# MILVLG/mmnas

Measured on AMD Instinct MI355X. Metric: supernet fwd+bwd steps/sec (VQA arch, bs=64), higher is better.
Workload: dtype f32 (bf16x6 split-operand MFMA, fp32 accumulate); 1 GPU; Net_Search supernet WEIGHT step: sample + fwd + BCE(sum) + bwd (+ gradient all-reduce), HSIZE 256, B=64/GPU, 100x2048 regions + 14 tokens, dropout 0.1 (search_vqa.py:279-292; BASELINE configs[2]); global_batch=64, parallelism=dp1, grad_allreduce=none, rccl_ranks=1, rank_id_sum_ok=True, lstm_fallback=False, dp_rows=1, dp_buckets=3, optimizer_in_step=False, gemm_split=6, hip_force_dev_kernarg=1

## Files before the change

include/mmnas_hip.h:

```cpp
#ifndef MMNAS_HIP_H
#define MMNAS_HIP_H

#include <stddef.h>
#include <stdint.h>

#ifdef __cplusplus
extern "C" {
#endif

#define MMNAS_ABI_VERSION 1

enum {
  MMNAS_OK = 0,
  MMNAS_E_SHAPE = -1,
  MMNAS_E_ARG = -2,
  MMNAS_E_LAUNCH = -3
};

enum {
  MMNAS_F_NORM = 1,
  MMNAS_F_RESIDUAL = 2,
  MMNAS_F_MASK = 4,
  MMNAS_F_REL = 8,
  MMNAS_F_SELF = 16,
  MMNAS_F_TRAIN = 32,
  MMNAS_F_RELRAW = 64
};

int mmnas_abi_version(void);
const char* mmnas_last_error(void);

enum {
  MMNAS_SWITCH_DEFAULT = 0,
  MMNAS_SWITCH_ENV = 1,
  MMNAS_SWITCH_SET = 2,
  MMNAS_SWITCH_UNREAD = 4
};
int mmnas_switch_count(void);
int mmnas_switch_info(int i, const char** name, const char** help, int* dflt, int* value, int* source);

int mmnas_dropout_mask(float* out, size_t n, float p, uint64_t seed, uint32_t site, void* stream);

enum { MMNAS_GEMM_NT = 0, MMNAS_GEMM_NN = 1, MMNAS_GEMM_TN = 2 };

typedef struct mmnas_gemm_group {
  int M;
  const float* A[3];
  const float* B[3];
  float* C;
  const float* bias;
  const float* residual;
  const float* gate;
  float* colsum;
  uint64_t drop_seed;
} mmnas_gemm_group;

#define MMNAS_GEMM_MAX_GROUPS 9

typedef struct mmnas_gemm_desc {
  int layout, ngroups, nseg;
  int N, K;
  int lda, ldb, ldc, ldres, ldgate;
  int relu, split_k;
  int accumulate;
  int b_planes;
  float alpha, gate_scale;
  float drop_p;
  uint32_t drop_site;
  uint64_t drop_seed;
  mmnas_gemm_group g[MMNAS_GEMM_MAX_GROUPS];
} mmnas_gemm_desc;

int mmnas_gemm(const mmnas_gemm_desc* d, void* stream);

int mmnas_gemm_ln(const mmnas_gemm_desc* d, const float* ln_a, const float* ln_b, float* y, float eps, void* stream);
int mmnas_set_gemm_ln(int on);

int mmnas_split_planes(const float* w, void* planes, size_t n, void* stream);

int mmnas_gemm_pair(const mmnas_gemm_desc* dgrad, const mmnas_gemm_desc* wgrad, void* stream);

int mmnas_lstm_supported(int E, int H);
int mmnas_lstm_fwd(const float* x_tm, const float* Wih, const float* Whh, const float* bias, float* xp, float* Hall,
                   float* Call, float* Gall, float* out, int T, int B, int E, int H, void* stream);
int mmnas_lstm_bwd(const float* dout, const float* Whh, const float* Call, const float* Gall, float* DG, float* dc,
                   float* scratch, int T, int B, int H, void* stream);

int mmnas_lstm_seq_supported(int H, int B);
int mmnas_lstm_seq_fwd(const float* xp, const float* bhh, const float* Whh, float* Hprev, float* Cs, float* Gall,
                       float* out, int T, int B, int H, void* stream);
int mmnas_lstm_seq_bwd(const float* dout, const float* Whh, const float* Cs, const float* Gall, float* DG, int T,
                       int B, int H, void* stream);
int mmnas_lstm_seq_timed_out(void* stream);

int mmnas_gemm_reload_tuning(void);

int mmnas_layernorm_fwd(const float* x, const float* a, const float* b, float* y,
                        int M, int d, float eps, void* stream);
int mmnas_layernorm_bwd(const float* x, const float* a, const float* dy, float* dx,
                        float* da, float* db, float* ddrop, float* dcol, float* ws,
                        float drop_p, uint64_t seed, uint32_t site,
                        int M, int d, float eps, void* stream);

size_t mmnas_layernorm_bwd_ws_floats(int M, int d);

int mmnas_colsum(const float* x, float* out, int M, int N, int ldx, void* stream);

int mmnas_eltwise_fwd(int kind, const float* x, float* y, size_t n, void* stream);
int mmnas_eltwise_bwd(int kind, const float* x, const float* dy, float* dx, size_t n, void* stream);
int mmnas_drop_add(const float* x, const float* res, float* y, size_t n, float drop_p, uint64_t seed,
                   uint32_t site, void* stream);
int mmnas_glu_fwd(const float* h, float* y, int M, int C, int relu, float drop_p, uint64_t seed,
                  uint32_t site, void* stream);
int mmnas_glu_bwd(const float* h, const float* dy, float* dh, int M, int C, int relu, float drop_p,
                  uint64_t seed, uint32_t site, void* stream);

int mmnas_row_is_zero(const float* f, uint8_t* mask, long rows, int d, void* stream);
int mmnas_glimpse1_supported(int K);
size_t mmnas_glimpse1_bwd_ws_floats(long rows, int K);
int mmnas_glimpse1_fwd(const float* x, const float* w, const float* b, float* y, long rows, int K, void* stream);
int mmnas_glimpse1_bwd(const float* dy, const float* x, const float* w, float* dx, float* dw, float* db, float* ws, long rows, int K,
                       void* stream);
int mmnas_attflat_pool_fwd(const float* logits, const float* x, const uint8_t* mask, float* probs, float* pooled,
                           int B, int S, int d, int G, void* stream);
int mmnas_attflat_pool_bwd(const float* probs, const float* x, const uint8_t* mask, const float* dpooled,
                           float* dlogits, float* dx, int B, int S, int d, int G, void* stream);

int mmnas_relation_embedding(const float* bbox, const int* nobj, float* out, int B, int S, void* stream);

int mmnas_semantic_embedding(const long* ques_ix, const int* nwords, const float* emb, float* out, int B, int S,
                             int E, long V, void* stream);

int mmnas_onehot_rows(float* out, int rows, int width, const int* idx_host, void* stream);

#define MMNAS_MIXED_MAX 8
size_t mmnas_mixed_sum_ws_floats(void);
int mmnas_node_mix_fwd(const float* const* z, const float* const* ln_a, const float* const* ln_b, int n, const float* gate,
                       float* out, int M, int d, float eps, void* stream);
int mmnas_node_mix_bwd(const float* const* z, const float* const* ln_a, const float* const* ln_b, int n, const float* gate,
                       const float* dout, float* d_active, int active, float* dgate, float* ws, int M, int d, float eps,
                       void* stream);
int mmnas_mixed_sum_fwd(const float* const* outs_host, int n, const float* gate, float* out, size_t count,
                        void* stream);
int mmnas_mixed_sum_bwd(const float* const* outs_host, int n, const float* gate, const float* dout,
                        float* d_active, int active, float* dgate, float* ws, size_t count, void* stream);
int mmnas_alpha_full_step(float* prob, const float* gate_grad, float* m, float* v, float* prob_grad, int rows,
                          int width, float lr, float beta1, float beta2, float eps, int step, void* stream);
int mmnas_alpha_full_step_wd(float* prob, const float* gate_grad, float* m, float* v, float* prob_grad, int rows,
                             int width, float lr, float beta1, float beta2, float eps, float weight_decay, int step,
                             void* stream);
int mmnas_alpha_two_step(float* prob, const float* gate_grad, float* m, float* v, float* prob_grad, int rows, int width,
                         const int* pair_host, float lr, float beta1, float beta2, float eps, float weight_decay, int step,
                         void* stream);

int mmnas_embedding_bwd(const long* idx, const float* dy, float* dW, long n_tok, int E, long V, void* stream);
size_t mmnas_embedding_bwd_det_ws_floats(long n_tok, int E);
int mmnas_embedding_bwd_det(const long* idx, const float* dy, float* dW, float* ws, long n_tok, int E, long V, float scale,
                            void* stream);

int mmnas_rel_bias_fwd(const float* rel, const float* Wr, const float* br, float* biasT,
                       int B, int Sq, int Sk, int R, int H, void* stream);
int mmnas_rel_bias_bwd(const float* rel, const float* Wr, const float* br, const float* dbiasT,
                       float* drel, float* dWr, float* dbr, int accumulate_drel,
                       int B, int Sq, int Sk, int R, int H, void* stream);

int mmnas_rel_fused_supported(int C, int R, int H);
int mmnas_rel_fused_fwd(const float* raw, const float* Wy, const float* by, const float* Wr,
                        const float* br, float* biasT, int B, int Sq, int Sk, int C, int R, int H,
                        void* stream);
size_t mmnas_rel_fused_bwd_ws_floats(int B, int Sq, int Sk);
int mmnas_rel_fused_bwd(const float* raw, const float* Wy, const float* by, const float* Wr,
                        const float* br, const float* dbiasT, float* dWy, float* dby, float* dWr,
                        float* dbr, float* ws, int B, int Sq, int Sk, int C, int R, int H,
                        void* stream);
int mmnas_rel_fused_fwd_ragged(const float* raw, const float* Wy, const float* by, const float* Wr, const float* br,
                               float* biasT, int B, int S, int C, int R, int H, const int* off, void* stream);
int mmnas_rel_fused_bwd_ragged(const float* raw, const float* Wy, const float* by, const float* Wr, const float* br,
                               const float* dbiasT, float* dWy, float* dby, float* dWr, float* dbr, float* ws,
                               int B, int S, int C, int R, int H, const int* off, const int* tile_off, int ntiles, void* stream);

#define MMNAS_REL_MULTI_MAX 32
typedef struct mmnas_rel_multi {
  int B, S, C, R, H, n_ops;
  const float* raw;
  const float* Wy; const float* by;
  float* dWy; float* dby;
  const float* Wr[MMNAS_REL_MULTI_MAX];
  const float* br[MMNAS_REL_MULTI_MAX];
  float* biasT[MMNAS_REL_MULTI_MAX];
  const float* dbiasT[MMNAS_REL_MULTI_MAX];
  float* dWr[MMNAS_REL_MULTI_MAX]; float* dbr[MMNAS_REL_MULTI_MAX];
  const int* off; const int* tile_off; int ntiles, reserved;
  float* ws;
  const unsigned char* key_mask;
} mmnas_rel_multi;
int mmnas_rel_multi_supported(int C, int R, int H);
size_t mmnas_rel_multi_bwd_ws_floats(int B, int S);
int mmnas_rel_multi_fwd(const mmnas_rel_multi* m, void* stream);
int mmnas_rel_multi_bwd(const mmnas_rel_multi* m, void* stream);
int mmnas_set_rel_hoist(int on);
int mmnas_set_rel_keylimit(int on);
int mmnas_set_guided_hoist(int on);
int mmnas_set_rel_overlap(int on);

typedef struct mmnas_mha_desc {
  int B, H, Sq, Sk, dh;
  int ldq, ldk, ldv, ldo;
  const float* Q; const float* K; const float* V;
  const uint8_t* mask;
  const float* biasT;
  float* O;
  float* lse;
  float drop_p; uint32_t drop_site; uint64_t drop_seed;
  const float* dO;
  float* dQ; float* dK; float* dV;
  float* dbiasT;
  float* delta;
  const int* q_off; const int* k_off;
} mmnas_mha_desc;

int mmnas_mha_core_fwd(const mmnas_mha_desc* d, void* stream);
int mmnas_mha_core_bwd(const mmnas_mha_desc* d, void* stream);
int mmnas_mha_core_fwd_indexed(const mmnas_mha_desc* d, const int* kv_idx, void* stream);

typedef struct mmnas_att_op {
  int B, Sq, Sk, d, di, H, dh, R;
  int flags;
  float drop_p, eps;
  uint64_t seed;
  const float* xq;
  const float* xkv;
  const uint8_t* mask;
  const float* rel;
  const float* Wq; const float* Wk; const float* Wv;
  const float* Wm;
  const float* Wr; const float* br;
  const float* ln_a; const float* ln_b;
  float* y;
  void* save;
  void* ws;
  const float* dy;
  float* dxq;
  float* dxkv;
  float* drel;
  float* dWq; float* dWk; float* dWv; float* dWm;
  float* dWr; float* dbr; float* dln_a; float* dln_b;
  int C;
  const float* Wy; const float* by;
  float* dWy; float* dby;
  const int* q_off; const int* k_off;
  int Mq, Mk;
  const int* rel_tile_off;
  int rel_ntiles, reserved2;
} mmnas_att_op;

typedef struct mmnas_plan {
  size_t save_bytes, ws_fwd_bytes, ws_bwd_bytes;
} mmnas_plan;

int mmnas_set_small_ops(int on);
int mmnas_set_small_bwd(int on);
int mmnas_set_small_ffn(int on);
int mmnas_att_op_plan(const mmnas_att_op* op, mmnas_plan* plan);
int mmnas_att_op_fwd(const mmnas_att_op* op, void* stream);
int mmnas_att_op_bwd(const mmnas_att_op* op, void* stream);

typedef struct mmnas_mlp_op {
  int M, nl;
  int dims[4];
  int flags;
  float drop_p, eps;
  uint64_t seed;
  const float* x;
  const float* W[3];
  const float* b[3];
  const float* ln_a; const float* ln_b;
  float* y;
  void* save; void* ws;
  const float* dy;
  float* dx;
  float* dW[3]; float* db[3];
  float* dln_a; float* dln_b;
} mmnas_mlp_op;

int mmnas_mlp_op_plan(const mmnas_mlp_op* op, mmnas_plan* plan);
int mmnas_mlp_op_fwd(const mmnas_mlp_op* op, void* stream);
int mmnas_mlp_op_bwd(const mmnas_mlp_op* op, void* stream);

#define MMNAS_CHAIN_MAX_OPS 128
enum { MMNAS_CHAIN_ATT = 0, MMNAS_CHAIN_MLP = 1 };
typedef struct mmnas_chain_op {
  int kind, on_y;
  mmnas_att_op att;
  mmnas_mlp_op mlp;
  int node, cand, detached, reserved;
} mmnas_chain_op;
typedef struct mmnas_chain {
  int n_ops;
  const mmnas_chain_op* ops;
  int B, Sx, Sy, d;
  const float* x_in; const float* y_in;
  const uint8_t* x_mask; const uint8_t* y_mask;
  const float* x_rel; const float* y_rel;
  void* arena;
  float* x_out; float* y_out;
  const float* dx_out; const float* dy_out;
  float* dx_in; float* dy_in;
  int use_side_stream, reserved;
  void* const* marks;
  int mixed, gate_width;
  const float* gate;
  float* dgate;
  const int* y_off;
  const int* y_tile_off;
  int Ny, y_ntiles;
} mmnas_chain;
int mmnas_chain_plan(const mmnas_chain* c, size_t* arena_bytes);
int mmnas_chain_fwd(const mmnas_chain* c, void* stream);
int mmnas_chain_bwd(const mmnas_chain* c, void* stream);
int mmnas_chain_join(void* main_stream, void* waiting_stream);
int mmnas_set_chain_overlap(int on);

typedef struct mmnas_attflat_side {
  int S, reserved;
  const float* x; const uint8_t* mask;
  const float* W1; const float* b1; const float* W2; const float* b2; const float* Wm; const float* bm;
  float* dW1; float* db1; float* dW2; float* db2; float* dWm; float* dbm;
  uint64_t seed;
  float* dx;
  const int* off;
  int M, reserved2;
} mmnas_attflat_side;
typedef struct mmnas_head {
  int B, d, MID, G, OUT, ANS, flags, reserved;
  float drop_p, eps;
  mmnas_attflat_side sx, sy;
  const float* ln_a; const float* ln_b; float* dln_a; float* dln_b;
  const float* Wp; const float* bp; float* dWp; float* dbp;
  float* logits;
  const float* dlogits;
  void* arena;
} mmnas_head;
int mmnas_head_plan(const mmnas_head* hd, size_t* arena_bytes);
int mmnas_head_fwd(const mmnas_head* hd, void* stream);
int mmnas_head_bwd(const mmnas_head* hd, void* stream);
int mmnas_bce_logits_sum_fwd(const float* logits, const float* target, float* loss, size_t n, void* stream);
int mmnas_bce_logits_bwd(const float* logits, const float* target, const float* go, float* dlogits, size_t n, void* stream);

int mmnas_im2col_seq(const float* x, float* col, int B, int S, int d, int k, void* stream);
int mmnas_pad_seq(const float* x, float* xp, int B, int S, int d, int front, int Sp, long rows_total, void* stream);
int mmnas_col2im_seq(const float* dcol, float* dx, int B, int S, int d, int k, void* stream);
int mmnas_dwconv_seq_fwd(const float* x, const float* w, const float* bias, float* y,
                         int B, int S, int d, int k, void* stream);
int mmnas_dwconv_seq_bwd(const float* x, const float* w, const float* dy, float* dx, float* dw,
                         float* db, int B, int S, int d, int k, void* stream);

typedef struct mmnas_segment { float* ptr; uint64_t offset; uint64_t n; } mmnas_segment;
int mmnas_pack_segments(const mmnas_segment* segs, int nseg, float* staging, float scale,
                        int direction, void* stream);
int mmnas_pack_rows(const float* x, const int* off, float* packed, int B, int S, int d, void* stream);
int mmnas_unpack_rows(const float* packed, const int* off, float* x, int B, int S, int d, void* stream);
int mmnas_pack_segments_host(const mmnas_segment* segs_host, int nseg, float* staging, float scale,
                             int direction, void* stream);

int mmnas_adam_step(float* p, const float* g, float* m, float* v, size_t n, float lr, float beta1,
                    float beta2, float eps, float weight_decay, const float* sumsq, float max_norm,
                    int step, void* stream);
int mmnas_sgd_step(float* p, const float* g, float* buf, size_t n, float lr, float momentum, float dampening,
                   float weight_decay, int nesterov, int first, const float* sumsq, float max_norm, void* stream);
int mmnas_sumsq(const float* g, size_t n, float* out, void* stream);

int mmnas_itm_pair_head(const float* xflat, const int* cap_idx, const float* yflat, const float* ln_a, const float* ln_b,
                        const float* Wp, const float* bp, float* logits, float* scores, const int* img_row, const int* cap_col,
                        long ld, int P, int D, float eps, void* stream);
int mmnas_rank_matrix(const float* S, int Ni, int Nc, long ld, int* i2t_rank, int* i2t_tie, int* t2i_rank, int* t2i_tie,
                      int* nan_flag, void* stream);
int mmnas_row_topk(const float* S, int N, int C, long ld, int k, int* out, int* nan_flag, void* stream);

int mmnas_vgd_targets(const float* bbox, const int* nobj, const double* gt, int B, int S, double thr, int mode, const double* norm,
                      float* scores, float* scores_mask, float* transformed, float* bbox_mask, int* err_flag, void* stream);
int mmnas_vgd_ground(const float* pred_scores, const float* pred_reg, const float* bbox, const float* img_shape, const float* gt,
                     int B, int S, double thr, long long* idx, float* box, double* iou, unsigned char* hit, long long* counts,
                     int* err_flag, void* stream);

int mmnas_vqa_answer(const float* logits, int B, int A, long ld, const int* slot_idx, long slot_base, int slot_step, int nslots,
                     const int* qmap, const int* row_ptr, const int* col, const int* k, int nq, long long* pred, int* credit,
                     int* count, int* err_flag, void* stream);
int mmnas_vqa_accuracy(const int* credit, const int* qmap, const int* ans_type, const int* ques_type, int N, int nq, int n_at,
                       int n_qt, long long* totals, int* err_flag, void* stream);
int mmnas_vqa_answer_targets(const int* ans_ix, int B, int n, int A, float* out, int* err_flag, void* stream);

int mmnas_vgd_loss_fwd(const float* pred_scores, const float* pred_reg, const float* scores, const float* bbox,
                       const float* scores_mask, const float* bbox_mask, int B, int S, int smask_full, int bmask_full, int mode,
                       int loss_avg, double batch_size, double lam, float* loss, float* parts, float* dpred_scores,
                       float* dpred_reg, void* stream);
int mmnas_itm_triplet_loss_fwd(const float* scores_pos, const float* scores_negc, const float* scores_negi, long n, int mode,
                               float margin, int mean, float* loss, float* grads, void* stream);
int mmnas_loss_grad_scale(const float* saved, const float* go, float* out, size_t n, void* stream);

int mmnas_vgd_head_supported(int S, int F);
size_t mmnas_vgd_head_bwd_ws_floats(int B, int S, int F);
int mmnas_vgd_head_fwd(const float* yf, const float* xp, const float* ln_a, const float* ln_b, const float* Ws, const float* bs,
                       const float* Wr, const float* br, float* scores, float* reg, float* mean, float* rstd, int B, int S, int F,
                       float eps, int log_softmax, void* stream);
int mmnas_vgd_head_bwd(const float* dscores, const float* dreg, const float* yf, const float* xp, const float* ln_a,
                       const float* ln_b, const float* Ws, const float* Wr, const float* scores, const float* mean,
                       const float* rstd, float* dyf, float* dxp, float* dln_a, float* dln_b, float* dWs, float* dbs, float* dWr,
                       float* dbr, float* ws, int B, int S, int F, float eps, int log_softmax, void* stream);

enum { MMNAS_K_GEMM = 0, MMNAS_K_MHA_FWD = 1, MMNAS_K_MHA_BWD = 2, MMNAS_K_REL_FWD = 3, MMNAS_K_REL_BWD = 4,
       MMNAS_K_ROWOPS = 5, MMNAS_K_LSTM = 6, MMNAS_K_SMALL = 7 , MMNAS_K_COUNT = 8 };
typedef struct mmnas_prof_stat { double ms, flops, bytes; long launches; } mmnas_prof_stat;
int mmnas_prof_enable(int on);
int mmnas_prof_collect(mmnas_prof_stat* stats );

#ifdef __cplusplus
}
#endif
#endif
```

mmnas_amd/_lib.py:

```python
import ctypes as C
import logging
import os

import torch

from . import switches

_HERE = os.path.dirname(os.path.abspath(__file__))
LIB_PATH = os.environ.get(switches.LIB_PATH.name) or os.path.join(_HERE, 'lib', 'libmmnas_hip.so')

log = logging.getLogger('mmnas_amd')


def _launch_configuration():
    name = 'HIP_FORCE_DEV_KERNARG'
    if name in os.environ:
        return os.environ[name], 'inherited'
    if torch.cuda.is_initialized():
        log.warning('mmnas_amd was imported after HIP had initialised and %s is not set: kernel arguments go through host-visible '
                    'memory, the ~300 short launches of a step run 20-40 %% slower.  Export %s=1 or import mmnas / mmnas_amd '
                    'before the first CUDA call.', name, name)
        return None, 'unset_after_hip_init'
    os.environ[name] = '1'
    return '1', 'set_by_library'


KERNARG_VALUE, KERNARG_SOURCE = _launch_configuration()

F_NORM, F_RESIDUAL, F_MASK, F_REL, F_SELF, F_TRAIN, F_RELRAW = 1, 2, 4, 8, 16, 32, 64
GEMM_NT, GEMM_NN, GEMM_TN = 0, 1, 2

_fp = C.c_void_p


class GemmGroup(C.Structure):
    _fields_ = [('M', C.c_int), ('A', _fp * 3), ('B', _fp * 3), ('C', _fp), ('bias', _fp),
                ('residual', _fp), ('gate', _fp), ('colsum', _fp), ('drop_seed', C.c_uint64)]


GEMM_MAX_GROUPS = 9


class GemmDesc(C.Structure):
    _fields_ = [('layout', C.c_int), ('ngroups', C.c_int), ('nseg', C.c_int), ('N', C.c_int), ('K', C.c_int),
                ('lda', C.c_int), ('ldb', C.c_int), ('ldc', C.c_int), ('ldres', C.c_int), ('ldgate', C.c_int),
                ('relu', C.c_int), ('split_k', C.c_int), ('accumulate', C.c_int), ('b_planes', C.c_int), ('alpha', C.c_float), ('gate_scale', C.c_float),
                ('drop_p', C.c_float), ('drop_site', C.c_uint32), ('drop_seed', C.c_uint64),
                ('g', GemmGroup * GEMM_MAX_GROUPS)]


class MhaDesc(C.Structure):
    _fields_ = [('B', C.c_int), ('H', C.c_int), ('Sq', C.c_int), ('Sk', C.c_int), ('dh', C.c_int),
                ('ldq', C.c_int), ('ldk', C.c_int), ('ldv', C.c_int), ('ldo', C.c_int),
                ('Q', _fp), ('K', _fp), ('V', _fp), ('mask', _fp), ('biasT', _fp), ('O', _fp), ('lse', _fp),
                ('drop_p', C.c_float), ('drop_site', C.c_uint32), ('drop_seed', C.c_uint64),
                ('dO', _fp), ('dQ', _fp), ('dK', _fp), ('dV', _fp), ('dbiasT', _fp), ('delta', _fp), ('q_off', _fp), ('k_off', _fp)]


class AttOp(C.Structure):
    _fields_ = [('B', C.c_int), ('Sq', C.c_int), ('Sk', C.c_int), ('d', C.c_int), ('di', C.c_int),
                ('H', C.c_int), ('dh', C.c_int), ('R', C.c_int), ('flags', C.c_int),
                ('drop_p', C.c_float), ('eps', C.c_float), ('seed', C.c_uint64),
                ('xq', _fp), ('xkv', _fp), ('mask', _fp), ('rel', _fp),
                ('Wq', _fp), ('Wk', _fp), ('Wv', _fp), ('Wm', _fp), ('Wr', _fp), ('br', _fp),
                ('ln_a', _fp), ('ln_b', _fp), ('y', _fp), ('save', _fp), ('ws', _fp),
                ('dy', _fp), ('dxq', _fp), ('dxkv', _fp), ('drel', _fp),
                ('dWq', _fp), ('dWk', _fp), ('dWv', _fp), ('dWm', _fp), ('dWr', _fp), ('dbr', _fp),
                ('dln_a', _fp), ('dln_b', _fp),
                ('C', C.c_int), ('Wy', _fp), ('by', _fp), ('dWy', _fp), ('dby', _fp),
                ('q_off', _fp), ('k_off', _fp), ('Mq', C.c_int), ('Mk', C.c_int), ('rel_tile_off', _fp), ('rel_ntiles', C.c_int), ('reserved2', C.c_int)]


class Plan(C.Structure):
    _fields_ = [('save_bytes', C.c_size_t), ('ws_fwd_bytes', C.c_size_t), ('ws_bwd_bytes', C.c_size_t)]


class MlpOp(C.Structure):
    _fields_ = [('M', C.c_int), ('nl', C.c_int), ('dims', C.c_int * 4), ('flags', C.c_int),
                ('drop_p', C.c_float), ('eps', C.c_float), ('seed', C.c_uint64),
                ('x', _fp), ('W', _fp * 3), ('b', _fp * 3), ('ln_a', _fp), ('ln_b', _fp), ('y', _fp),
                ('save', _fp), ('ws', _fp), ('dy', _fp), ('dx', _fp), ('dW', _fp * 3), ('db', _fp * 3),
                ('dln_a', _fp), ('dln_b', _fp)]


class ChainOp(C.Structure):
    _fields_ = [('kind', C.c_int), ('on_y', C.c_int), ('att', AttOp), ('mlp', MlpOp),
                ('node', C.c_int), ('cand', C.c_int), ('detached', C.c_int), ('reserved', C.c_int)]


class Chain(C.Structure):
    _fields_ = [('n_ops', C.c_int), ('ops', C.POINTER(ChainOp)), ('B', C.c_int), ('Sx', C.c_int), ('Sy', C.c_int),
                ('d', C.c_int), ('x_in', _fp), ('y_in', _fp), ('x_mask', _fp), ('y_mask', _fp), ('x_rel', _fp),
                ('y_rel', _fp), ('arena', _fp), ('x_out', _fp), ('y_out', _fp), ('dx_out', _fp), ('dy_out', _fp),
                ('dx_in', _fp), ('dy_in', _fp), ('use_side_stream', C.c_int), ('reserved', C.c_int),
                ('marks', C.c_void_p), ('mixed', C.c_int), ('gate_width', C.c_int), ('gate', _fp), ('dgate', _fp),
                ('y_off', _fp), ('y_tile_off', _fp), ('Ny', C.c_int), ('y_ntiles', C.c_int)]


CHAIN_MAX_OPS = 128


class AttFlatSide(C.Structure):
    _fields_ = [('S', C.c_int), ('reserved', C.c_int), ('x', _fp), ('mask', _fp), ('W1', _fp), ('b1', _fp), ('W2', _fp),
                ('b2', _fp), ('Wm', _fp), ('bm', _fp), ('dW1', _fp), ('db1', _fp), ('dW2', _fp), ('db2', _fp), ('dWm', _fp),
                ('dbm', _fp), ('seed', C.c_uint64), ('dx', _fp), ('off', _fp), ('M', C.c_int), ('reserved2', C.c_int)]


class Head(C.Structure):
    _fields_ = [('B', C.c_int), ('d', C.c_int), ('MID', C.c_int), ('G', C.c_int), ('OUT', C.c_int), ('ANS', C.c_int),
                ('flags', C.c_int), ('reserved', C.c_int), ('drop_p', C.c_float), ('eps', C.c_float),
                ('sx', AttFlatSide), ('sy', AttFlatSide), ('ln_a', _fp), ('ln_b', _fp), ('dln_a', _fp), ('dln_b', _fp),
                ('Wp', _fp), ('bp', _fp), ('dWp', _fp), ('dbp', _fp), ('logits', _fp), ('dlogits', _fp), ('arena', _fp)]


REL_MULTI_MAX = 32


class RelMulti(C.Structure):
    _fields_ = [('B', C.c_int), ('S', C.c_int), ('C', C.c_int), ('R', C.c_int), ('H', C.c_int), ('n_ops', C.c_int),
                ('raw', _fp), ('Wy', _fp), ('by', _fp), ('dWy', _fp), ('dby', _fp),
                ('Wr', _fp * REL_MULTI_MAX), ('br', _fp * REL_MULTI_MAX), ('biasT', _fp * REL_MULTI_MAX),
                ('dbiasT', _fp * REL_MULTI_MAX), ('dWr', _fp * REL_MULTI_MAX), ('dbr', _fp * REL_MULTI_MAX),
                ('off', _fp), ('tile_off', _fp), ('ntiles', C.c_int), ('reserved', C.c_int), ('ws', _fp), ('key_mask', _fp)]


class ProfStat(C.Structure):
    _fields_ = [('ms', C.c_double), ('flops', C.c_double), ('bytes', C.c_double), ('launches', C.c_long)]


K_NAMES = ['gemm', 'mha_fwd', 'mha_bwd', 'rel_fwd', 'rel_bwd', 'rowops', 'lstm', 'small_ops']


class Segment(C.Structure):
    _fields_ = [('ptr', _fp), ('offset', C.c_uint64), ('n', C.c_uint64)]


_i, _f, _u32, _u64, _sz = C.c_int, C.c_float, C.c_uint32, C.c_uint64, C.c_size_t
SYMBOLS = {
    'mmnas_abi_version': (_i, []),
    'mmnas_last_error': (C.c_char_p, []),
    'mmnas_switch_count': (_i, []),
    'mmnas_switch_info': (_i, [_i, C.POINTER(C.c_char_p), C.POINTER(C.c_char_p)] + [C.POINTER(_i)] * 3),
    'mmnas_dropout_mask': (_i, [_fp, _sz, _f, _u64, _u32, _fp]),
    'mmnas_gemm': (_i, [C.POINTER(GemmDesc), _fp]),
    'mmnas_split_planes': (_i, [_fp, _fp, _sz, _fp]),
    'mmnas_gemm_ln': (_i, [C.POINTER(GemmDesc), _fp, _fp, _fp, _f, _fp]),
    'mmnas_set_gemm_ln': (_i, [_i]),
    'mmnas_gemm_pair': (_i, [C.POINTER(GemmDesc), C.POINTER(GemmDesc), _fp]),
    'mmnas_gemm_reload_tuning': (_i, []),
    'mmnas_lstm_supported': (_i, [_i, _i]),
    'mmnas_lstm_fwd': (_i, [_fp] * 9 + [_i, _i, _i, _i, _fp]),
    'mmnas_lstm_bwd': (_i, [_fp] * 7 + [_i, _i, _i, _fp]),
    'mmnas_lstm_seq_supported': (_i, [_i, _i]),
    'mmnas_set_small_ops': (_i, [_i]),
    'mmnas_set_small_bwd': (_i, [_i]),
    'mmnas_set_small_ffn': (_i, [_i]),
    'mmnas_set_chain_overlap': (_i, [_i]),
    'mmnas_lstm_seq_fwd': (_i, [_fp] * 7 + [_i, _i, _i, _fp]),
    'mmnas_lstm_seq_bwd': (_i, [_fp] * 5 + [_i, _i, _i, _fp]),
    'mmnas_lstm_seq_timed_out': (_i, [_fp]),
    'mmnas_layernorm_fwd': (_i, [_fp, _fp, _fp, _fp, _i, _i, _f, _fp]),
    'mmnas_layernorm_bwd': (_i, [_fp, _fp, _fp, _fp, _fp, _fp, _fp, _fp, _fp, _f, _u64, _u32, _i, _i, _f, _fp]),
    'mmnas_layernorm_bwd_ws_floats': (_sz, [_i, _i]),
    'mmnas_colsum': (_i, [_fp, _fp, _i, _i, _i, _fp]),
    'mmnas_eltwise_fwd': (_i, [_i, _fp, _fp, _sz, _fp]),
    'mmnas_eltwise_bwd': (_i, [_i, _fp, _fp, _fp, _sz, _fp]),
    'mmnas_drop_add': (_i, [_fp, _fp, _fp, _sz, _f, _u64, _u32, _fp]),
    'mmnas_glu_fwd': (_i, [_fp, _fp, _i, _i, _i, _f, _u64, _u32, _fp]),
    'mmnas_glu_bwd': (_i, [_fp, _fp, _fp, _i, _i, _i, _f, _u64, _u32, _fp]),
    'mmnas_rel_bias_fwd': (_i, [_fp, _fp, _fp, _fp, _i, _i, _i, _i, _i, _fp]),
    'mmnas_rel_bias_bwd': (_i, [_fp, _fp, _fp, _fp, _fp, _fp, _fp, _i, _i, _i, _i, _i, _i, _fp]),
    'mmnas_row_is_zero': (_i, [_fp, _fp, C.c_long, _i, _fp]),
    'mmnas_glimpse1_supported': (_i, [_i]),
    'mmnas_glimpse1_bwd_ws_floats': (_sz, [C.c_long, _i]),
    'mmnas_glimpse1_fwd': (_i, [_fp, _fp, _fp, _fp, C.c_long, _i, _fp]),
    'mmnas_glimpse1_bwd': (_i, [_fp, _fp, _fp, _fp, _fp, _fp, _fp, C.c_long, _i, _fp]),
    'mmnas_attflat_pool_fwd': (_i, [_fp, _fp, _fp, _fp, _fp, _i, _i, _i, _i, _fp]),
    'mmnas_attflat_pool_bwd': (_i, [_fp, _fp, _fp, _fp, _fp, _fp, _i, _i, _i, _i, _fp]),
    'mmnas_relation_embedding': (_i, [_fp, _fp, _fp, _i, _i, _fp]),
    'mmnas_semantic_embedding': (_i, [_fp, _fp, _fp, _fp, _i, _i, _i, C.c_long, _fp]),
    'mmnas_onehot_rows': (_i, [_fp, _i, _i, C.POINTER(C.c_int), _fp]),
    'mmnas_mixed_sum_ws_floats': (_sz, []),
    'mmnas_mixed_sum_fwd': (_i, [C.POINTER(_fp), _i, _fp, _fp, _sz, _fp]),
    'mmnas_mixed_sum_bwd': (_i, [C.POINTER(_fp), _i, _fp, _fp, _fp, _i, _fp, _fp, _sz, _fp]),
    'mmnas_alpha_full_step': (_i, [_fp, _fp, _fp, _fp, _fp, _i, _i, _f, _f, _f, _f, _i, _fp]),
    'mmnas_alpha_full_step_wd': (_i, [_fp, _fp, _fp, _fp, _fp, _i, _i, _f, _f, _f, _f, _f, _i, _fp]),
    'mmnas_alpha_two_step': (_i, [_fp, _fp, _fp, _fp, _fp, _i, _i, C.POINTER(C.c_int), _f, _f, _f, _f, _f, _i, _fp]),
    'mmnas_embedding_bwd': (_i, [_fp, _fp, _fp, C.c_long, _i, C.c_long, _fp]),
    'mmnas_node_mix_fwd': (_i, [_fp, _fp, _fp, _i, _fp, _fp, _i, _i, _f, _fp]),
    'mmnas_node_mix_bwd': (_i, [_fp, _fp, _fp, _i, _fp, _fp, _fp, _i, _fp, _fp, _i, _i, _f, _fp]),
    'mmnas_embedding_bwd_det': (_i, [_fp, _fp, _fp, _fp, C.c_long, _i, C.c_long, _f, _fp]),
    'mmnas_embedding_bwd_det_ws_floats': (_sz, [C.c_long, _i]),
    'mmnas_rel_fused_supported': (_i, [_i, _i, _i]),
    'mmnas_rel_fused_fwd': (_i, [_fp, _fp, _fp, _fp, _fp, _fp, _i, _i, _i, _i, _i, _i, _fp]),
    'mmnas_rel_fused_bwd_ws_floats': (_sz, [_i, _i, _i]),
    'mmnas_rel_fused_bwd': (_i, [_fp, _fp, _fp, _fp, _fp, _fp, _fp, _fp, _fp, _fp, _fp, _i, _i, _i, _i, _i, _i, _fp]),
    'mmnas_rel_fused_fwd_ragged': (_i, [_fp, _fp, _fp, _fp, _fp, _fp, _i, _i, _i, _i, _i, _fp, _fp]),
    'mmnas_rel_fused_bwd_ragged': (_i, [_fp] * 11 + [_i, _i, _i, _i, _i, _fp, _fp, _i, _fp]),
    'mmnas_rel_multi_supported': (_i, [_i, _i, _i]),
    'mmnas_rel_multi_bwd_ws_floats': (_sz, [_i, _i]),
    'mmnas_rel_multi_fwd': (_i, [C.POINTER(RelMulti), _fp]),
    'mmnas_rel_multi_bwd': (_i, [C.POINTER(RelMulti), _fp]),
    'mmnas_set_rel_hoist': (_i, [_i]),
    'mmnas_set_rel_keylimit': (_i, [_i]),
    'mmnas_set_guided_hoist': (_i, [_i]),
    'mmnas_set_rel_overlap': (_i, [_i]),
    'mmnas_mha_core_fwd': (_i, [C.POINTER(MhaDesc), _fp]),
    'mmnas_mha_core_bwd': (_i, [C.POINTER(MhaDesc), _fp]),
    'mmnas_mha_core_fwd_indexed': (_i, [C.POINTER(MhaDesc), _fp, _fp]),
    'mmnas_itm_pair_head': (_i, [_fp] * 11 + [C.c_long, _i, _i, _f, _fp]),
    'mmnas_rank_matrix': (_i, [_fp, _i, _i, C.c_long, _fp, _fp, _fp, _fp, _fp, _fp]),
    'mmnas_row_topk': (_i, [_fp, _i, _i, C.c_long, _i, _fp, _fp, _fp]),
    'mmnas_vgd_targets': (_i, [_fp, _fp, _fp, _i, _i, C.c_double, _i, _fp, _fp, _fp, _fp, _fp, _fp, _fp]),
    'mmnas_vgd_ground': (_i, [_fp] * 5 + [_i, _i, C.c_double] + [_fp] * 7),
    'mmnas_vqa_answer': (_i, [_fp, _i, _i, C.c_long, _fp, C.c_long, _i, _i] + [_fp] * 4 + [_i] + [_fp] * 5),
    'mmnas_vqa_accuracy': (_i, [_fp] * 4 + [_i] * 4 + [_fp, _fp, _fp]),
    'mmnas_vqa_answer_targets': (_i, [_fp, _i, _i, _i, _fp, _fp, _fp]),
    'mmnas_vgd_loss_fwd': (_i, [_fp] * 6 + [_i] * 6 + [C.c_double, C.c_double] + [_fp] * 5),
    'mmnas_itm_triplet_loss_fwd': (_i, [_fp, _fp, _fp, C.c_long, _i, _f, _i, _fp, _fp, _fp]),
    'mmnas_loss_grad_scale': (_i, [_fp, _fp, _fp, _sz, _fp]),
    'mmnas_vgd_head_supported': (_i, [_i, _i]),
    'mmnas_vgd_head_bwd_ws_floats': (_sz, [_i, _i, _i]),
    'mmnas_vgd_head_fwd': (_i, [_fp] * 12 + [_i, _i, _i, _f, _i, _fp]),
    'mmnas_vgd_head_bwd': (_i, [_fp] * 20 + [_i, _i, _i, _f, _i, _fp]),
    'mmnas_att_op_plan': (_i, [C.POINTER(AttOp), C.POINTER(Plan)]),
    'mmnas_att_op_fwd': (_i, [C.POINTER(AttOp), _fp]),
    'mmnas_att_op_bwd': (_i, [C.POINTER(AttOp), _fp]),
    'mmnas_mlp_op_plan': (_i, [C.POINTER(MlpOp), C.POINTER(Plan)]),
    'mmnas_mlp_op_fwd': (_i, [C.POINTER(MlpOp), _fp]),
    'mmnas_mlp_op_bwd': (_i, [C.POINTER(MlpOp), _fp]),
    'mmnas_chain_plan': (_i, [C.POINTER(Chain), C.POINTER(C.c_size_t)]),
    'mmnas_chain_fwd': (_i, [C.POINTER(Chain), _fp]),
    'mmnas_chain_bwd': (_i, [C.POINTER(Chain), _fp]),
    'mmnas_chain_join': (_i, [_fp, _fp]),
    'mmnas_head_plan': (_i, [C.POINTER(Head), C.POINTER(C.c_size_t)]),
    'mmnas_head_fwd': (_i, [C.POINTER(Head), _fp]),
    'mmnas_head_bwd': (_i, [C.POINTER(Head), _fp]),
    'mmnas_bce_logits_sum_fwd': (_i, [_fp, _fp, _fp, _sz, _fp]),
    'mmnas_bce_logits_bwd': (_i, [_fp, _fp, _fp, _fp, _sz, _fp]),
    'mmnas_im2col_seq': (_i, [_fp, _fp, _i, _i, _i, _i, _fp]),
    'mmnas_pack_rows': (_i, [_fp, _fp, _fp, _i, _i, _i, _fp]),
    'mmnas_unpack_rows': (_i, [_fp, _fp, _fp, _i, _i, _i, _fp]),
    'mmnas_pad_seq': (_i, [_fp, _fp, _i, _i, _i, _i, _i, C.c_long, _fp]),
    'mmnas_col2im_seq': (_i, [_fp, _fp, _i, _i, _i, _i, _fp]),
    'mmnas_dwconv_seq_fwd': (_i, [_fp, _fp, _fp, _fp, _i, _i, _i, _i, _fp]),
    'mmnas_dwconv_seq_bwd': (_i, [_fp, _fp, _fp, _fp, _fp, _fp, _i, _i, _i, _i, _fp]),
    'mmnas_pack_segments': (_i, [_fp, _i, _fp, _f, _i, _fp]),
    'mmnas_pack_segments_host': (_i, [C.POINTER(Segment), _i, _fp, _f, _i, _fp]),
    'mmnas_adam_step': (_i, [_fp, _fp, _fp, _fp, _sz, _f, _f, _f, _f, _f, _fp, _f, _i, _fp]),
    'mmnas_sgd_step': (_i, [_fp, _fp, _fp, _sz, _f, _f, _f, _f, _i, _i, _fp, _f, _fp]),
    'mmnas_sumsq': (_i, [_fp, _sz, _fp, _fp]),
    'mmnas_prof_enable': (_i, [_i]),
    'mmnas_prof_collect': (_i, [C.POINTER(ProfStat)]),
}

_lib = None


class MMNasHipError(RuntimeError):
    pass


def lib():
    global _lib
    if _lib is None:
        if not os.path.exists(LIB_PATH):
            raise MMNasHipError(
                'libmmnas_hip.so not found at %s -- build it with `python -c "import __graft_entry__ as g; '
                'g.build()"` or `make -C mmnas_amd/csrc`.  There is no CPU fallback.' % LIB_PATH)
        l = C.CDLL(LIB_PATH)
        for name, (res, args) in SYMBOLS.items():
            fn = getattr(l, name)
            fn.restype = res
            fn.argtypes = args
        if l.mmnas_abi_version() != 1:
            raise MMNasHipError('libmmnas_hip.so ABI version %d != 1' % l.mmnas_abi_version())
        _lib = l
    return _lib


def check(rc):
    if rc != 0:
        raise MMNasHipError('libmmnas_hip: %s (code %d)' % (lib().mmnas_last_error().decode(), rc))


def ptr(t):
    if t is None:
        return None
    if not t.is_cuda:
        raise MMNasHipError('mmnas_amd operators run on the MI355X only: got a %s tensor (no CPU fallback)'
                            % t.device)
    if not t.is_contiguous():
        raise MMNasHipError('non-contiguous tensor passed to the HIP boundary')
    return t.data_ptr()


def fptr(t):
    if t is not None and t.dtype != torch.float32:
        raise MMNasHipError('expected float32, got %s' % t.dtype)
    return ptr(t)


def stream():
    return torch._C._cuda_getCurrentRawStream(torch._C._cuda_getDevice())
```

mmnas_amd/csrc/gemm.hip:

```cpp
#include <stddef.h>
#include <string.h>
#include <map>
#include <mutex>
#include <utility>
#include <algorithm>
#include <climits>
#include "common.h"
#include "gemm_split.h"

namespace mmnas {

struct GemmGroupK {
  int M;
  int tile0;
  const float* A[3];
  const float* B[3];
  float* C;
  const float* bias;
  const float* residual;
  const float* gate;
  float* colsum;
  uint32_t seed_lo, site_key;
};

constexpr int MAXG = MMNAS_GEMM_MAX_GROUPS;

struct GemmK {
  int ngroups, nseg, N, K;
  int lda, ldb, ldc, ldres, ldgate;
  int relu, accumulate;
  int tiles_n, ntiles;
  int xcd_remap;
  int gm;
  int ntk, T;
  int mode;
  int n_full, full_per, sk_per;
  int P;
  int U;
  int gtile0[MAXG];
  int tn_shift;
  unsigned nt_magic;
  float* ws;
  int* cnt;
  int avec, bvec;
  float alpha, gate_scale;
  DropCfg drop;
  const float* lg_cprev;
  const float* lg_c;
  float* lg_cout;
  float* lg_gates;
  float* lg_h2;
  float* lg_dc;
  const float* lg_act;
  int lg_ldh2, lg_pad;
  GemmGroupK g[MAXG];
};

enum { MODE_TILE = 0, MODE_SPLIT = 1, MODE_STREAM = 2 };

__device__ __forceinline__ int cdiv_dev(int a, int b) { return (a + b - 1) / b; }

#ifndef MMNAS_OCC64
#define MMNAS_OCC64 4
#endif
#ifndef MMNAS_OCC_NS
#define MMNAS_OCC_NS 3
#endif
#ifndef MMNAS_OCC128
#define MMNAS_OCC128 2
#endif
#ifndef MMNAS_BK
#define MMNAS_BK 32
#endif
constexpr int BK = MMNAS_BK;
constexpr int LDK = BK + 4;
constexpr int KQ = BK / 4;

typedef unsigned long long u64;
__device__ __forceinline__ void st_agent(u64* ptr, float a, float b) {
  __hip_atomic_store(ptr, ((u64)__float_as_uint(b) << 32) | __float_as_uint(a), __ATOMIC_RELAXED, __HIP_MEMORY_SCOPE_AGENT);
}
__device__ __forceinline__ u64 ld_agent(const u64* ptr) {
  return __hip_atomic_load(ptr, __ATOMIC_RELAXED, __HIP_MEMORY_SCOPE_AGENT);
}

#ifndef MMNAS_TMAP
#define MMNAS_TMAP 2
#endif
template <int BR>
__device__ __forceinline__ void t_map(int tid, int j, int& kp, int& rq) {
#if MMNAS_TMAP == 2
  const int hi = tid >> 5;
  constexpr int RB = BR / 32;
  rq = (tid & 7) | ((hi % RB) << 3);
  kp = ((tid >> 3) & 3) + 4 * (hi / RB) + (1024 / BR) * j;
#elif MMNAS_TMAP == 1
  rq = (tid >> 3) % (BR / 4);
  kp = (tid & 7) + 8 * ((tid >> 3) / (BR / 4)) + (1024 / BR) * j;
#else
  kp = tid / (BR / 4) + (1024 / BR) * j;
  rq = tid % (BR / 4);
#endif
}
__device__ __forceinline__ int t_flip(int rq) { return MMNAS_TMAP == 2 ? (rq >> 2) & 1 : 0; }

template <int NS>
__device__ __forceinline__ void split_put(unsigned* dst, float x0, float x1, int row, int kp) {
  constexpr int RSW = NS * 16 + 4;
  unsigned a0, a1 = 0, a2 = 0;
  split_pair<NS>(x0, x1, a0, a1, a2);
  unsigned* d = dst + row * RSW + swz(kp, row);
  d[0] = a0;
  if (NS > 1) d[16] = a1;
  if (NS > 2) d[32] = a2;
}
template <int BR, int NS>
__device__ __forceinline__ void split_store_t(unsigned* dst, const float4 e, const float4 o, int tid, int j) {
  int kp, rq;
  t_map<BR>(tid, j, kp, rq);
  const int row = 4 * rq, fl = t_flip(rq);
  split_put<NS>(dst, fl ? e.y : e.x, fl ? o.y : o.x, row + fl, kp);
  split_put<NS>(dst, fl ? e.x : e.y, fl ? o.x : o.y, row + 1 - fl, kp);
  split_put<NS>(dst, fl ? e.w : e.z, fl ? o.w : o.z, row + 2 + fl, kp);
  split_put<NS>(dst, fl ? e.z : e.w, fl ? o.z : o.w, row + 3 - fl, kp);
}

#ifdef MMNAS_DBG_STAMP
__device__ unsigned long long g_stamp_acc[8];
__device__ unsigned long long g_life_acc[8];
#endif

template <int BM, int BN, int NS>
struct GemmShape {
  static constexpr int RSW = NS ? NS * 16 + 4 : LDK;
  static constexpr int A_SZ = BM * RSW, B_SZ = BN * RSW;
};

template <int BM, int BN, bool AKC, bool BKC, bool FAST, int NS, int EPI = 0, int PF = 1, bool BDMA = false, int LEAN = 0>
__device__ __forceinline__ void gemm_body(const GemmK& p, const int bid, const int nwg, const int koff,
                                          float* __restrict__ As, float* __restrict__ Bs, float* __restrict__ As1,
                                          float* __restrict__ Bs1, int& s_old) {
  static_assert(PF == 1 || (PF == 2 && FAST && (NS == 0 || NS == 1 || NS == 3)), "the two-stage prefetch exists for the buffer-load path (fp32, bf16x1 and bf16x6)");
  static_assert(NS == 0 || (FAST && BK == 32), "the bf16-split path exists for the buffer-load path only");
  static_assert(!BDMA || (NS == 3 && AKC && BKC && FAST && PF == 1 && BM == 64 && BN == 64 && EPI == 0), "LDS-DMA weight planes: NT 64^2 bf16x6 only");
  static_assert(!LEAN || (NS > 0 && (AKC || !BKC) && FAST && PF == 2 && BM == 64 && BN == 64 && EPI == 0 && !BDMA), "lean form: 64^2 split-operand kernels");
  constexpr bool LEAN_TN = LEAN && !AKC;
  constexpr bool LEAN_EL = LEAN == 3;
  constexpr bool LEAN_SW = LEAN && AKC && !LEAN_EL;
  constexpr bool LEAN_WT = (LEAN_SW && LEAN == 1) || LEAN_EL;
  constexpr int RSWB = 48;
  constexpr int WM = BM / 2, WN = BN / 2, TM = WM / 32, TN = WN / 32;
  constexpr int RSW = GemmShape<BM, BN, NS>::RSW;
  constexpr int NA = BM * BK / 1024, NB = BN * BK / 1024;

#ifdef MMNAS_DBG_STAMP
  unsigned long long life_prev = __builtin_readcyclecounter();
#define MMNAS_LIFE(i) do { const unsigned long long c_ = __builtin_readcyclecounter(); if (threadIdx.x == 0 && bid == MMNAS_DBG_STAMP) g_life_acc[i] += c_ - life_prev; life_prev = c_; } while (0)
#else
#define MMNAS_LIFE(i) do { } while (0)
#endif
  {
    const char* ka = (const char*)__builtin_amdgcn_kernarg_segment_ptr() + koff;
    unsigned t0, t1, t2, t3, t4, t5, t6, t7, t8, t9;
    asm volatile(
        "s_load_dword %0, %10, 0x0\n\ts_load_dword %1, %10, 0x40\n\ts_load_dword %2, %10, 0x80\n\t"
        "s_load_dword %3, %10, 0xc0\n\ts_load_dword %4, %10, 0x100\n\ts_load_dword %5, %10, 0x140\n\t"
        "s_load_dword %6, %10, 0x180\n\ts_load_dword %7, %10, 0x1c0\n\ts_load_dword %8, %10, 0x200\n\t"
        "s_load_dword %9, %10, 0x240\n\ts_waitcnt lgkmcnt(0)"
        : "=&s"(t0), "=&s"(t1), "=&s"(t2), "=&s"(t3), "=&s"(t4), "=&s"(t5), "=&s"(t6), "=&s"(t7), "=&s"(t8), "=&s"(t9)
        : "s"(ka)
        : "memory");
  }
  static_assert(offsetof(GemmK, g) + 3 * sizeof(GemmGroupK) > 0x200 && offsetof(GemmK, g) + 3 * sizeof(GemmGroupK) <= 0x280,
                "update the kernel-argument warm-up loads (header + the first three groups; further groups -- the architecture "
                "step's node-wide launches -- take their first-touch miss)");

  MMNAS_LIFE(0);
  const int tid = threadIdx.x;
  const int lane = tid & 63, wave = tid >> 6;
  const int l31 = lane & 31, hh = lane >> 5;
  const int wm = wave >> 1, wn = wave & 1;

  struct Hdr { int N, K, lda, ldb, tiles_n, ntiles, xcd_remap, gm, ntk, T, mode, n_full, full_per, sk_per, P, U, gt[MAXG]; };
  Hdr h;
  h.N = p.N; h.K = p.K; h.lda = p.lda; h.ldb = p.ldb; h.tiles_n = p.tiles_n; h.ntiles = p.ntiles; h.xcd_remap = p.xcd_remap;
  h.gm = p.gm; h.ntk = p.ntk; h.T = p.T; h.mode = p.mode; h.n_full = p.n_full; h.full_per = p.full_per; h.sk_per = p.sk_per;
  h.P = p.P; h.U = p.U;
#pragma unroll
  for (int g = 0; g < MAXG; ++g) h.gt[g] = p.gtile0[g];
  asm volatile("" : "+s"(h.N), "+s"(h.K), "+s"(h.lda), "+s"(h.ldb), "+s"(h.tiles_n), "+s"(h.ntiles), "+s"(h.xcd_remap), "+s"(h.gm),
               "+s"(h.ntk), "+s"(h.T), "+s"(h.mode), "+s"(h.n_full), "+s"(h.full_per), "+s"(h.sk_per), "+s"(h.P));
  static_assert(MAXG == 9, "the list of group boundaries below names nine groups");
  asm volatile("" : "+s"(h.U), "+s"(h.gt[1]), "+s"(h.gt[2]), "+s"(h.gt[3]), "+s"(h.gt[4]), "+s"(h.gt[5]), "+s"(h.gt[6]), "+s"(h.gt[7]),
               "+s"(h.gt[8]));
  int v;
  {
    const int q = nwg >> 3, r = nwg & 7, xcd = bid & 7, in = bid >> 3;
    v = (xcd < r ? xcd * (q + 1) : r * (q + 1) + (xcd - r) * q) + in;
    if (!h.xcd_remap) v = bid;
  }
  const int mode = LEAN_TN ? (int)MODE_SPLIT : (LEAN_WT ? (int)MODE_TILE : h.mode);
  int u = 0, uend = 1;
  int vs = v;
  int whole = -1;
  if (mode == MODE_STREAM) {
    if (h.n_full > 0) {
      const int xcd = bid & 7, li = bid >> 3;
      if (li < h.sk_per) vs = xcd * h.sk_per + li;
      else whole = xcd * h.full_per + (li - h.sk_per);
    }
    if (whole < 0) { u = vs * h.P; uend = min(h.U, u + h.P); }
  }

  while (u < uend) {
    int tile, q0, nq;
    if (mode == MODE_TILE || whole >= 0) {
      tile = whole >= 0 ? whole : v; q0 = 0; nq = h.T;
      u = uend;
    } else if (!LEAN_SW && !LEAN_EL && mode == MODE_SPLIT) {
      const int sl = LEAN_TN ? (int)__umulhi((unsigned)v, p.nt_magic) : v / h.ntiles;
      tile = v - sl * h.ntiles;
      q0 = sl * h.P;
      nq = min(h.P, h.T - q0);
      u = uend;
      if (nq <= 0) break;
    } else {
      const int tt = u / h.T;
      tile = h.n_full + tt;
      q0 = u - tt * h.T;
      nq = min(h.T - q0, uend - u);
      u += nq;
    }
    int grp = 0;
#pragma unroll
    for (int g = 1; g < MAXG; ++g) grp += tile >= h.gt[g] ? 1 : 0;
    const GemmGroupK& G = p.g[grp];
    const int Mg = G.M;
    const int tl = tile - G.tile0;
    float* __restrict__ const Cp = G.C;
    const float* __restrict__ const biasp = G.bias;
    const float* __restrict__ const resp = G.residual;
    const float* __restrict__ const gatep = G.gate;
    float* __restrict__ const csp = G.colsum;
    const uint32_t gseed_lo = G.seed_lo, gsite_key = G.site_key;
    const float* const Aseg[3] = {G.A[0], G.A[1], G.A[2]};
    const float* const Bseg[3] = {G.B[0], G.B[1], G.B[2]};
    int tile_m, tile_n;
    if (LEAN) {
      tile_m = tl >> p.tn_shift;
      tile_n = tl - (tile_m << p.tn_shift);
    } else {
      const int tiles_m = cdiv_dev(Mg, BM);
      const int per_block = h.gm * h.tiles_n;
      const int blk = tl / per_block, in = tl - blk * per_block;
      const int rows = min(h.gm, tiles_m - blk * h.gm);
      tile_n = in / rows;
      tile_m = blk * h.gm + (in - tile_n * rows);
    }
    const int m0 = tile_m * BM, n0 = tile_n * BN;

    f32x16 acc[TM][TN];
#pragma unroll
    for (int i = 0; i < TM; ++i)
#pragma unroll
      for (int j = 0; j < TN; ++j)
#pragma unroll
        for (int r = 0; r < 16; ++r) acc[i][j][r] = 0.f;

    float4 rA[2][NA], rB[2][NB];

    unsigned offa[NA], offb[NB];
    size_t bdma_off[3] = {0, 0, 0};
    unsigned stepa = 0, stepb = 0;
    unsigned bytesa = 0, bytesb = 0;
    if (FAST) {
#pragma unroll
      for (int i = 0; i < NA; ++i) {
        const int f = tid + 256 * i;
        if (AKC) {
          const int row = NS ? kc_row(f) : f / KQ, kq = f % KQ, gr = m0 + row;
          offa[i] = gr < Mg ? (unsigned)(gr * h.lda + 4 * kq) * 4u : ~0u;
        } else if (NS) {
          int kp, rq;
          t_map<BM>(tid, i >> 1, kp, rq);
          const int gr = m0 + 4 * rq;
          offa[i] = gr < Mg ? (unsigned)((2 * kp + (i & 1)) * h.lda + gr) * 4u : ~0u;
        } else {
          const int k = f / (BM / 4), rq = f - k * (BM / 4), gr = m0 + 4 * rq;
          offa[i] = gr < Mg ? (unsigned)(k * h.lda + gr) * 4u : ~0u;
        }
      }
#pragma unroll
      for (int i = 0; i < NB; ++i) {
        const int f = tid + 256 * i;
        if (BDMA) {
          offb[i] = 0;
        } else if (BKC) {
          const int row = NS ? kc_row(f) : f / KQ, kq = f % KQ, gr = n0 + row;
          offb[i] = gr < h.N ? (unsigned)(gr * h.ldb + 4 * kq) * 4u : ~0u;
        } else if (NS) {
          int kp, rq;
          t_map<BN>(tid, i >> 1, kp, rq);
          const int gr = n0 + 4 * rq;
          offb[i] = gr < h.N ? (unsigned)((2 * kp + (i & 1)) * h.ldb + gr) * 4u : ~0u;
        } else {
          const int k = f / (BN / 4), rq = f - k * (BN / 4), gr = n0 + 4 * rq;
          offb[i] = gr < h.N ? (unsigned)(k * h.ldb + gr) * 4u : ~0u;
        }
      }
      if (BDMA) {
#pragma unroll
        for (int i = 0; i < 3; ++i) {
          const int o = (wave * 3 + i) * 1024 + lane * 16;
          const int r = o / 192, w = o - r * 192, c = w >> 6, j = ((w & 63) >> 4) ^ ((r >> 2) & 3);
          bdma_off[i] = ((size_t)c * (size_t)h.N * (size_t)h.ldb + (size_t)(n0 + r) * (size_t)h.ldb + 8 * j) * 2u;
        }
      }
      stepa = AKC ? BK * 4u : (unsigned)h.lda * BK * 4u;
      stepb = BKC ? BK * 4u : (unsigned)h.ldb * BK * 4u;
      bytesa = (unsigned)(AKC ? Mg : h.K) * (unsigned)h.lda * 4u;
      bytesb = (unsigned)(BKC ? h.N : h.K) * (unsigned)h.ldb * 4u;
    }

    int seg_c = 0, kt_c = 0;
    if (LEAN_TN) kt_c = q0;
    else if (q0 != 0) { seg_c = q0 / h.ntk; kt_c = q0 - seg_c * h.ntk; }
    auto gload_to = [&](int q, bool live, const int st, const int dbuf = 0) __attribute__((always_inline)) {
      float4* const ra = rA[st];
      float4* const rb = rB[st];
      const int seg = seg_c, kt = kt_c;
      if (++kt_c == h.ntk) { kt_c = 0; ++seg_c; }
      const float* __restrict__ Ap = seg == 0 ? Aseg[0] : (seg == 1 ? Aseg[1] : Aseg[2]);
      const float* __restrict__ Bp = seg == 0 ? Bseg[0] : (seg == 1 ? Bseg[1] : Bseg[2]);
      if (FAST) {
        const __amdgpu_buffer_rsrc_t ra_src = __builtin_amdgcn_make_buffer_rsrc((void*)Ap, 0, bytesa, 0x00020000);
        const __amdgpu_buffer_rsrc_t rb_src = __builtin_amdgcn_make_buffer_rsrc((void*)Bp, 0, bytesb, 0x00020000);
        const unsigned ka = (unsigned)kt * stepa, kb = (unsigned)kt * stepb;
        if (LEAN_SW || LEAN_EL) {
          const __amdgpu_buffer_rsrc_t la_src = __builtin_amdgcn_make_buffer_rsrc((void*)Ap, 0, live ? bytesa : 0u, 0x00020000);
          const __amdgpu_buffer_rsrc_t lb_src = __builtin_amdgcn_make_buffer_rsrc((void*)Bp, 0, live ? bytesb : 0u, 0x00020000);
#pragma unroll
          for (int i = 0; i < NA; ++i) ra[i] = buf_load4(la_src, offa[i], ka);
#pragma unroll
          for (int i = 0; i < NB; ++i) rb[i] = buf_load4(lb_src, offb[i], kb);
          return;
        }
#pragma unroll
        for (int i = 0; i < NA; ++i) ra[i] = buf_load4(ra_src, (offa[i] == ~0u || !live) ? ~0u : offa[i] + ka);
        if (BDMA) {
          const char* bsrc = reinterpret_cast<const char*>(Bp) + (size_t)kt * 64u;
          float* const bd = dbuf ? Bs1 : Bs;
          const int wv = __builtin_amdgcn_readfirstlane(wave);
#pragma unroll
          for (int i = 0; i < 3; ++i)
            __builtin_amdgcn_global_load_lds((const __attribute__((address_space(1))) void*)(bsrc + bdma_off[i]),
                                             (__attribute__((address_space(3))) void*)(bd + (wv * 3 + i) * 256), 16, 0, 0);
          return;
        }
#pragma unroll
        for (int i = 0; i < NB; ++i) rb[i] = buf_load4(rb_src, (offb[i] == ~0u || !live) ? ~0u : offb[i] + kb);
        return;
      }
      const int k0 = kt * BK, kend = h.K;
#pragma unroll
      for (int i = 0; i < NA; ++i) {
        const int f = tid + 256 * i;
        float4 v4 = make_float4(0.f, 0.f, 0.f, 0.f);
        if (AKC) {
          const int row = f / KQ, kq = f % KQ;
          const int gr = m0 + row, gk = k0 + 4 * kq;
          if (gr < Mg && gk < kend) {
            const float* src = Ap + (size_t)gr * h.lda + gk;
            if (p.avec) v4 = *reinterpret_cast<const float4*>(src);
            else {
              v4.x = src[0];
              if (gk + 1 < kend) v4.y = src[1];
              if (gk + 2 < kend) v4.z = src[2];
              if (gk + 3 < kend) v4.w = src[3];
            }
          }
        } else {
          const int k = f / (BM / 4), rq = f - k * (BM / 4);
          const int gk = k0 + k, gr = m0 + 4 * rq;
          if (gk < kend && gr < Mg) {
            const float* src = Ap + (size_t)gk * h.lda + gr;
            if (p.avec) v4 = *reinterpret_cast<const float4*>(src);
            else {
              v4.x = src[0];
              if (gr + 1 < Mg) v4.y = src[1];
              if (gr + 2 < Mg) v4.z = src[2];
              if (gr + 3 < Mg) v4.w = src[3];
            }
          }
        }
        ra[i] = v4;
      }
#pragma unroll
      for (int i = 0; i < NB; ++i) {
        const int f = tid + 256 * i;
        float4 v4 = make_float4(0.f, 0.f, 0.f, 0.f);
        if (BKC) {
          const int row = f / KQ, kq = f % KQ;
          const int gr = n0 + row, gk = k0 + 4 * kq;
          if (gr < h.N && gk < kend) {
            const float* src = Bp + (size_t)gr * h.ldb + gk;
            if (p.bvec) v4 = *reinterpret_cast<const float4*>(src);
            else {
              v4.x = src[0];
              if (gk + 1 < kend) v4.y = src[1];
              if (gk + 2 < kend) v4.z = src[2];
              if (gk + 3 < kend) v4.w = src[3];
            }
          }
        } else {
          const int k = f / (BN / 4), rq = f - k * (BN / 4);
          const int gk = k0 + k, gr = n0 + 4 * rq;
          if (gk < kend && gr < h.N) {
            const float* src = Bp + (size_t)gk * h.ldb + gr;
            if (p.bvec) v4 = *reinterpret_cast<const float4*>(src);
            else {
              v4.x = src[0];
              if (gr + 1 < h.N) v4.y = src[1];
              if (gr + 2 < h.N) v4.z = src[2];
              if (gr + 3 < h.N) v4.w = src[3];
            }
          }
        }
        rb[i] = v4;
      }
    };
    auto gload = [&](int q, int dbuf = 0) __attribute__((always_inline)) { gload_to(q, true, 0, dbuf); };

    auto lstore_from = [&](int buf, const int st) __attribute__((always_inline)) {
      const float4* const ra = rA[st];
      const float4* const rb = rB[st];
      float* a = buf ? As1 : As;
      float* b = buf ? Bs1 : Bs;
      if (NS) {
        unsigned* ua = reinterpret_cast<unsigned*>(a);
        unsigned* ub = reinterpret_cast<unsigned*>(b);
        if (AKC) {
#pragma unroll
          for (int i = 0; i < NA; ++i) split_store_kc<BM, true, NS ? NS : 2>(ua, ra[i], tid + 256 * i);
        } else {
#pragma unroll
          for (int j = 0; j < NA / 2; ++j) split_store_t<BM, NS ? NS : 2>(ua, ra[2 * j], ra[2 * j + 1], tid, j);
        }
        if (BDMA) {
        } else if (BKC) {
#pragma unroll
          for (int i = 0; i < NB; ++i) split_store_kc<BN, true, NS ? NS : 2>(ub, rb[i], tid + 256 * i);
        } else {
#pragma unroll
          for (int j = 0; j < NB / 2; ++j) split_store_t<BN, NS ? NS : 2>(ub, rb[2 * j], rb[2 * j + 1], tid, j);
        }
        return;
      }
#pragma unroll
      for (int i = 0; i < NA; ++i) {
        const int f = tid + 256 * i;
        if (AKC) {
          const int row = f / KQ, kq = f % KQ;
          *reinterpret_cast<float4*>(a + row * LDK + 4 * kq) = ra[i];
        } else {
          const int k = f / (BM / 4), rq = f - k * (BM / 4);
          *reinterpret_cast<float4*>(a + k * BM + 4 * rq) = ra[i];
        }
      }
#pragma unroll
      for (int i = 0; i < NB; ++i) {
        const int f = tid + 256 * i;
        if (BKC) {
          const int row = f / KQ, kq = f % KQ;
          *reinterpret_cast<float4*>(b + row * LDK + 4 * kq) = rb[i];
        } else {
          const int k = f / (BN / 4), rq = f - k * (BN / 4);
          *reinterpret_cast<float4*>(b + k * BN + 4 * rq) = rb[i];
        }
      }
    };
    auto lstore = [&](int buf) __attribute__((always_inline)) { lstore_from(buf, 0); };

    auto mfma_block = [&](int buf) __attribute__((always_inline)) {
#ifdef MMNAS_DBG_NOMFMA
      return;
#endif
      const float* a = buf ? As1 : As;
      const float* b = buf ? Bs1 : Bs;
      if (NS) {
#pragma unroll
// ... 587 lines not shown
    const mmnas_gemm_group& s = d->g[g];
    if (!akc && s.M % 4 != 0) avec = 0;
    MMNAS_REQUIRE(s.M > 0 && s.C, MMNAS_E_ARG, "mmnas_gemm: group %d M=%d C=%p", g, s.M, (void*)s.C);
    k.g[g].M = s.M; k.g[g].C = s.C; k.g[g].bias = s.bias; k.g[g].residual = s.residual; k.g[g].gate = s.gate;
    k.g[g].colsum = s.colsum;
    {
      const DropCfg gd = s.drop_seed ? make_drop(d->drop_p, s.drop_seed, d->drop_site) : k.drop;
      k.g[g].seed_lo = gd.seed_lo; k.g[g].site_key = gd.site_key;
    }
    MMNAS_REQUIRE(!(s.colsum && accumulate), MMNAS_E_ARG, "mmnas_gemm: no column sums when accumulating onto C");
    for (int i = 0; i < 3; ++i) {
      k.g[g].A[i] = s.A[i]; k.g[g].B[i] = s.B[i];
      if (i < d->nseg) {
        MMNAS_REQUIRE(s.A[i] && s.B[i], MMNAS_E_ARG, "mmnas_gemm: group %d segment %d null operand", g, i);
        if (((uintptr_t)s.A[i] & 15) != 0) avec = 0;
        if (((uintptr_t)s.B[i] & 15) != 0) bvec = 0;
      }
    }
    sumM += s.M;
    const double ab = 4.0 * (akc ? (double)(s.M + 128) : (double)d->K) * d->lda;
    if (ab > maxbytes) maxbytes = ab;
  }
  const double bb = 4.0 * (bkc ? (double)(d->N + 128) : (double)d->K) * d->ldb;
  if (bb > maxbytes) maxbytes = bb;
  k.avec = avec; k.bvec = bvec;
  bool fast = avec && bvec && (d->K % BK == 0 || tn) && maxbytes < 4.0e9;
  if (g_tune.generic) fast = false;
  k.ntk = cdiv(d->K, BK);
  k.T = k.ntk * d->nseg;

  auto ntiles_for = [&](int bt) {
    long n = 0;
    for (int g = 0; g < d->ngroups; ++g) n += (long)cdiv(d->g[g].M, bt) * cdiv(d->N, bt);
    return n;
  };
  const int min_units = g_tune.min_units;
  bool big = ntiles_for(128) >= 2048;
  if (g_tune.tile == 128) big = true;
  if (g_tune.tile == 64 || g_tune.tile == 12864) big = false;
  bool wide = !big && g_tune.tile == 12864 && !accumulate && fast && g_tune.split != 2 && g_tune.split != 1;
  if (wide) {
    long n = 0;
    for (int g = 0; g < d->ngroups; ++g) n += (long)cdiv(d->g[g].M, 128) * cdiv(d->N, 64);
    if (n < g_tune.wide_min) wide = false;
  }
  const int bt = big ? 128 : 64;
  const int btm = wide ? 128 : bt, btn = bt;
  k.tiles_n = cdiv(d->N, btn);
  long t0 = 0;
  for (int g = 0; g < MAXG; ++g) k.gtile0[g] = INT_MAX;
  for (int g = 0; g < d->ngroups; ++g) { k.g[g].tile0 = k.gtile0[g] = (int)t0; t0 += (long)cdiv(d->g[g].M, btm) * k.tiles_n; }
  MMNAS_REQUIRE(t0 < (1l << 30), MMNAS_E_SHAPE, "mmnas_gemm: too many output tiles");
  k.ntiles = (int)t0;
  k.gm = g_tune.gm > 0 ? g_tune.gm : 8;
  k.xcd_remap = g_tune.xcd;
  const int slots = g_tune.wgs > 0 ? (g_tune.wgs < MAX_WGS ? g_tune.wgs : MAX_WGS) : ((big || wide) ? 512 : 1024);
  const double per_cu = (double)k.ntiles / 256.0;
  const double dp_eff = per_cu / (double)(long)(per_cu + 0.999999);
  const long long U = (long long)k.ntiles * k.T;
  int sk = g_tune.sk;
  k.mode = MODE_TILE;
  k.P = k.T;
  int nwg = k.ntiles;
  if (accumulate && sk != 0) {
    int want;
    if (g_tune.split_slots > 0) want = g_tune.split_slots / k.ntiles;
    else {
      want = (k.T + g_tune.split_p / 2) / g_tune.split_p;
      if ((long)want * k.ntiles < g_tune.split_minwg) want = (g_tune.split_minwg + k.ntiles - 1) / k.ntiles;
    }
    if (want < 1) want = 1;
    if (want > k.T / min_units) want = k.T / min_units;
    if (want > 1) {
      k.P = (k.T + want - 1) / want;
      const int S = (k.T + k.P - 1) / k.P;
      MMNAS_REQUIRE((long long)S * k.ntiles < (1ll << 30), MMNAS_E_SHAPE, "mmnas_gemm: too many split-K pieces");
      k.mode = MODE_SPLIT;
      nwg = S * k.ntiles;
    }
  } else if (!accumulate && sk != 0 && !big && !wide && U < (1ll << 30) && k.ntiles <= MAX_CNT_TILES && g_tune.wgs == 0 &&
             sk == 1 && k.ntiles > 256 && k.ntiles < 8192 && k.ntiles % 256 != 0 && k.T >= g_tune.hyb_t) {
    const int n_full = (k.ntiles / 256) * 256, R = k.ntiles - n_full;
    const long long Ut = (long long)R * k.T;
    long long P = (Ut + 255) / 256;
    if (P < 2) P = 2;
    int n_sk = (int)((Ut + P - 1) / P);
    n_sk = (n_sk + 7) / 8 * 8;
    k.mode = MODE_STREAM;
    k.n_full = n_full; k.full_per = n_full / 8; k.sk_per = n_sk / 8;
    k.P = (int)P;
    k.U = (int)Ut;
    nwg = n_full + n_sk;
  } else if (!accumulate && sk != 0 && U < (1ll << 30) && k.ntiles <= MAX_CNT_TILES && k.T >= 2 * min_units &&
             (sk == 2 || (!big && !wide && ((dp_eff < 0.6 && k.T >= 16) || (dp_eff < 0.9 && k.T >= 48))))) {
    const int smu = sk == 2 ? min_units : 2 * min_units;
    long long G = U / smu;
    if (G > slots) G = slots;
    if (G < 1) G = 1;
    const long long P = (U + G - 1) / G;
    if (P < k.T) {
      k.mode = MODE_STREAM;
      k.P = (int)P;
      k.U = (int)U;
      nwg = (int)((U + P - 1) / P);
    }
  }
  if (k.mode == MODE_STREAM) {
    SkWorkspace w;
    const int rc = get_workspace(st, &w);
    if (rc) return rc;
    k.ws = w.ws; k.cnt = w.cnt;
  }
  out.tag[0] = 0;
  if (prof_enabled())
    snprintf(out.tag, sizeof(out.tag), "%s M=%d/%d/%d N=%d K=%d seg=%d t%d wg=%d P=%d/%d %s%s", tn ? "TN" : (bkc ? "NT" : "NN"),
             d->g[0].M, d->ngroups > 1 ? d->g[1].M : 0, d->ngroups > 2 ? d->g[2].M : 0, d->N, d->K, d->nseg, wide ? 12864 : bt, nwg, k.P, k.T,
             k.mode == MODE_TILE ? "tile" : (k.mode == MODE_SPLIT ? "split" : (k.n_full ? "hybrid" : "stream")),
             fast ? (g_tune.split == 2 ? " bf16x3" : (g_tune.split == 3 ? " bf16x6" : (g_tune.split == 1 ? " bf16x1" : ""))) : " generic");
  out.flops = 2.0 * sumM * d->N * d->K * d->nseg;
  out.bytes = 4.0 * (sumM * d->K * d->nseg + (double)d->N * d->K * d->nseg * d->ngroups + sumM * d->N);
  out.nwg = nwg; out.layout = d->layout; out.big = big; out.fast = fast; out.wide = wide;
  out.bdma = d->b_planes != 0;
  if (out.bdma) {
    MMNAS_REQUIRE(d->layout == MMNAS_GEMM_NT && fast && !big && !wide && !accumulate && g_tune.split == 3 && d->N % 64 == 0 &&
                  (d->ldb % 8) == 0, MMNAS_E_ARG,
                  "mmnas_gemm: b_planes needs layout NT, 64^2 tiles on the buffer-load path, N %% 64 == 0, ldb %% 8 == 0, MMNAS_GEMM_SPLIT=6 "
                  "(N=%d K=%d ldb=%d)", d->N, d->K, d->ldb);
    if (out.tag[0]) strncat(out.tag, " Bdma", sizeof(out.tag) - strlen(out.tag) - 1);
  }
  out.lean = 0;
  const bool lean_base = fast && !big && !wide && !out.bdma && g_tune.split == 3 && g_tune.pf == 2 &&
                         (k.tiles_n & (k.tiles_n - 1)) == 0 && d->ldc % 4 == 0;
  if (lean_base && (g_tune.lean & 1) && !tn && k.mode != MODE_SPLIT && d->N % 4 == 0 && 4.0 * d->N * d->K * d->nseg <= (double)g_tune.lean_maxb) {
    bool ok = true, any_colsum = false;
    for (int g = 0; g < d->ngroups && ok; ++g) {
      const mmnas_gemm_group& s = d->g[g];
      const double rows = (double)s.M + 1.0;
      if (s.colsum) any_colsum = true;
      ok = ((uintptr_t)s.C & 15) == 0 && rows * d->ldc * 4.0 < 4.0e9 &&
           (!s.bias || ((uintptr_t)s.bias & 15) == 0) &&
           (!s.residual || (((uintptr_t)s.residual & 15) == 0 && d->ldres % 4 == 0 && rows * d->ldres * 4.0 < 4.0e9)) &&
           (!s.gate || (((uintptr_t)s.gate & 15) == 0 && d->ldgate % 4 == 0 && rows * d->ldgate * 4.0 < 4.0e9));
    }
    out.lean = ok ? (k.mode == MODE_TILE ? 1 : 2) : 0;
    if (any_colsum) out.lean = (ok && k.mode == MODE_TILE && d->layout == MMNAS_GEMM_NN) ? 3 : 0;
  } else if (lean_base && tn && k.mode == MODE_SPLIT && d->nseg == 1 && (g_tune.lean & 2) && k.ntiles >= 2 && k.ntiles < 65536 && nwg < 65536) {
    bool ok = true;
    for (int g = 0; g < d->ngroups && ok; ++g) {
      const mmnas_gemm_group& s = d->g[g];
      ok = !s.bias && !s.residual && !s.gate && !s.colsum && ((double)s.M + 1.0) * d->ldc * 4.0 < 4.0e9;
    }
    out.lean = ok ? 1 : 0;
    if (ok) k.nt_magic = (unsigned)(((1ull << 32) + (unsigned)k.ntiles - 1) / (unsigned)k.ntiles);
  }
  if (out.lean) {
    int sh = 0;
    while ((1 << sh) < k.tiles_n) ++sh;
    k.tn_shift = sh;
    if (out.tag[0]) strncat(out.tag, " lean", sizeof(out.tag) - strlen(out.tag) - 1);
  }
  return MMNAS_OK;
}

static int launch_plan(GemmPlan& pl, hipStream_t st) {
  GemmK& k = pl.k;
  ProfScope ps(MMNAS_K_GEMM, pl.flops, pl.bytes, st, pl.tag);
  const int ns = pl.fast ? g_tune.split : 0;
  if (pl.bdma) {
    MMNAS_LAUNCH((gemm_kernel<64, 64, true, true, true, 3, 0, 1, true>), dim3(pl.nwg), dim3(256), 0, st, k);
    return check_launch("gemm");
  }
  if (pl.lean) {
    const dim3 grid(pl.nwg), block(256);
    if (pl.layout == MMNAS_GEMM_NT) {
      if (pl.lean == 1) MMNAS_LAUNCH((gemm_kernel<64, 64, true, true, true, 3, 0, 2, false, 1>), grid, block, 0, st, k);
      else MMNAS_LAUNCH((gemm_kernel<64, 64, true, true, true, 3, 0, 2, false, 2>), grid, block, 0, st, k);
    } else if (pl.layout == MMNAS_GEMM_NN) {
      if (pl.lean == 3) MMNAS_LAUNCH((gemm_kernel<64, 64, true, false, true, 3, 0, 2, false, 3>), grid, block, 0, st, k);
      else if (pl.lean == 1) MMNAS_LAUNCH((gemm_kernel<64, 64, true, false, true, 3, 0, 2, false, 1>), grid, block, 0, st, k);
      else MMNAS_LAUNCH((gemm_kernel<64, 64, true, false, true, 3, 0, 2, false, 2>), grid, block, 0, st, k);
    } else MMNAS_LAUNCH((gemm_kernel<64, 64, false, false, true, 3, 0, 2, false, 1>), grid, block, 0, st, k);
    return check_launch("gemm");
  }
  if (pl.big) {
    if (ns == 1) return launch<128, 128, true, 1>(k, pl.layout, pl.nwg, st);
    if (ns == 2) return launch<128, 128, true, 2>(k, pl.layout, pl.nwg, st);
    if (ns == 3) return launch<128, 128, true, 3>(k, pl.layout, pl.nwg, st);
    return pl.fast ? launch<128, 128, true, 0>(k, pl.layout, pl.nwg, st) : launch<128, 128, false, 0>(k, pl.layout, pl.nwg, st);
  }
  if (pl.wide) return ns == 3 ? launch<128, 64, true, 3>(k, pl.layout, pl.nwg, st) : launch<128, 64, true, 0, 2>(k, pl.layout, pl.nwg, st);
  if (ns == 1) return launch<64, 64, true, 1, 2>(k, pl.layout, pl.nwg, st);
  if (ns == 2) return launch<64, 64, true, 2>(k, pl.layout, pl.nwg, st);
  if (ns == 3) return g_tune.pf == 2 ? launch<64, 64, true, 3, 2>(k, pl.layout, pl.nwg, st) : launch<64, 64, true, 3>(k, pl.layout, pl.nwg, st);
  if (pl.fast && g_tune.pf == 2) return launch<64, 64, true, 0, 2>(k, pl.layout, pl.nwg, st);
  return pl.fast ? launch<64, 64, true, 0>(k, pl.layout, pl.nwg, st) : launch<64, 64, false, 0>(k, pl.layout, pl.nwg, st);
}

}

extern "C" int mmnas_gemm(const mmnas_gemm_desc* d, void* stream) {
  GemmPlan pl;
  const int rc = plan_gemm(d, (hipStream_t)stream, pl);
  if (rc) return rc;
  return launch_plan(pl, (hipStream_t)stream);
}

namespace mmnas {
int gemm_pair_aux(const mmnas_gemm_desc* dgrad, const mmnas_gemm_desc* wgrad, const AuxReduce* aux, hipStream_t st) {
  GemmPlan p0, p1;
  int rc;
  if ((rc = plan_gemm(dgrad, st, p0))) return rc;
  if ((rc = plan_gemm(wgrad, st, p1))) return rc;
  const bool pair = g_tune.pair && p0.fast && p1.fast && !p0.big && !p1.big && !p0.wide && !p1.wide && p0.layout == MMNAS_GEMM_NN &&
                    p1.layout == MMNAS_GEMM_TN && p1.k.mode != MODE_STREAM;
  if (!pair) {
    if (aux && (rc = launch_aux_reduce(*aux, st))) return rc;
    if ((rc = launch_plan(p0, st))) return rc;
    return launch_plan(p1, st);
  }
  AuxReduceK ak;
  memset(&ak, 0, sizeof(ak));
  if (aux && aux->part && g_tune.pair != 3) {
    ak.part = aux->part; ak.nrows = aux->nrows; ak.d = aux->d;
    for (int i = 0; i < 3; ++i) ak.out[i] = aux->out[i];
    ak.ncb = cdiv(aux->d, 16);
    ak.njobs = 3 * ak.ncb;
  } else if (aux && (rc = launch_aux_reduce(*aux, st))) return rc;
  const int naux8 = (ak.njobs + 7) / 8 * 8;
  char tag[96] = "";
  if (prof_enabled()) snprintf(tag, sizeof(tag), "PAIR %.44s | %.40s", p0.tag, p1.tag);
  ProfScope ps(MMNAS_K_GEMM, p0.flops + p1.flops, p0.bytes + p1.bytes, st, tag);
  const int nwg0p = (p0.nwg + 7) / 8 * 8;
  dim3 grid(naux8 + nwg0p + p1.nwg), block(256);
  switch (g_tune.split) {
    case 1: MMNAS_LAUNCH((gemm_pair_kernel<64, 64, 1, 2>), grid, block, 0, st, p0.k, p1.k, p0.nwg, nwg0p, ak, naux8); break;
    case 2: MMNAS_LAUNCH((gemm_pair_kernel<64, 64, 2>), grid, block, 0, st, p0.k, p1.k, p0.nwg, nwg0p, ak, naux8); break;
    case 3:
      if (p0.lean == 3 && p1.lean) MMNAS_LAUNCH((gemm_pair_kernel<64, 64, 3, 2, 3, 1>), grid, block, 0, st, p0.k, p1.k, p0.nwg, nwg0p, ak, naux8);
      else if (p0.lean == 3) MMNAS_LAUNCH((gemm_pair_kernel<64, 64, 3, 2, 3, 0>), grid, block, 0, st, p0.k, p1.k, p0.nwg, nwg0p, ak, naux8);
      else if (p0.lean == 1 && p1.lean) MMNAS_LAUNCH((gemm_pair_kernel<64, 64, 3, 2, 1, 1>), grid, block, 0, st, p0.k, p1.k, p0.nwg, nwg0p, ak, naux8);
      else if (p0.lean == 2 && p1.lean) MMNAS_LAUNCH((gemm_pair_kernel<64, 64, 3, 2, 2, 1>), grid, block, 0, st, p0.k, p1.k, p0.nwg, nwg0p, ak, naux8);
      else if (p0.lean) MMNAS_LAUNCH((gemm_pair_kernel<64, 64, 3, 2, 2, 0>), grid, block, 0, st, p0.k, p1.k, p0.nwg, nwg0p, ak, naux8);
      else if (p1.lean) MMNAS_LAUNCH((gemm_pair_kernel<64, 64, 3, 2, 0, 1>), grid, block, 0, st, p0.k, p1.k, p0.nwg, nwg0p, ak, naux8);
      else if (g_tune.pf == 2) MMNAS_LAUNCH((gemm_pair_kernel<64, 64, 3, 2>), grid, block, 0, st, p0.k, p1.k, p0.nwg, nwg0p, ak, naux8);
      else MMNAS_LAUNCH((gemm_pair_kernel<64, 64, 3>), grid, block, 0, st, p0.k, p1.k, p0.nwg, nwg0p, ak, naux8);
      break;
    default:
      if (g_tune.pf == 2) MMNAS_LAUNCH((gemm_pair_kernel<64, 64, 0, 2>), grid, block, 0, st, p0.k, p1.k, p0.nwg, nwg0p, ak, naux8);
      else MMNAS_LAUNCH((gemm_pair_kernel<64, 64, 0>), grid, block, 0, st, p0.k, p1.k, p0.nwg, nwg0p, ak, naux8);
      break;
  }
  return check_launch("gemm_pair");
}
}

namespace mmnas {
int gemm_wgrad_aux(const mmnas_gemm_desc* wgrad, const AuxReduce* aux, hipStream_t st) {
  GemmPlan p1;
  int rc;
  if ((rc = plan_gemm(wgrad, st, p1))) return rc;
  const bool ride = aux && aux->part && g_tune.pair && g_tune.pair != 3 && g_tune.split == 3 && g_tune.pf == 2 && p1.fast && !p1.big && !p1.wide &&
                    p1.layout == MMNAS_GEMM_TN && p1.k.mode != MODE_STREAM;
  if (!ride) {
    if (aux && (rc = launch_aux_reduce(*aux, st))) return rc;
    return launch_plan(p1, st);
  }
  AuxReduceK ak;
  memset(&ak, 0, sizeof(ak));
  ak.part = aux->part; ak.nrows = aux->nrows; ak.d = aux->d;
  for (int i = 0; i < 3; ++i) ak.out[i] = aux->out[i];
  ak.ncb = cdiv(aux->d, 16);
  ak.njobs = 3 * ak.ncb;
  const int naux8 = (ak.njobs + 7) / 8 * 8;
  char tag[96] = "";
  if (prof_enabled()) snprintf(tag, sizeof(tag), "WGRAD+AUX %.60s", p1.tag);
  ProfScope ps(MMNAS_K_GEMM, p1.flops, p1.bytes, st, tag);
  dim3 grid(naux8 + p1.nwg), block(256);
  if (p1.lean) MMNAS_LAUNCH((gemm_pair_kernel<64, 64, 3, 2, 0, 1>), grid, block, 0, st, p1.k, p1.k, 0, 0, ak, naux8);
  else MMNAS_LAUNCH((gemm_pair_kernel<64, 64, 3, 2>), grid, block, 0, st, p1.k, p1.k, 0, 0, ak, naux8);
  return check_launch("gemm_wgrad_aux");
}
}

extern "C" int mmnas_gemm_pair(const mmnas_gemm_desc* dgrad, const mmnas_gemm_desc* wgrad, void* stream) {
  return gemm_pair_aux(dgrad, wgrad, nullptr, (hipStream_t)stream);
}

namespace mmnas {
__global__ void __launch_bounds__(256) split_planes_kernel(const float4* __restrict__ w, uint2* __restrict__ p0, uint2* __restrict__ p1,
                                                           uint2* __restrict__ p2, size_t n4) {
  for (size_t i = (size_t)blockIdx.x * 256 + threadIdx.x; i < n4; i += (size_t)gridDim.x * 256) {
    const float4 v = w[i];
    unsigned a0, a1, a2, b0, b1, b2;
    split_pair<3>(v.x, v.y, a0, a1, a2);
    split_pair<3>(v.z, v.w, b0, b1, b2);
    p0[i] = make_uint2(a0, b0);
    p1[i] = make_uint2(a1, b1);
    p2[i] = make_uint2(a2, b2);
  }
}
}

extern "C" int mmnas_split_planes(const float* w, void* planes, size_t n, void* stream) {
  MMNAS_REQUIRE(w && planes, MMNAS_E_ARG, "split_planes: null pointer");
  MMNAS_REQUIRE(n > 0 && n % 8 == 0 && ((uintptr_t)w & 15) == 0 && ((uintptr_t)planes & 15) == 0, MMNAS_E_SHAPE,
                "split_planes: n = %zu must be a multiple of 8 and both buffers 16-byte aligned", n);
  const size_t n4 = n / 4;
  unsigned short* pl = (unsigned short*)planes;
  const int blocks = (int)std::min<size_t>((n4 + 255) / 256, 2048);
  MMNAS_LAUNCH(split_planes_kernel, dim3(blocks), dim3(256), 0, (hipStream_t)stream, (const float4*)w, (uint2*)pl, (uint2*)(pl + n),
               (uint2*)(pl + 2 * n), n4);
  return check_launch("split_planes");
}

namespace mmnas {
static int lstm_step_plan(GemmPlan& pl, const mmnas_gemm_desc& d, hipStream_t st, const char* who, int units_per_wg) {
  int rc = plan_gemm(&d, st, pl);
  if (rc) return rc;
  MMNAS_REQUIRE(pl.fast && !pl.big && !pl.wide, MMNAS_E_SHAPE, "%s: shape outside the step kernel's range (hidden size %% 32 == 0, aligned buffers)", who);
  GemmK& k = pl.k;
  k.n_full = k.full_per = k.sk_per = 0;
  if (units_per_wg <= 0 || units_per_wg >= k.T) {
    k.mode = MODE_TILE; k.P = k.T; pl.nwg = k.ntiles;
  } else {
    SkWorkspace w;
    if ((rc = get_workspace(st, &w))) return rc;
    k.ws = w.ws; k.cnt = w.cnt;
    k.mode = MODE_STREAM; k.P = units_per_wg; k.U = k.ntiles * k.T;
    pl.nwg = (k.U + k.P - 1) / k.P;
  }
  return MMNAS_OK;
}
}

extern "C" int mmnas_lstm_supported(int E, int H) { return E > 0 && H >= 32 && H % 32 == 0 && H <= 4096; }

extern "C" int mmnas_lstm_fwd(const float* x_tm, const float* Wih, const float* Whh, const float* bias, float* xp, float* Hall,
                              float* Call, float* Gall, float* out, int T, int B, int E, int H, void* stream) {
  MMNAS_REQUIRE(x_tm && Wih && Whh && bias && xp && Hall && Call && Gall && out, MMNAS_E_ARG, "lstm_fwd: null pointer");
  MMNAS_REQUIRE(T > 0 && B > 0 && mmnas_lstm_supported(E, H), MMNAS_E_SHAPE, "lstm_fwd: T=%d B=%d E=%d H=%d", T, B, E, H);
  hipStream_t st = (hipStream_t)stream;
  mmnas_gemm_desc d;
  memset(&d, 0, sizeof(d));
  d.layout = MMNAS_GEMM_NT; d.ngroups = 1; d.nseg = 1; d.N = 4 * H; d.K = E; d.lda = E; d.ldb = E; d.ldc = 4 * H;
  d.alpha = 1.f; d.gate_scale = 1.f; d.split_k = 1;
  d.g[0].M = T * B; d.g[0].A[0] = x_tm; d.g[0].B[0] = Wih; d.g[0].C = xp; d.g[0].bias = bias;
  int rc = mmnas_gemm(&d, stream);
  if (rc) return rc;
  const size_t bh = (size_t)B * H, bg = (size_t)B * 4 * H;
  for (int t = 0; t < T; ++t) {
    memset(&d, 0, sizeof(d));
    d.layout = MMNAS_GEMM_NT; d.ngroups = 1; d.nseg = 1; d.N = 4 * H; d.K = H; d.lda = H; d.ldb = H; d.ldc = H;
    d.ldres = 4 * H; d.alpha = 1.f; d.gate_scale = 1.f; d.split_k = 1;
    d.g[0].M = B; d.g[0].A[0] = Hall + t * bh; d.g[0].B[0] = Whh; d.g[0].C = Hall + (t + 1) * bh; d.g[0].residual = xp + t * bg;
    GemmPlan pl;
    if ((rc = lstm_step_plan(pl, d, st, "lstm_fwd", sw::lstm_fwd_p.get()))) return rc;
    pl.k.lg_cprev = Call + t * bh; pl.k.lg_cout = Call + (t + 1) * bh; pl.k.lg_gates = Gall + t * bg;
    pl.k.lg_h2 = out + (size_t)t * H; pl.k.lg_ldh2 = T * H;
    ProfScope ps(MMNAS_K_GEMM, pl.flops, pl.bytes, st, pl.tag);
    MMNAS_LAUNCH((gemm_kernel<64, 64, true, true, true, 0, 1>), dim3(pl.nwg), dim3(256), 0, st, pl.k);
  }
  return check_launch("lstm_fwd");
}

extern "C" int mmnas_lstm_bwd(const float* dout, const float* Whh, const float* Call, const float* Gall, float* DG, float* dc,
                              float* scratch, int T, int B, int H, void* stream) {
  MMNAS_REQUIRE(dout && Whh && Call && Gall && DG && dc && scratch, MMNAS_E_ARG, "lstm_bwd: null pointer");
  MMNAS_REQUIRE(T > 0 && B > 0 && mmnas_lstm_supported(1, H), MMNAS_E_SHAPE, "lstm_bwd: T=%d B=%d H=%d", T, B, H);
  hipStream_t st = (hipStream_t)stream;
  const size_t bh = (size_t)B * H, bg = (size_t)B * 4 * H;
  for (int t = T - 1; t >= 0; --t) {
    mmnas_gemm_desc d;
    memset(&d, 0, sizeof(d));
    d.layout = MMNAS_GEMM_NN; d.ngroups = 1; d.nseg = 1; d.N = H; d.K = 4 * H; d.lda = 4 * H; d.ldb = H; d.ldc = H;
    d.ldres = T * H; d.alpha = 1.f; d.gate_scale = 1.f; d.split_k = 1;
    d.g[0].M = B; d.g[0].A[0] = DG + (t + 1) * bg; d.g[0].B[0] = Whh; d.g[0].C = scratch; d.g[0].residual = dout + (size_t)t * H;
    GemmPlan pl;
    int rc;
    if ((rc = lstm_step_plan(pl, d, st, "lstm_bwd", sw::lstm_bwd_p.get()))) return rc;
    pl.k.lg_act = Gall + t * bg; pl.k.lg_c = Call + (t + 1) * bh; pl.k.lg_cprev = Call + t * bh;
    pl.k.lg_dc = dc; pl.k.lg_gates = DG + t * bg;
    ProfScope ps(MMNAS_K_GEMM, pl.flops, pl.bytes, st, pl.tag);
    MMNAS_LAUNCH((gemm_kernel<64, 64, true, false, true, 0, 2>), dim3(pl.nwg), dim3(256), 0, st, pl.k);
  }
  return check_launch("lstm_bwd");
}

#ifdef MMNAS_DBG_STAMP
extern "C" int mmnas_dbg_stamps(unsigned long long* out8, int reset) {
  if (hipMemcpyFromSymbol(out8, reset & 2 ? HIP_SYMBOL(mmnas::g_life_acc) : HIP_SYMBOL(mmnas::g_stamp_acc), 8 * sizeof(unsigned long long)) != hipSuccess) return 1;
  if (reset & 1) {
    unsigned long long z[8] = {0, 0, 0, 0, 0, 0, 0, 0};
    if (hipMemcpyToSymbol(reset & 2 ? HIP_SYMBOL(mmnas::g_life_acc) : HIP_SYMBOL(mmnas::g_stamp_acc), z, sizeof(z)) != hipSuccess) return 1;
  }
  return 0;
}
#endif
```

mmnas_amd/csrc/ops.hip:

```cpp
#include <string.h>
#include <functional>
#include <vector>
#include "common.h"

namespace mmnas {

static inline size_t al(size_t n) { return (n + 255) & ~(size_t)255; }
template <class Op> static inline bool drops(const Op* op) { return (op->flags & MMNAS_F_TRAIN) && op->drop_p > 0.f; }

struct Carver {
  char* base; size_t off;
  explicit Carver(void* p) : base((char*)p), off(0) {}
  float* take(size_t nfloats) { float* r = (float*)(base + off); off += al(nfloats * sizeof(float)); return r; }
};

static void gemm_init(mmnas_gemm_desc& g, int layout, int N, int K, int lda, int ldb, int ldc) {
  memset(&g, 0, sizeof(g));
  g.layout = layout; g.ngroups = 1; g.nseg = 1; g.N = N; g.K = K; g.lda = lda; g.ldb = ldb; g.ldc = ldc;
  g.alpha = 1.f; g.gate_scale = 1.f; g.split_k = 1;
}

struct AttLayout {
  size_t Mq, Mk;
  float *Q, *K, *V, *att, *stats, *z, *biasT;
// ... 64 lines not shown
                    "%s: a relation bias on packed rows needs the lazy handle (RELRAW), SELF and the relation tile offsets", who);
  }
  return MMNAS_OK;
}

}

using namespace mmnas;

extern "C" int mmnas_att_op_plan(const mmnas_att_op* op, mmnas_plan* plan) {
  int rc = att_check(op, "att_op_plan");
  if (rc) return rc;
  MMNAS_REQUIRE(plan, MMNAS_E_ARG, "att_op_plan: null plan");
  mmnas_att_op tmp = *op;
  tmp.save = nullptr; tmp.ws = nullptr;
  AttLayout L = att_layout(&tmp);
  plan->save_bytes = L.save_bytes;
  plan->ws_fwd_bytes = 256;
  plan->ws_bwd_bytes = L.ws_bwd_bytes;
  return MMNAS_OK;
}

namespace mmnas {
static int att_fwd_impl(const mmnas_att_op* op, void* stream, bool defer_ln, bool* ln_done, bool rel_ready = false, bool kv_ready = false);
}
extern "C" int mmnas_att_op_fwd(const mmnas_att_op* op, void* stream) {
  bool done;
  return mmnas::att_fwd_impl(op, stream, false, &done);
}
namespace mmnas {
static void att_qkv_groups(const mmnas_att_op* op, const AttLayout& L, mmnas_gemm_group* g) {
  memset(g, 0, 3 * sizeof(*g));
  g[0].M = (int)L.Mq; g[0].A[0] = op->xq;  g[0].B[0] = op->Wq; g[0].C = L.Q;
  g[1].M = (int)L.Mk; g[1].A[0] = op->xkv; g[1].B[0] = op->Wk; g[1].C = L.K;
  g[2].M = (int)L.Mk; g[2].A[0] = op->xkv; g[2].B[0] = op->Wv; g[2].C = L.V;
}

static void att_core_desc(const mmnas_att_op* op, const AttLayout& L, mmnas_mha_desc* m) {
  const int fl = op->flags, di = op->di;
  const bool drop = drops(op);
  memset(m, 0, sizeof(*m));
  m->B = op->B; m->H = op->H; m->Sq = op->Sq; m->Sk = op->Sk; m->dh = op->dh;
  m->ldq = m->ldk = m->ldv = m->ldo = di;
  m->Q = L.Q; m->K = L.K; m->V = L.V; m->mask = (fl & MMNAS_F_MASK) ? op->mask : nullptr; m->biasT = L.biasT;
  m->O = L.att; m->lse = L.stats;
  m->q_off = op->q_off; m->k_off = op->k_off;
  m->drop_p = drop ? op->drop_p : 0.f; m->drop_site = 0; m->drop_seed = op->seed;
}

static int att_core_fwd(const mmnas_att_op* op, const AttLayout& L, void* stream, mmnas_mha_desc* desc_only = nullptr, bool rel_ready = false) {
  const int fl = op->flags;
  const bool rel = (fl & MMNAS_F_REL) && !rel_ready;
  int rc;
  if (rel) {
    if (fl & MMNAS_F_RELRAW) {
      MMNAS_REQUIRE(op->Wy && op->by, MMNAS_E_ARG, "att_op_fwd: RELRAW without Wy/by");
      if (op->Sq == op->Sk && mmnas_rel_multi_supported(op->C, op->R, op->H) && (long)op->B * op->H * op->Sq * op->Sq < (1l << 31) &&
          !sw::rel_fwd_valu.get()) {
        mmnas_rel_multi q;
        memset(&q, 0, sizeof(q));
        q.B = op->B; q.S = op->Sq; q.C = op->C; q.R = op->R; q.H = op->H; q.n_ops = 1;
        q.raw = op->rel; q.Wy = op->Wy; q.by = op->by;
        q.Wr[0] = op->Wr; q.br[0] = op->br; q.biasT[0] = L.biasT;
        if (op->q_off) {
          MMNAS_REQUIRE(op->rel_tile_off, MMNAS_E_ARG, "att_op_fwd: packed rows without the relation tile offsets");
          q.off = op->q_off; q.tile_off = op->rel_tile_off; q.ntiles = op->rel_ntiles;
        }
        rc = mmnas_rel_multi_fwd(&q, stream);
      } else
      rc = op->q_off ? mmnas_rel_fused_fwd_ragged(op->rel, op->Wy, op->by, op->Wr, op->br, L.biasT, op->B, op->Sq, op->C, op->R,
                                                  op->H, op->q_off, stream)
                     : mmnas_rel_fused_fwd(op->rel, op->Wy, op->by, op->Wr, op->br, L.biasT, op->B, op->Sq, op->Sk, op->C, op->R,
                                           op->H, stream);
    } else {
      rc = mmnas_rel_bias_fwd(op->rel, op->Wr, op->br, L.biasT, op->B, op->Sq, op->Sk, op->R, op->H, stream);
    }
    if (rc) return rc;
  }
  if (desc_only) { att_core_desc(op, L, desc_only); return MMNAS_OK; }
  mmnas_mha_desc m;
  att_core_desc(op, L, &m);
  return mmnas_mha_core_fwd(&m, stream);
}

static void att_merge_group(const mmnas_att_op* op, const AttLayout& L, mmnas_gemm_group* g) {
  const bool norm = op->flags & MMNAS_F_NORM;
  memset(g, 0, sizeof(*g));
  g->M = (int)L.Mq; g->A[0] = L.att; g->B[0] = op->Wm; g->C = norm ? L.z : op->y;
  if (op->flags & MMNAS_F_RESIDUAL) g->residual = op->xq;
  g->drop_seed = op->seed;
}

static int att_fwd_args(const mmnas_att_op* op) {
  int rc = att_check(op, "att_op_fwd");
  if (rc) return rc;
  MMNAS_REQUIRE(op->xq && op->xkv && op->Wq && op->Wk && op->Wv && op->Wm && op->y && op->save, MMNAS_E_ARG,
                "att_op_fwd: null pointer");
  const int fl = op->flags;
  if (fl & MMNAS_F_NORM) MMNAS_REQUIRE(op->ln_a && op->ln_b, MMNAS_E_ARG, "att_op_fwd: NORM without ln parameters");
  if (fl & MMNAS_F_REL) MMNAS_REQUIRE(op->rel && op->Wr && op->br, MMNAS_E_ARG, "att_op_fwd: REL without rel/Wr/br");
  if (fl & MMNAS_F_MASK) MMNAS_REQUIRE(op->mask, MMNAS_E_ARG, "att_op_fwd: MASK without mask");
  return MMNAS_OK;
}
}

static int mmnas::att_fwd_impl(const mmnas_att_op* op, void* stream, bool defer_ln, bool* ln_done, bool rel_ready, bool kv_ready) {
  *ln_done = true;
  int rc = att_fwd_args(op);
  if (rc) return rc;
  const int fl = op->flags;
  const bool norm = fl & MMNAS_F_NORM;
  const bool drop = drops(op);
  AttLayout L = att_layout(op);
  const int d = op->d, di = op->di;
  if (op->xq == op->xkv && att_ln_place(op).fwd) return sa_small_fwd(op, L.Q, L.K, L.V, L.att, L.stats, L.z, (hipStream_t)stream);

  mmnas_gemm_desc g;
  gemm_init(g, MMNAS_GEMM_NT, di, d, d, d, di);
  g.ngroups = kv_ready ? 1 : 3;
  att_qkv_groups(op, L, g.g);
  if ((rc = mmnas_gemm(&g, stream))) return rc;
  if ((rc = att_core_fwd(op, L, stream, nullptr, rel_ready))) return rc;
  gemm_init(g, MMNAS_GEMM_NT, d, di, di, di, d);
  att_merge_group(op, L, &g.g[0]);
  if (fl & MMNAS_F_RESIDUAL) g.ldres = d;
  if (drop) { g.drop_p = op->drop_p; g.drop_site = 1; g.drop_seed = op->seed; }
  if (norm && !defer_ln && gemm_ln_applies(&g)) return gemm_ln(&g, op->ln_a, op->ln_b, op->y, d, op->eps, (hipStream_t)stream);
  if ((rc = mmnas_gemm(&g, stream))) return rc;

  if (norm && defer_ln) { *ln_done = false; return MMNAS_OK; }
  if (norm) return mmnas_layernorm_fwd(L.z, op->ln_a, op->ln_b, op->y, (int)L.Mq, d, op->eps, stream);
  return MMNAS_OK;
}

namespace mmnas {
struct SideQueue {
  std::vector<std::function<int(hipStream_t)>> work;
  bool rel_only = false;
  int flush(hipStream_t main, hipStream_t side, hipEvent_t ev) {
    if (work.empty()) return MMNAS_OK;
    hipStream_t s = side;
    if (hipEventRecord(ev, main) != hipSuccess || hipStreamWaitEvent(side, ev, 0) != hipSuccess)
      s = main;
    for (auto& f : work) {
      const int rc = f(s);
      if (rc) return rc;
    }
    work.clear();
    return MMNAS_OK;
  }
};

static int att_bwd_impl(const mmnas_att_op* op, hipStream_t stream, SideQueue* sq, bool acc_kv = false, bool rel_defer = false, bool kv_defer = false,
                        const AuxReduce* ln_pre = nullptr) {
  const bool side = sq != nullptr && !sq->rel_only;
  const bool side_rel = sq != nullptr;
  int rc = att_check(op, "att_op_bwd");
  if (rc) return rc;
  MMNAS_REQUIRE(op->xq && op->xkv && op->Wq && op->Wk && op->Wv && op->Wm && op->save && op->ws && op->dy &&
                    op->dxq && op->dWq && op->dWk && op->dWv && op->dWm,
                MMNAS_E_ARG, "att_op_bwd: null pointer");
  const int fl = op->flags;
  const bool norm = fl & MMNAS_F_NORM, rel = fl & MMNAS_F_REL, self = fl & MMNAS_F_SELF;
  const bool drop = drops(op);
  if (!self) MMNAS_REQUIRE(op->dxkv, MMNAS_E_ARG, "att_op_bwd: dxkv required unless SELF");
  if (norm) MMNAS_REQUIRE(op->ln_a && op->dln_a && op->dln_b, MMNAS_E_ARG, "att_op_bwd: NORM gradients missing");
  if (rel) MMNAS_REQUIRE(op->rel && op->Wr && op->br && op->dWr && op->dbr, MMNAS_E_ARG, "att_op_bwd: REL gradients missing");
  AttLayout L = att_layout(op);
  const int d = op->d, di = op->di, Mq = (int)L.Mq, Mk = (int)L.Mk;

  if (!ln_pre && !sq && op->xq == op->xkv && att_ln_place(op).bwd) {
    float* const dt_out = drop ? L.dt : (norm ? L.dz : nullptr);
    if ((rc = sa_small_bwd(op, L.Q, L.K, L.V, L.stats, L.z, dt_out, L.dQ, L.dK, L.dV, norm ? L.lnws : nullptr, stream))) return rc;
    mmnas_gemm_desc w4;
    gemm_init(w4, MMNAS_GEMM_TN, d, Mq, d, d, d);
    w4.ngroups = 4;
    w4.g[0].M = d; w4.g[0].A[0] = dt_out ? dt_out : op->dy; w4.g[0].B[0] = L.att; w4.g[0].C = op->dWm;
    w4.g[1].M = d; w4.g[1].A[0] = L.dQ; w4.g[1].B[0] = op->xq; w4.g[1].C = op->dWq;
    w4.g[2].M = d; w4.g[2].A[0] = L.dK; w4.g[2].B[0] = op->xq; w4.g[2].C = op->dWk;
    w4.g[3].M = d; w4.g[3].A[0] = L.dV; w4.g[3].B[0] = op->xq; w4.g[3].C = op->dWv;
    w4.accumulate = 1;
    AuxReduce red;
    red.part = norm ? L.lnws : nullptr; red.nrows = op->B; red.d = d;
    red.out[0] = op->dln_a; red.out[1] = op->dln_b; red.out[2] = nullptr;
    return gemm_wgrad_aux(&w4, &red, stream);
  }

  const float* dz = op->dy;
  const float* dt = op->dy;
  AuxReduce lnred;
  lnred.part = nullptr;
  if (norm && ln_pre) {
    lnred = *ln_pre;
    dz = L.dz; dt = drop ? L.dt : L.dz;
  } else if (norm) {
    if ((rc = layernorm_bwd_deferred(L.z, op->ln_a, op->dy, L.dz, op->dln_a, op->dln_b, drop ? L.dt : nullptr, nullptr,
                                     L.lnws, drop ? op->drop_p : 0.f, op->seed, 1, Mq, d, op->eps, (hipStream_t)stream, &lnred)))
      return rc;
    dz = L.dz; dt = drop ? L.dt : L.dz;
  } else if (drop) {
    if ((rc = mmnas_drop_add(op->dy, nullptr, L.dt, (size_t)Mq * d, op->drop_p, op->seed, 1, stream))) return rc;
    dt = L.dt;
  }

  mmnas_gemm_desc g, w, wm, w2;
  gemm_init(g, MMNAS_GEMM_NN, di, d, d, di, di);
  g.g[0].M = Mq; g.g[0].A[0] = dt; g.g[0].B[0] = op->Wm; g.g[0].C = L.datt;
  gemm_init(wm, MMNAS_GEMM_TN, di, Mq, d, di, di);
  wm.g[0].M = d; wm.g[0].A[0] = dt; wm.g[0].B[0] = L.att; wm.g[0].C = op->dWm;
  wm.accumulate = 1;
  if (side) { if ((rc = mmnas_gemm(&g, stream))) return rc; }
  else if ((rc = gemm_pair_aux(&g, &wm, &lnred, (hipStream_t)stream))) return rc;

  mmnas_mha_desc m;
  att_core_desc(op, L, &m);
  m.dO = L.datt; m.dQ = L.dQ; m.dK = L.dK; m.dV = L.dV; m.dbiasT = L.dbiasT; m.delta = L.delta;
  if ((rc = mmnas_mha_core_bwd(&m, stream))) return rc;

  if (self) {
    gemm_init(w, MMNAS_GEMM_TN, d, Mq, di, d, d);
    w.ngroups = 3;
    w.g[0].M = di; w.g[0].A[0] = L.dQ; w.g[0].B[0] = op->xq;  w.g[0].C = op->dWq;
    w.g[1].M = di; w.g[1].A[0] = L.dK; w.g[1].B[0] = op->xkv; w.g[1].C = op->dWk;
    w.g[2].M = di; w.g[2].A[0] = L.dV; w.g[2].B[0] = op->xkv; w.g[2].C = op->dWv;
    w.accumulate = 1;
    gemm_init(g, MMNAS_GEMM_NN, d, di, di, d, d);
    g.nseg = 3;
    g.g[0].M = Mq; g.g[0].C = op->dxq;
    g.g[0].A[0] = L.dQ; g.g[0].B[0] = op->Wq;
    g.g[0].A[1] = L.dK; g.g[0].B[1] = op->Wk;
    g.g[0].A[2] = L.dV; g.g[0].B[2] = op->Wv;
    if (fl & MMNAS_F_RESIDUAL) { g.g[0].residual = dz; g.ldres = d; }
    if (side) {
      if ((rc = mmnas_gemm(&g, stream))) return rc;
    } else if ((rc = mmnas_gemm_pair(&g, &w, stream))) return rc;
  } else {
    gemm_init(w, MMNAS_GEMM_TN, d, Mq, di, d, d);
    w.g[0].M = di; w.g[0].A[0] = L.dQ; w.g[0].B[0] = op->xq; w.g[0].C = op->dWq;
    w.accumulate = 1;
    gemm_init(g, MMNAS_GEMM_NN, d, di, di, d, d);
    g.g[0].M = Mq; g.g[0].C = op->dxq; g.g[0].A[0] = L.dQ; g.g[0].B[0] = op->Wq;
    if (fl & MMNAS_F_RESIDUAL) { g.g[0].residual = dz; g.ldres = d; }
    if (side) {
      if ((rc = mmnas_gemm(&g, stream))) return rc;
    } else if ((rc = mmnas_gemm_pair(&g, &w, stream))) return rc;
    if (kv_defer) goto params;
    gemm_init(w2, MMNAS_GEMM_TN, d, Mk, di, d, d);
    w2.ngroups = 2;
    w2.g[0].M = di; w2.g[0].A[0] = L.dK; w2.g[0].B[0] = op->xkv; w2.g[0].C = op->dWk;
    w2.g[1].M = di; w2.g[1].A[0] = L.dV; w2.g[1].B[0] = op->xkv; w2.g[1].C = op->dWv;
    w2.accumulate = 1;
    gemm_init(g, MMNAS_GEMM_NN, d, di, di, d, d);
    g.nseg = 2;
    g.g[0].M = Mk; g.g[0].C = op->dxkv;
    g.g[0].A[0] = L.dK; g.g[0].B[0] = op->Wk;
    g.g[0].A[1] = L.dV; g.g[0].B[1] = op->Wv;
    if (acc_kv) g.accumulate = 1;
    if (side) {
      if ((rc = mmnas_gemm(&g, stream))) return rc;
    } else if ((rc = mmnas_gemm_pair(&g, &w2, stream))) return rc;
  }

params:
  if (side) {
    sq->work.push_back([lnred](hipStream_t s) { return launch_aux_reduce(lnred, s); });
    sq->work.push_back([wm](hipStream_t s) { return mmnas_gemm(&wm, s); });
    sq->work.push_back([w](hipStream_t s) { return mmnas_gemm(&w, s); });
    if (!self) sq->work.push_back([w2](hipStream_t s) { return mmnas_gemm(&w2, s); });
  }
  if (rel && rel_defer) return MMNAS_OK;
  if (rel && (fl & MMNAS_F_RELRAW)) {
    MMNAS_REQUIRE(op->Wy && op->by && op->dWy && op->dby, MMNAS_E_ARG, "att_op_bwd: RELRAW gradients missing");
    const mmnas_att_op o = *op;
    float* const dbiasT = L.dbiasT;
    float* const relws = L.relws;
    auto relb = [o, dbiasT, relws](hipStream_t s) {
      if (o.q_off)
        return mmnas_rel_fused_bwd_ragged(o.rel, o.Wy, o.by, o.Wr, o.br, dbiasT, o.dWy, o.dby, o.dWr, o.dbr, relws, o.B, o.Sq,
                                          o.C, o.R, o.H, o.q_off, o.rel_tile_off, o.rel_ntiles, s);
      return mmnas_rel_fused_bwd(o.rel, o.Wy, o.by, o.Wr, o.br, dbiasT, o.dWy, o.dby, o.dWr, o.dbr, relws, o.B, o.Sq, o.Sk,
                                 o.C, o.R, o.H, s);
    };
    if (side_rel) { sq->work.push_back(relb); return MMNAS_OK; }
    return relb(stream);
  }
  if (rel)
    return mmnas_rel_bias_bwd(op->rel, op->Wr, op->br, L.dbiasT, op->drel, op->dWr, op->dbr, 0, op->B, op->Sq,
                              op->Sk, op->R, op->H, stream);
  return MMNAS_OK;
}
}

extern "C" int mmnas_att_op_bwd(const mmnas_att_op* op, void* stream) {
  return att_bwd_impl(op, (hipStream_t)stream, nullptr);
}

namespace mmnas {

struct MlpLayout {
  float* h[3];
  float* z;
  float *dz, *dt, *dp[3], *lnws;
  size_t save_bytes, ws_bwd_bytes;
};

static MlpLayout mlp_layout(const mmnas_mlp_op* op) {
  MlpLayout L;
  const bool norm = op->flags & MMNAS_F_NORM;
  const bool drop = drops(op);
  const size_t M = (size_t)op->M;
  Carver s(op->save);
  L.h[0] = nullptr;
  for (int i = 1; i < 3; ++i) L.h[i] = (i < op->nl) ? s.take(M * op->dims[i]) : nullptr;
  L.z = norm ? s.take(M * op->dims[0]) : nullptr;
  L.save_bytes = s.off;
  size_t maxh = 4;
  for (int i = 1; i < op->nl; ++i) if ((size_t)op->dims[i] > maxh) maxh = op->dims[i];
  Carver w(op->ws);
  L.dz = norm ? w.take(M * op->dims[0]) : nullptr;
  L.dt = drop ? w.take(M * op->dims[0]) : nullptr;
  L.dp[0] = w.take(M * maxh);
  L.dp[1] = op->nl > 2 ? w.take(M * maxh) : nullptr;
  L.dp[2] = nullptr;
  L.lnws = norm ? w.take(mmnas_layernorm_bwd_ws_floats(op->M, op->dims[0])) : nullptr;
  L.ws_bwd_bytes = w.off;
  return L;
}

static int mlp_check(const mmnas_mlp_op* op, const char* who) {
  MMNAS_REQUIRE(op, MMNAS_E_ARG, "%s: null descriptor", who);
  MMNAS_REQUIRE(op->nl >= 1 && op->nl <= 3 && op->M > 0, MMNAS_E_SHAPE, "%s: nl=%d M=%d", who, op->nl, op->M);
  MMNAS_REQUIRE(op->dims[0] == op->dims[op->nl], MMNAS_E_SHAPE, "%s: in/out width differ (%d vs %d)", who,
                op->dims[0], op->dims[op->nl]);
  for (int i = 0; i <= op->nl; ++i)
    MMNAS_REQUIRE(op->dims[i] > 0 && op->dims[i] % 4 == 0, MMNAS_E_SHAPE, "%s: dims[%d]=%d", who, i, op->dims[i]);
  return MMNAS_OK;
}

}

extern "C" int mmnas_mlp_op_plan(const mmnas_mlp_op* op, mmnas_plan* plan) {
  int rc = mlp_check(op, "mlp_op_plan");
  if (rc) return rc;
  MMNAS_REQUIRE(plan, MMNAS_E_ARG, "mlp_op_plan: null plan");
  mmnas_mlp_op tmp = *op;
  tmp.save = nullptr; tmp.ws = nullptr;
  MlpLayout L = mlp_layout(&tmp);
  plan->save_bytes = L.save_bytes ? L.save_bytes : 256;
  plan->ws_fwd_bytes = 256;
  plan->ws_bwd_bytes = L.ws_bwd_bytes;
  return MMNAS_OK;
}

namespace mmnas {
static int mlp_fwd_impl(const mmnas_mlp_op* op, void* stream, bool defer_ln, bool* ln_done);
}
extern "C" int mmnas_mlp_op_fwd(const mmnas_mlp_op* op, void* stream) {
  bool done;
  return mmnas::mlp_fwd_impl(op, stream, false, &done);
}
static int mmnas::mlp_fwd_impl(const mmnas_mlp_op* op, void* stream, bool defer_ln, bool* ln_done) {
  *ln_done = true;
  int rc = mlp_check(op, "mlp_op_fwd");
  if (rc) return rc;
  MMNAS_REQUIRE(op->x && op->y && op->save, MMNAS_E_ARG, "mlp_op_fwd: null pointer");
  const int fl = op->flags;
  const bool norm = fl & MMNAS_F_NORM;
  const bool drop = drops(op);
  if (norm) MMNAS_REQUIRE(op->ln_a && op->ln_b, MMNAS_E_ARG, "mlp_op_fwd: NORM without ln parameters");
  MlpLayout L = mlp_layout(op);
  const int d = op->dims[0];
  if (!(norm && defer_ln) && ffn_small_applies(op)) return ffn_small_fwd(op, L.h[1], L.z, (hipStream_t)stream);
  const float* in = op->x;
  mmnas_gemm_desc g;
  for (int i = 0; i < op->nl; ++i) {
    MMNAS_REQUIRE(op->W[i], MMNAS_E_ARG, "mlp_op_fwd: W[%d] null", i);
    const bool last = i == op->nl - 1;
    gemm_init(g, MMNAS_GEMM_NT, op->dims[i + 1], op->dims[i], op->dims[i], op->dims[i], op->dims[i + 1]);
    g.g[0].M = op->M; g.g[0].A[0] = in; g.g[0].B[0] = op->W[i]; g.g[0].bias = op->b[i];
    if (drop) { g.drop_p = op->drop_p; g.drop_seed = op->seed; g.drop_site = last ? 1u : (i == 0 ? 0u : 2u); }
    if (last) {
      g.g[0].C = norm ? L.z : op->y;
      if (fl & MMNAS_F_RESIDUAL) { g.g[0].residual = op->x; g.ldres = d; }
    } else {
      g.relu = 1;
      g.g[0].C = L.h[i + 1];
    }
    if (last && norm && !defer_ln && gemm_ln_applies(&g)) return gemm_ln(&g, op->ln_a, op->ln_b, op->y, d, op->eps, (hipStream_t)stream);
    if ((rc = mmnas_gemm(&g, stream))) return rc;
    in = L.h[i + 1];
  }
  if (norm && defer_ln) { *ln_done = false; return MMNAS_OK; }
  if (norm) return mmnas_layernorm_fwd(L.z, op->ln_a, op->ln_b, op->y, op->M, d, op->eps, stream);
  return MMNAS_OK;
}

namespace mmnas {
static int mlp_bwd_impl(const mmnas_mlp_op* op, hipStream_t stream, SideQueue* sq, const AuxReduce* ln_pre = nullptr) {
  const bool side = sq != nullptr && !sq->rel_only;
  int rc = mlp_check(op, "mlp_op_bwd");
  if (rc) return rc;
  MMNAS_REQUIRE(op->x && op->save && op->ws && op->dy && op->dx, MMNAS_E_ARG, "mlp_op_bwd: null pointer");
  const int fl = op->flags;
  const bool norm = fl & MMNAS_F_NORM;
  const bool drop = drops(op);
  MlpLayout L = mlp_layout(op);
  const int d = op->dims[0], M = op->M, nl = op->nl;
  for (int i = 0; i < nl; ++i)
    MMNAS_REQUIRE(op->W[i] && op->dW[i], MMNAS_E_ARG, "mlp_op_bwd: W/dW[%d] null", i);

  const float* dz = op->dy;
  const float* dt = op->dy;
  bool last_bias_done = false;
  AuxReduce lnred;
  lnred.part = nullptr;
  if (norm) {
    MMNAS_REQUIRE(op->ln_a && op->dln_a && op->dln_b, MMNAS_E_ARG, "mlp_op_bwd: NORM gradients missing");
    float* dcol = (drop && op->db[nl - 1]) ? op->db[nl - 1] : nullptr;
    if (ln_pre) lnred = *ln_pre;
    else if ((rc = layernorm_bwd_deferred(L.z, op->ln_a, op->dy, L.dz, op->dln_a, op->dln_b, drop ? L.dt : nullptr, dcol,
                                          L.lnws, drop ? op->drop_p : 0.f, op->seed, 1, M, d, op->eps, (hipStream_t)stream, &lnred)))
      return rc;
    dz = L.dz; dt = drop ? L.dt : L.dz;
    last_bias_done = dcol != nullptr;
  } else if (drop) {
    if ((rc = mmnas_drop_add(op->dy, nullptr, L.dt, (size_t)M * d, op->drop_p, op->seed, 1, stream))) return rc;
    dt = L.dt;
  }

  const float gate_scale = drop ? 1.0f / (1.0f - op->drop_p) : 1.0f;
  const float* dpre = dt;
  mmnas_gemm_desc g;
  mmnas_gemm_desc wd[3];
  const bool last_colsum = op->db[nl - 1] && !last_bias_done;
  if (last_colsum && !side)
    if ((rc = mmnas_colsum(dpre, op->db[nl - 1], M, op->dims[nl], op->dims[nl], stream))) return rc;
  for (int i = nl - 1; i >= 0; --i) {
    const float* hin = i == 0 ? op->x : L.h[i];
    const int nout = op->dims[i + 1], nin = op->dims[i];
    mmnas_gemm_desc& w = wd[i];
    gemm_init(w, MMNAS_GEMM_TN, nin, M, nout, nin, nin);
    w.g[0].M = nout; w.g[0].A[0] = dpre; w.g[0].B[0] = hin; w.g[0].C = op->dW[i];
    w.accumulate = 1;
    gemm_init(g, MMNAS_GEMM_NN, nin, nout, nout, nin, nin);
    g.g[0].M = M; g.g[0].A[0] = dpre; g.g[0].B[0] = op->W[i];
    if (i == 0) {
      g.g[0].C = op->dx;
      if (fl & MMNAS_F_RESIDUAL) { g.g[0].residual = dz; g.ldres = d; }
    } else {
      float* out = L.dp[(nl - 1 - i) % 3];
      g.g[0].C = out;
      g.g[0].gate = L.h[i]; g.ldgate = nin; g.gate_scale = gate_scale;
      g.g[0].colsum = op->db[i - 1];
    }
    if (side) {
      if ((rc = mmnas_gemm(&g, stream))) return rc;
    } else if ((rc = gemm_pair_aux(&g, &w, i == nl - 1 ? &lnred : nullptr, (hipStream_t)stream))) return rc;
    if (i > 0) dpre = g.g[0].C;
  }
  if (side) {
    sq->work.push_back([lnred](hipStream_t s) { return launch_aux_reduce(lnred, s); });
    if (last_colsum) {
      float* const db = op->db[nl - 1];
      const int n = op->dims[nl];
      sq->work.push_back([dt, db, M, n](hipStream_t s) { return mmnas_colsum(dt, db, M, n, n, s); });
    }
    for (int i = nl - 1; i >= 0; --i) {
      const mmnas_gemm_desc w = wd[i];
      sq->work.push_back([w](hipStream_t s) { return mmnas_gemm(&w, s); });
    }
  }
  return MMNAS_OK;
}
}

extern "C" int mmnas_mlp_op_bwd(const mmnas_mlp_op* op, void* stream) {
  return mlp_bwd_impl(op, (hipStream_t)stream, nullptr);
}

#include <map>
#include <mutex>
#include <utility>
namespace mmnas {

struct ChainLayout {
  size_t y[MMNAS_CHAIN_MAX_OPS], save[MMNAS_CHAIN_MAX_OPS], ws[MMNAS_CHAIN_MAX_OPS], dx[MMNAS_CHAIN_MAX_OPS],
      tmp[MMNAS_CHAIN_MAX_OPS];
  size_t dpre, encdy, relws, total;
  int last_x, last_y, first_x, first_y, n_guided;
  int src[MMNAS_CHAIN_MAX_OPS], head[MMNAS_CHAIN_MAX_OPS];
  size_t nout[MMNAS_CHAIN_MAX_OPS], ndact[MMNAS_CHAIN_MAX_OPS], mixws;
};

static int chain_check(const mmnas_chain* c, const char* who) {
  MMNAS_REQUIRE(c && c->ops, MMNAS_E_ARG, "%s: null chain", who);
  MMNAS_REQUIRE(c->n_ops >= 1 && c->n_ops <= MMNAS_CHAIN_MAX_OPS, MMNAS_E_SHAPE, "%s: %d operators (1..%d)", who, c->n_ops, MMNAS_CHAIN_MAX_OPS);
  MMNAS_REQUIRE(c->B > 0 && c->Sx > 0 && c->Sy > 0 && c->d > 0, MMNAS_E_SHAPE, "%s: B=%d Sx=%d Sy=%d d=%d", who, c->B, c->Sx, c->Sy, c->d);
  if (c->y_off) MMNAS_REQUIRE(c->Ny > 0 && c->Ny <= c->B * c->Sy && c->Sy <= 128 && !c->use_side_stream, MMNAS_E_ARG,
                              "%s: ragged decoder stream: Ny=%d of B*Sy=%d rows, Sy=%d <= 128, single stream", who, c->Ny, c->B * c->Sy, c->Sy);
  bool seen_y = false;
  for (int i = 0; i < c->n_ops; ++i) {
    const mmnas_chain_op& o = c->ops[i];
    MMNAS_REQUIRE(o.kind == MMNAS_CHAIN_ATT || o.kind == MMNAS_CHAIN_MLP, MMNAS_E_ARG, "%s: operator %d: kind %d", who, i, o.kind);
    if (o.on_y) seen_y = true;
    else MMNAS_REQUIRE(!seen_y, MMNAS_E_ARG, "%s: encoder operators must precede the decoder's (operator %d)", who, i);
    if (o.kind == MMNAS_CHAIN_ATT && !(o.att.flags & MMNAS_F_SELF))
      MMNAS_REQUIRE(o.on_y, MMNAS_E_ARG, "%s: operator %d: guided attention needs the decoder stream", who, i);
  }
  if (c->mixed) {
    MMNAS_REQUIRE(c->gate && c->gate_width >= 1 && c->gate_width <= MMNAS_MIXED_MAX, MMNAS_E_ARG, "%s: mixed chain without a gate block (width %d)", who, c->gate_width);
    MMNAS_REQUIRE(!c->use_side_stream, MMNAS_E_ARG, "%s: mixed chains run on one stream", who);
    MMNAS_REQUIRE(c->d <= 1024, MMNAS_E_SHAPE, "%s: mixed chains need d <= 1024", who);
    int node = -1, live = 0, count = 0;
    for (int i = 0; i < c->n_ops; ++i) {
      const mmnas_chain_op& o = c->ops[i];
      if (o.node != node) {
        MMNAS_REQUIRE(o.node == node + 1, MMNAS_E_ARG, "%s: operator %d: node %d after node %d", who, i, o.node, node);
        MMNAS_REQUIRE(node < 0 || live == 1, MMNAS_E_ARG, "%s: node %d has %d differentiated candidates (exactly one)", who, node, live);
        node = o.node; live = 0; count = 0;
      } else {
        MMNAS_REQUIRE(o.on_y == c->ops[i - 1].on_y, MMNAS_E_ARG, "%s: node %d mixes the two streams", who, node);
      }
      MMNAS_REQUIRE(o.cand >= 0 && o.cand < c->gate_width, MMNAS_E_ARG, "%s: operator %d: candidate %d outside the gate row", who, i, o.cand);
      MMNAS_REQUIRE(++count <= MMNAS_MIXED_MAX, MMNAS_E_SHAPE, "%s: node %d has more than %d candidates", who, node, MMNAS_MIXED_MAX);
      live += o.detached ? 0 : 1;
    }
    MMNAS_REQUIRE(live == 1, MMNAS_E_ARG, "%s: node %d has %d differentiated candidates (exactly one)", who, node, live);
  }
  return MMNAS_OK;
}

static inline size_t chain_rows_y(const mmnas_chain* c) { return c->y_off ? (size_t)c->Ny : (size_t)c->B * c->Sy; }

static void chain_op_shapes(const mmnas_chain* c, int i, mmnas_att_op& a, mmnas_mlp_op& m) {
  const mmnas_chain_op& o = c->ops[i];
  const int S = o.on_y ? c->Sy : c->Sx;
  if (o.kind == MMNAS_CHAIN_ATT) {
    a = o.att;
    a.B = c->B; a.d = c->d; a.Sq = S;
    const bool self = a.flags & MMNAS_F_SELF;
    a.Sk = self ? S : c->Sx;
    const uint8_t* mask = (self && o.on_y) ? c->y_mask : c->x_mask;
    a.q_off = a.k_off = nullptr; a.Mq = a.Mk = 0; a.rel_tile_off = nullptr; a.rel_ntiles = 0;
    if (o.on_y && c->y_off) {
      a.q_off = c->y_off; a.Mq = c->Ny;
      if (self) { a.k_off = c->y_off; a.Mk = c->Ny; mask = nullptr; a.rel_tile_off = c->y_tile_off; a.rel_ntiles = c->y_ntiles; }
    }
    a.mask = mask;
    if (mask) a.flags |= MMNAS_F_MASK; else a.flags &= ~MMNAS_F_MASK;
    if (a.flags & MMNAS_F_REL) a.rel = o.on_y ? c->y_rel : c->x_rel;
  } else {
    m = o.mlp;
    m.M = (o.on_y && c->y_off) ? c->Ny : c->B * S;
  }
}

static int chain_layout(const mmnas_chain* c, ChainLayout& L) {
  size_t off = 0;
  auto take = [&](size_t bytes) { size_t r = off; off += al(bytes); return r; };
  L.last_x = L.last_y = L.first_x = L.first_y = -1;
  L.n_guided = 0;
  int cur[2] = {-1, -1}, head = 0;
  for (int i = 0; i < c->n_ops; ++i) {
    if (i > 0 && (!c->mixed || c->ops[i].node != c->ops[i - 1].node)) { cur[c->ops[head].on_y ? 1 : 0] = head; head = i; }
    L.head[i] = head; L.src[i] = cur[c->ops[i].on_y ? 1 : 0];
    if (head != i) continue;
    if (c->ops[i].on_y) { if (L.first_y < 0) L.first_y = i; L.last_y = i; }
    else { if (L.first_x < 0) L.first_x = i; L.last_x = i; }
  }
  const size_t nx = (size_t)c->B * c->Sx * c->d * sizeof(float), ny = chain_rows_y(c) * c->d * sizeof(float);
  for (int i = 0; i < c->n_ops; ++i) {
    const mmnas_chain_op& o = c->ops[i];
    mmnas_att_op a; mmnas_mlp_op m;
    chain_op_shapes(c, i, a, m);
    mmnas_plan pl;
    int rc = o.kind == MMNAS_CHAIN_ATT ? mmnas_att_op_plan(&a, &pl) : mmnas_mlp_op_plan(&m, &pl);
    if (rc) return rc;
    const size_t n = o.on_y ? ny : nx;
    L.y[i] = take(n);
    L.save[i] = take(pl.save_bytes);
    L.ws[i] = take(pl.ws_bwd_bytes);
    L.dx[i] = take(n);
    const bool guided = o.kind == MMNAS_CHAIN_ATT && !(a.flags & MMNAS_F_SELF) && !(c->mixed && o.detached);
    L.tmp[i] = guided ? take(nx) : 0;
    L.n_guided += guided;
  }
  L.dpre = take(nx);
  L.encdy = take(nx);
  L.relws = take(mmnas_rel_multi_bwd_ws_floats(c->B, c->Sx > c->Sy ? c->Sx : c->Sy) * sizeof(float));
  L.mixws = 0;
  if (c->mixed) {
    int nodes = 0;
    for (int i = 0; i < c->n_ops; ++i) {
      const bool first = L.head[i] == i;
      L.nout[i] = first ? take(c->ops[i].on_y ? ny : nx) : 0;
      L.ndact[i] = first ? take(c->ops[i].on_y ? ny : nx) : 0;
      nodes += first;
    }
    L.mixws = take((size_t)(nodes > 0 ? nodes : 1) * mmnas_mixed_sum_ws_floats() * sizeof(float));
  }
  L.total = off;
  return MMNAS_OK;
}

struct BoundOp {
  int i;
  bool att;
  mmnas_att_op a; mmnas_mlp_op m;
  AttLayout al; MlpLayout ml;
  float* y;
  int flags() const { return att ? a.flags : m.flags; }
  float eps() const { return att ? a.eps : m.eps; }
};
static inline float* chain_buf(const mmnas_chain* c, size_t off) { return (float*)((char*)c->arena + off); }
static void chain_bind(const mmnas_chain* c, const ChainLayout& L, int i, BoundOp& b, bool layouts = false) {
  b.i = i; b.att = c->ops[i].kind == MMNAS_CHAIN_ATT;
  chain_op_shapes(c, i, b.a, b.m);
  b.y = chain_buf(c, L.y[i]);
  if (b.att) { b.a.save = chain_buf(c, L.save[i]); b.a.ws = chain_buf(c, L.ws[i]); if (layouts) b.al = att_layout(&b.a); }
  else { b.m.save = chain_buf(c, L.save[i]); b.m.ws = chain_buf(c, L.ws[i]); if (layouts) b.ml = mlp_layout(&b.m); }
}
static float* chain_out(const mmnas_chain* c, const ChainLayout& L, int i) {
  return i == L.last_x ? c->x_out : (i == L.last_y ? c->y_out : chain_buf(c, c->mixed ? L.nout[i] : L.y[i]));
}
static const float* chain_in(const mmnas_chain* c, const ChainLayout& L, int i) {
  return L.src[i] >= 0 ? chain_out(c, L, L.src[i]) : (c->ops[i].on_y ? c->y_in : c->x_in);
}
static const float* chain_x_final(const mmnas_chain* c, const ChainLayout& L) { return L.last_x >= 0 ? c->x_out : c->x_in; }
static float* chain_din(const mmnas_chain* c, const ChainLayout& L, int i) {
  return L.head[i] == L.first_x ? c->dx_in : (L.head[i] == L.first_y ? c->dy_in : chain_buf(c, L.dx[i]));
}
static float* chain_guided_tmp(const mmnas_chain* c, const ChainLayout& L, int i) { return chain_buf(c, L.tmp[i]); }
static float* chain_node_dact(const mmnas_chain* c, const ChainLayout& L, int i0) { return chain_buf(c, L.ndact[i0]); }
static float* chain_gate_ws(const mmnas_chain* c, const ChainLayout& L, int k) { return chain_buf(c, L.mixws) + (size_t)k * mmnas_mixed_sum_ws_floats(); }
static void chain_bind_fwd(BoundOp& b, const mmnas_chain* c, const ChainLayout& L, float* out) {
  const float* in = chain_in(c, L, b.i);
  if (b.att) { b.a.xq = in; b.a.xkv = (b.a.flags & MMNAS_F_SELF) ? in : chain_x_final(c, L); b.a.y = out; }
  else { b.m.x = in; b.m.y = out; }
}
static float* chain_bind_bwd(BoundOp& b, const mmnas_chain* c, const ChainLayout& L, const float* dy) {
  const float* in = chain_in(c, L, b.i);
  float* dx = chain_din(c, L, b.i);
  if (b.att) {
    const bool self = b.a.flags & MMNAS_F_SELF;
    b.a.xq = in; b.a.xkv = self ? in : chain_x_final(c, L);
    b.a.dy = dy; b.a.dxq = dx;
    b.a.dxkv = self ? nullptr : chain_buf(c, L.dpre);
    b.a.drel = nullptr;
  } else { b.m.x = in; b.m.dy = dy; b.m.dx = dx; }
  return dx;
}
static int chain_run_fwd(const BoundOp& b, hipStream_t s, bool defer_ln, bool* ln_done, bool rel_ready, bool kv_ready) {
  return b.att ? att_fwd_impl(&b.a, s, defer_ln, ln_done, rel_ready, kv_ready) : mlp_fwd_impl(&b.m, s, defer_ln, ln_done);
}
static int chain_run_bwd(const BoundOp& b, hipStream_t s, SideQueue* sq, bool rel_defer, bool kv_defer, const AuxReduce* ln_pre = nullptr) {
  return b.att ? att_bwd_impl(&b.a, s, sq, !(b.a.flags & MMNAS_F_SELF), rel_defer, kv_defer, ln_pre) : mlp_bwd_impl(&b.m, s, sq, ln_pre);
}
static LnPlace chain_cand_view(const BoundOp& b, const float** z, const float** la, const float** lb) {
  LnPlace p = {false, false};
  if (b.att) p = att_ln_place(&b.a);
  if (!(b.flags() & MMNAS_F_NORM) || p.fwd) { *z = b.y; *la = nullptr; *lb = nullptr; }
  else if (b.att) { *z = b.al.z; *la = b.a.ln_a; *lb = b.a.ln_b; }
  else { *z = b.ml.z; *la = b.m.ln_a; *lb = b.m.ln_b; }
  return p;
}

struct SideCtx { hipStream_t side; hipStream_t enc; hipEvent_t ev[MMNAS_CHAIN_MAX_OPS + 2]; hipEvent_t ovl[4]; bool used; };
static std::mutex g_side_mu;
static std::map<std::pair<int, hipStream_t>, SideCtx> g_side;

static SideCtx* side_ctx(hipStream_t main, bool create) {
  int dev = 0;
  if (hipGetDevice(&dev) != hipSuccess) return nullptr;
  std::lock_guard<std::mutex> lk(g_side_mu);
  auto key = std::make_pair(dev, main);
  auto it = g_side.find(key);
  if (it == g_side.end()) {
    if (!create) return nullptr;
    SideCtx s;
    memset(&s, 0, sizeof(s));
    int least = 0, greatest = 0;
    const bool prio = sw::side_prio.get() &&
                      hipDeviceGetStreamPriorityRange(&least, &greatest) == hipSuccess && least != greatest;
    if ((prio ? hipStreamCreateWithPriority(&s.side, hipStreamNonBlocking, least)
              : hipStreamCreateWithFlags(&s.side, hipStreamNonBlocking)) != hipSuccess) return nullptr;
    for (auto& e : s.ev)
      if (hipEventCreateWithFlags(&e, hipEventDisableTiming) != hipSuccess) return nullptr;
    if ((prio ? hipStreamCreateWithPriority(&s.enc, hipStreamNonBlocking, greatest)
              : hipStreamCreateWithFlags(&s.enc, hipStreamNonBlocking)) != hipSuccess) return nullptr;
    for (auto& e : s.ovl)
      if (hipEventCreateWithFlags(&e, hipEventDisableTiming) != hipSuccess) return nullptr;
    it = g_side.emplace(key, s).first;
  }
  return &it->second;
}

static bool chain_overlap_on() { return sw::chain_overlap.get() != 0; }
static bool head_overlap_on() { return sw::head_overlap.get() != 0; }
static bool head_glimpse1_on() { return sw::head_glimpse1.get() != 0; }
static bool head_projT_on() { return sw::head_projt.get() != 0; }
static int first_guided(const mmnas_chain* c) {
  for (int i = 0; i < c->n_ops; ++i)
    if (c->ops[i].kind == MMNAS_CHAIN_ATT && !(c->ops[i].att.flags & MMNAS_F_SELF)) return i;
  return c->n_ops;
}
static int ev_fork(hipStream_t from, hipStream_t to, hipEvent_t e) {
  if (hipEventRecord(e, from) != hipSuccess || hipStreamWaitEvent(to, e, 0) != hipSuccess) {
    set_error("chain: event record / wait failed");
    return MMNAS_E_LAUNCH;
  }
  return MMNAS_OK;
}


static bool rel_hoist_on() { return sw::rel_hoist.get() != 0; }
struct RelGroups {
  std::vector<mmnas_rel_multi> groups[2];
  bool hoisted[MMNAS_CHAIN_MAX_OPS];
  RelGroups() { memset(hoisted, 0, sizeof(hoisted)); }
};
static void chain_rel_groups(const mmnas_chain* c, const ChainLayout& L, bool bwd, RelGroups& G) {
  if (!rel_hoist_on() || c->use_side_stream) return;
  for (int i = 0; i < c->n_ops; ++i) {
    const mmnas_chain_op& o = c->ops[i];
    if (o.kind != MMNAS_CHAIN_ATT) continue;
    if (bwd && c->mixed && o.detached) continue;
    if (!(o.att.flags & MMNAS_F_REL) || !(o.att.flags & MMNAS_F_RELRAW) || !(o.att.flags & MMNAS_F_SELF)) continue;
    BoundOp b;
    chain_bind(c, L, i, b, true);
    const mmnas_att_op& a = b.a;
    const AttLayout& al_ = b.al;
    if (!mmnas_rel_multi_supported(a.C, a.R, a.H) || !a.rel || !a.Wy || !a.by) continue;
    if ((long)a.B * a.H * a.Sq * a.Sq >= (1l << 31)) continue;
    std::vector<mmnas_rel_multi>& gs = G.groups[o.on_y ? 1 : 0];
    mmnas_rel_multi* g = nullptr;
    const unsigned char* const kmask = (a.flags & MMNAS_F_MASK) ? (const unsigned char*)a.mask : nullptr;
    for (auto& q : gs)
      if (q.raw == a.rel && q.Wy == a.Wy && q.by == a.by && q.H == a.H && q.C == a.C && q.key_mask == kmask && q.n_ops < MMNAS_REL_MULTI_MAX) { g = &q; break; }
    if (!g) {
      mmnas_rel_multi q;
      memset(&q, 0, sizeof(q));
      q.B = a.B; q.S = a.Sq; q.C = a.C; q.R = a.R; q.H = a.H;
      q.raw = a.rel; q.Wy = a.Wy; q.by = a.by; q.dWy = a.dWy; q.dby = a.dby;
      q.off = a.q_off; q.tile_off = a.rel_tile_off; q.ntiles = a.rel_ntiles;
      q.key_mask = kmask;
      q.ws = chain_buf(c, L.relws);
      gs.push_back(q);
      g = &gs.back();
    }
    const int j = g->n_ops++;
    g->Wr[j] = a.Wr; g->br[j] = a.br; g->biasT[j] = al_.biasT; g->dbiasT[j] = al_.dbiasT; g->dWr[j] = a.dWr; g->dbr[j] = a.dbr;
    G.hoisted[i] = true;
  }
}
static int chain_rel_fwd(const RelGroups& G, hipStream_t st, int only = -1) {
  for (int s = 0; s < 2; ++s)
    if (only < 0 || only == s)
      for (const auto& g : G.groups[s]) { const int rc = mmnas_rel_multi_fwd(&g, st); if (rc) return rc; }
  return MMNAS_OK;
}
static bool rel_overlap_on() { return sw::rel_overlap.get() != 0; }
static int chain_rel_bwd(const RelGroups& G, int stream_y, hipStream_t st) {
  for (const auto& g : G.groups[stream_y]) {
    MMNAS_REQUIRE(g.dWy && g.dby, MMNAS_E_ARG, "chain_bwd: relation operators without the stem layer's gradient sinks");
    const int rc = mmnas_rel_multi_bwd(&g, st);
    if (rc) return rc;
  }
  return MMNAS_OK;
}


static bool node_lnb_on() { return sw::node_lnb.get() != 0; }
static bool guided_hoist_on() { return sw::guided_hoist.get() != 0; }
struct GuidedSet {
  int idx[MMNAS_CHAIN_MAX_OPS], n;
  bool hoisted[MMNAS_CHAIN_MAX_OPS];
  GuidedSet() : n(0) { memset(hoisted, 0, sizeof(hoisted)); }
};
constexpr int GUIDED_PER_LAUNCH = 4;
static void chain_guided_set(const mmnas_chain* c, bool bwd, bool allow, GuidedSet& G) {
  if (!allow || !guided_hoist_on() || c->use_side_stream) return;
  int di = -1;
  for (int i = 0; i < c->n_ops; ++i) {
    const mmnas_chain_op& o = c->ops[i];
    if (o.kind != MMNAS_CHAIN_ATT || (o.att.flags & MMNAS_F_SELF)) continue;
    if (bwd && c->mixed && o.detached) continue;
    if (di < 0) di = o.att.di;
    if (o.att.di != di || G.n >= ADD_MANY_MAX - 2) continue;
    G.idx[G.n++] = i; G.hoisted[i] = true;
  }
  if (G.n < 2) { for (int j = 0; j < G.n; ++j) G.hoisted[G.idx[j]] = false; G.n = 0; }
}
static int chain_guided_kv_fwd(const mmnas_chain* c, const ChainLayout& L, const GuidedSet& G, hipStream_t st) {
  const float* x_final = chain_x_final(c, L);
  for (int j0 = 0; j0 < G.n; j0 += GUIDED_PER_LAUNCH) {
    const int n = G.n - j0 < GUIDED_PER_LAUNCH ? G.n - j0 : GUIDED_PER_LAUNCH;
    mmnas_gemm_desc g;
    for (int j = 0; j < n; ++j) {
      const int i = G.idx[j0 + j];
      BoundOp b;
      chain_bind(c, L, i, b, true);
      const mmnas_att_op& a = b.a;
      const AttLayout& al_ = b.al;
      if (j == 0) { gemm_init(g, MMNAS_GEMM_NT, a.di, c->d, c->d, c->d, a.di); g.ngroups = 2 * n; }
      mmnas_gemm_group* gg = g.g + 2 * j;
      memset(gg, 0, 2 * sizeof(*gg));
      gg[0].M = (int)al_.Mk; gg[0].A[0] = x_final; gg[0].B[0] = a.Wk; gg[0].C = al_.K;
      gg[1].M = (int)al_.Mk; gg[1].A[0] = x_final; gg[1].B[0] = a.Wv; gg[1].C = al_.V;
    }
    const int rc = mmnas_gemm(&g, st);
    if (rc) return rc;
  }
  return MMNAS_OK;
}
static int chain_guided_kv_bwd(const mmnas_chain* c, const ChainLayout& L, const GuidedSet& G, const float* extra, const float* extra2,
                               float* out, hipStream_t st) {
  const float* x_final = chain_x_final(c, L);
  const float* srcs[ADD_MANY_MAX + 2];
  int ns = 0;
  if (extra) srcs[ns++] = extra;
  if (extra2) srcs[ns++] = extra2;
  for (int j0 = 0; j0 < G.n; j0 += GUIDED_PER_LAUNCH) {
    const int n = G.n - j0 < GUIDED_PER_LAUNCH ? G.n - j0 : GUIDED_PER_LAUNCH;
    mmnas_gemm_desc g, w;
    for (int j = 0; j < n; ++j) {
      const int i = G.idx[j0 + j];
      BoundOp b;
      chain_bind(c, L, i, b, true);
      const mmnas_att_op& a = b.a;
      const AttLayout& al_ = b.al;
      const int Mk = (int)al_.Mk, di = a.di, d = c->d;
      if (j == 0) {
        gemm_init(g, MMNAS_GEMM_NN, d, di, di, d, d); g.ngroups = n; g.nseg = 2;
        gemm_init(w, MMNAS_GEMM_TN, d, Mk, di, d, d); w.ngroups = 2 * n; w.accumulate = 1;
      }
      float* tmp = chain_guided_tmp(c, L, i);
      memset(&g.g[j], 0, sizeof(g.g[j]));
      g.g[j].M = Mk; g.g[j].C = tmp;
      g.g[j].A[0] = al_.dK; g.g[j].B[0] = a.Wk;
      g.g[j].A[1] = al_.dV; g.g[j].B[1] = a.Wv;
      memset(&w.g[2 * j], 0, 2 * sizeof(w.g[0]));
      w.g[2 * j].M = di; w.g[2 * j].A[0] = al_.dK; w.g[2 * j].B[0] = x_final; w.g[2 * j].C = a.dWk;
      w.g[2 * j + 1].M = di; w.g[2 * j + 1].A[0] = al_.dV; w.g[2 * j + 1].B[0] = x_final; w.g[2 * j + 1].C = a.dWv;
      srcs[ns++] = tmp;
    }
    const int rc = mmnas_gemm_pair(&g, &w, st);
    if (rc) return rc;
  }
  return add_many(srcs, ns, out, (size_t)c->B * c->Sx * c->d, st);
}

}

extern "C" int mmnas_set_rel_overlap(int on) { return mmnas::sw::rel_overlap.set(on != 0); }
extern "C" int mmnas_set_guided_hoist(int on) { return mmnas::sw::guided_hoist.set(on != 0); }
extern "C" int mmnas_set_rel_hoist(int on) { return mmnas::sw::rel_hoist.set(on != 0); }
extern "C" int mmnas_set_chain_overlap(int on) { return mmnas::sw::chain_overlap.set(on != 0); }

extern "C" int mmnas_chain_plan(const mmnas_chain* c, size_t* arena_bytes) {
  int rc = chain_check(c, "chain_plan");
  if (rc) return rc;
  MMNAS_REQUIRE(arena_bytes, MMNAS_E_ARG, "chain_plan: null output");
  ChainLayout L;
  if ((rc = chain_layout(c, L))) return rc;
  *arena_bytes = L.total;
  return MMNAS_OK;
}

namespace mmnas {
static int chain_rel_prologue(const mmnas_chain* c, const ChainLayout& L, const RelGroups& RG, hipStream_t st, bool may_fork, SideCtx** forked) {
  SideCtx* rsc = (may_fork && rel_overlap_on() && !RG.groups[1].empty() && L.last_x >= 0 && L.first_y >= 0) ? side_ctx(st, true) : nullptr;
  *forked = rsc;
  if (!rsc) return chain_rel_fwd(RG, st);
  int rc;
  if ((rc = ev_fork(st, rsc->side, rsc->ovl[0]))) return rc;
  if ((rc = chain_rel_fwd(RG, rsc->side, 1))) return rc;
  return chain_rel_fwd(RG, st, 0);
}
static int chain_rel_join(SideCtx* rsc, hipStream_t st) { return ev_fork(rsc->side, st, rsc->ovl[1]); }
static int chain_fwd_passthrough(const mmnas_chain* c, const ChainLayout& L, hipStream_t st) {
  const size_t nx = (size_t)c->B * c->Sx * c->d * sizeof(float), ny = chain_rows_y(c) * c->d * sizeof(float);
  if (L.last_x < 0 && hipMemcpyAsync(c->x_out, c->x_in, nx, hipMemcpyDeviceToDevice, st) != hipSuccess) return MMNAS_E_LAUNCH;
  if (L.last_y < 0 && hipMemcpyAsync(c->y_out, c->y_in, ny, hipMemcpyDeviceToDevice, st) != hipSuccess) return MMNAS_E_LAUNCH;
  return MMNAS_OK;
}

struct ChainBwd {
  const mmnas_chain* c; const ChainLayout* L;
  hipStream_t st;
  SideQueue* sq;
  RelGroups RG;
  GuidedSet GS;
  int G;
  float *dpre, *encdy;
  size_t ex;
  const float* enc_grad = nullptr;
  SideCtx* rel_bwd_side = nullptr;
};
static int chain_bwd_begin(ChainBwd& S, const mmnas_chain* c, const ChainLayout& L, hipStream_t st, SideQueue* sq, bool hoist) {
  S.c = c; S.L = &L; S.st = st; S.sq = sq;
  S.dpre = chain_buf(c, L.dpre); S.encdy = chain_buf(c, L.encdy);
  S.ex = (size_t)c->B * c->Sx * c->d;
  if (hoist) chain_rel_groups(c, L, true, S.RG);
  chain_guided_set(c, true, hoist, S.GS);
  S.G = -1;
  for (int i = 0; i < c->n_ops && S.G < 0; ++i)
    if (S.GS.hoisted[i]) S.G = i;
  if (L.n_guided > S.GS.n && hipMemsetAsync(S.dpre, 0, S.ex * sizeof(float), st) != hipSuccess) return MMNAS_E_LAUNCH;
  return MMNAS_OK;
}
static int chain_enc_dy(ChainBwd& S, hipStream_t s, const float** out) {
  const mmnas_chain* c = S.c;
  MMNAS_REQUIRE(c->dx_out || S.L->n_guided, MMNAS_E_ARG, "chain_bwd: no gradient reaches the encoder (dx_out NULL, no guided operator)");
  if (S.enc_grad) { *out = S.enc_grad; return MMNAS_OK; }
  if (c->dx_out && S.L->n_guided) {
    const int r = mmnas_drop_add(c->dx_out, S.dpre, S.encdy, S.ex, 0.f, 0, 0, s);
    if (r) return r;
    *out = S.encdy;
  } else *out = c->dx_out ? c->dx_out : S.dpre;
  return MMNAS_OK;
}
static int chain_guided_release(ChainBwd& S, int i, hipStream_t s) {
  if (!S.GS.n || i != S.G) return MMNAS_OK;
  const int r = chain_guided_kv_bwd(S.c, *S.L, S.GS, S.c->dx_out, S.GS.n < S.L->n_guided ? S.dpre : nullptr, S.encdy, s);
  if (!r) S.enc_grad = S.encdy;
  return r;
}
static int chain_first_done(ChainBwd& S, int i, int mark, hipStream_t s) {
  const mmnas_chain* c = S.c; const ChainLayout& L = *S.L;
  int r;
  hipStream_t mark_stream = s;
  if (i == L.first_y && !S.RG.groups[1].empty()) {
    SideCtx* rsc = (rel_overlap_on() && L.last_x >= 0 && !S.sq) ? side_ctx(S.st, true) : nullptr;
    if (rsc) {
      if ((r = ev_fork(s, rsc->side, rsc->ovl[2]))) return r;
      if ((r = chain_rel_bwd(S.RG, 1, rsc->side))) return r;
      S.rel_bwd_side = rsc;
      mark_stream = rsc->side;
    } else if ((r = chain_rel_bwd(S.RG, 1, s))) return r;
  }
  if (i == L.first_x && !S.RG.groups[0].empty()) {
    if (S.rel_bwd_side) { if ((r = ev_fork(S.rel_bwd_side->side, s, S.rel_bwd_side->ovl[3]))) return r; S.rel_bwd_side = nullptr; }
    if ((r = chain_rel_bwd(S.RG, 0, s))) return r;
  }
  if (mark >= 0 && c->marks && c->marks[mark] && hipEventRecord((hipEvent_t)c->marks[mark], mark_stream) != hipSuccess) {
    set_error("chain_bwd: cannot record the mark event of operator %d", mark);
    return MMNAS_E_LAUNCH;
  }
  return MMNAS_OK;
}
struct GateReds {
  const float* part[MMNAS_CHAIN_MAX_OPS]; float* out[MMNAS_CHAIN_MAX_OPS]; int nwg[MMNAS_CHAIN_MAX_OPS], width[MMNAS_CHAIN_MAX_OPS];
  int n = 0;
};
static int chain_bwd_close(ChainBwd& S, const GateReds* reds) {
  const mmnas_chain* c = S.c; const ChainLayout& L = *S.L;
  hipStream_t st = S.st;
  int rc;
  if (S.rel_bwd_side && (rc = ev_fork(S.rel_bwd_side->side, st, S.rel_bwd_side->ovl[3]))) return rc;
  if (reds && reds->n && (rc = mixed_reduce_many(reds->part, reds->out, reds->nwg, reds->width, reds->n, st))) return rc;
  if (L.first_y < 0 && hipMemcpyAsync(c->dy_in, c->dy_out, chain_rows_y(c) * c->d * sizeof(float), hipMemcpyDeviceToDevice, st) != hipSuccess)
    return MMNAS_E_LAUNCH;
  if (L.first_x < 0) {
    const float* g0 = c->dx_out;
    if (S.enc_grad) g0 = S.enc_grad;
    else if (c->dx_out && L.n_guided) {
      if ((rc = mmnas_drop_add(c->dx_out, S.dpre, c->dx_in, S.ex, 0.f, 0, 0, st))) return rc;
      g0 = nullptr;
    } else if (!c->dx_out) g0 = S.dpre;
    if (g0 && hipMemcpyAsync(c->dx_in, g0, S.ex * sizeof(float), hipMemcpyDeviceToDevice, st) != hipSuccess) return MMNAS_E_LAUNCH;
  }
  return MMNAS_OK;
}

static int chain_fwd_mixed(const mmnas_chain* c, hipStream_t st, const ChainLayout& L) {
  int rc;
  RelGroups RG;
  chain_rel_groups(c, L, false, RG);
  SideCtx* rsc = nullptr;
  if ((rc = chain_rel_prologue(c, L, RG, st, true, &rsc))) return rc;
  for (int i0 = 0; i0 < c->n_ops;) {
    int i1 = i0;
    while (i1 < c->n_ops && c->ops[i1].node == c->ops[i0].node) ++i1;
    if (rsc && i0 == L.first_y && (rc = chain_rel_join(rsc, st))) return rc;
    BoundOp cand[MMNAS_MIXED_MAX];
    for (int i = i0; i < i1; ++i) {
      chain_bind(c, L, i, cand[i - i0], true);
      chain_bind_fwd(cand[i - i0], c, L, cand[i - i0].y);
    }
    const BoundOp* g[MMNAS_MIXED_MAX];
    int ng = 0;
    for (int i = i0; i < i1; ++i) {
      const BoundOp& b = cand[i - i0];
      if (!b.att || att_ln_place(&b.a).fwd) continue;
      if (ng > 0) {
        const mmnas_att_op& f = g[0]->a;
        const bool d0 = drops(&f), d1 = drops(&b.a);
        if (b.a.di != f.di || ((b.a.flags ^ f.flags) & MMNAS_F_RESIDUAL) || d0 != d1 || (d0 && b.a.drop_p != f.drop_p)) continue;
      }
      if (3 * (ng + 1) > MMNAS_GEMM_MAX_GROUPS) continue;
      if ((rc = att_fwd_args(&b.a))) return rc;
      g[ng++] = &b;
    }
    if (ng < 2) ng = 0;
    if (ng) {
      const mmnas_att_op& f = g[0]->a;
      mmnas_gemm_desc gd;
      gemm_init(gd, MMNAS_GEMM_NT, f.di, c->d, c->d, c->d, f.di);
      gd.ngroups = 3 * ng;
      for (int j = 0; j < ng; ++j) att_qkv_groups(&g[j]->a, g[j]->al, gd.g + 3 * j);
      if ((rc = mmnas_gemm(&gd, st))) return rc;
      {
        mmnas_mha_desc md[MMNAS_MIXED_MAX];
        for (int j = 0; j < ng; ++j)
          if ((rc = att_core_fwd(&g[j]->a, g[j]->al, st, &md[j], RG.hoisted[g[j]->i]))) return rc;
        bool done[MMNAS_MIXED_MAX] = {false};
        for (int j = 0; j < ng; ++j) {
          if (done[j]) continue;
          int mate = -1;
          for (int q = j + 1; q < ng && mate < 0; ++q)
            if (!done[q] && md[q].Sq == md[j].Sq && md[q].Sk == md[j].Sk && md[q].H == md[j].H && md[q].dh == md[j].dh) mate = q;
          if (mate >= 0) { if ((rc = mha_core_fwd_pair(&md[j], &md[mate], st))) return rc; done[mate] = true; }
          else if ((rc = mmnas_mha_core_fwd(&md[j], st))) return rc;
          done[j] = true;
        }
      }
      gemm_init(gd, MMNAS_GEMM_NT, c->d, f.di, f.di, f.di, c->d);
      gd.ngroups = ng;
      for (int j = 0; j < ng; ++j) att_merge_group(&g[j]->a, g[j]->al, &gd.g[j]);
      if (f.flags & MMNAS_F_RESIDUAL) gd.ldres = c->d;
      if (drops(&f)) { gd.drop_p = f.drop_p; gd.drop_site = 1; gd.drop_seed = f.seed; }
      if ((rc = mmnas_gemm(&gd, st))) return rc;
    }
    const float* zs[MMNAS_MIXED_MAX] = {nullptr}; const float* as[MMNAS_MIXED_MAX] = {nullptr}; const float* bs[MMNAS_MIXED_MAX] = {nullptr};
    int width = 0;
    float eps = 1e-6f;
    for (int i = i0; i < i1; ++i) {
      const BoundOp& b = cand[i - i0];
      bool staged = false;
      for (int j = 0; j < ng; ++j) staged |= g[j] == &b;
      bool ln_done;
      if (!staged && (rc = chain_run_fwd(b, st, true, &ln_done, RG.hoisted[i], false))) return rc;
      if (b.flags() & MMNAS_F_NORM) eps = b.eps();
      const int k = c->ops[i].cand;
      chain_cand_view(b, &zs[k], &as[k], &bs[k]);
      if (k + 1 > width) width = k + 1;
    }
    const int M = c->ops[i0].on_y ? (int)chain_rows_y(c) : c->B * c->Sx;
    if ((rc = mmnas_node_mix_fwd(zs, as, bs, width, c->gate + (size_t)c->ops[i0].node * c->gate_width, chain_out(c, L, i0), M, c->d, eps, st))) return rc;
    i0 = i1;
  }
  return chain_fwd_passthrough(c, L, st);
}

static int chain_bwd_mixed(const mmnas_chain* c, hipStream_t st, const ChainLayout& L) {
  MMNAS_REQUIRE(c->dgate, MMNAS_E_ARG, "chain_bwd: mixed chain without a gate-gradient block");
  int rc;
  ChainBwd S;
  if ((rc = chain_bwd_begin(S, c, L, st, nullptr, true))) return rc;
  GateReds reds;
  int starts[MMNAS_CHAIN_MAX_OPS + 1], nn = 0;
  for (int i = 0; i < c->n_ops; ++i)
    if (L.head[i] == i) starts[nn++] = i;
  starts[nn] = c->n_ops;
  const float* cur_dy = c->dy_out;
  for (int k = nn - 1; k >= 0; --k) {
    const int i0 = starts[k], i1 = starts[k + 1];
    if (i0 == L.last_x && (rc = chain_enc_dy(S, st, &cur_dy))) return rc;
    BoundOp cand[MMNAS_MIXED_MAX];
    const float* zs[MMNAS_MIXED_MAX] = {nullptr}; const float* as[MMNAS_MIXED_MAX] = {nullptr}; const float* bs[MMNAS_MIXED_MAX] = {nullptr};
    int width = 0, act = -1, act_op = -1;
    LnPlace act_ln = {false, false};
    float eps = 1e-6f;
    for (int i = i0; i < i1; ++i) {
      BoundOp& b = cand[i - i0];
      chain_bind(c, L, i, b, true);
      const int kc = c->ops[i].cand;
      const LnPlace p = chain_cand_view(b, &zs[kc], &as[kc], &bs[kc]);
      if (kc + 1 > width) width = kc + 1;
      if (!c->ops[i].detached) { act = kc; act_op = i; act_ln = p; }
      if (b.flags() & MMNAS_F_NORM) eps = b.eps();
    }
    float* dact = chain_node_dact(c, L, i0);
    const int M = c->ops[i0].on_y ? (int)chain_rows_y(c) : c->B * c->Sx;
    const size_t grow = (size_t)c->ops[i0].node * c->gate_width;
    BoundOp& b = cand[act_op - i0];
    float* dx = chain_bind_bwd(b, c, L, dact);
    NodeLnBwd lnb;
    lnb.dz = nullptr;
    AuxReduce lnpre;
    lnpre.part = nullptr;
    if (node_lnb_on() && c->d <= 256 && as[act] && !act_ln.bwd) {
      const bool drop = b.att ? drops(&b.a) : drops(&b.m);
      lnb.dz = b.att ? b.al.dz : b.ml.dz; lnb.dt = !drop ? nullptr : (b.att ? b.al.dt : b.ml.dt); lnb.part = b.att ? b.al.lnws : b.ml.lnws;
      lnb.drop = make_drop(drop ? (b.att ? b.a.drop_p : b.m.drop_p) : 0.f, b.att ? b.a.seed : b.m.seed, 1);
      lnpre.part = lnb.part; lnpre.d = c->d;
      lnpre.out[0] = b.att ? b.a.dln_a : b.m.dln_a; lnpre.out[1] = b.att ? b.a.dln_b : b.m.dln_b;
      lnpre.out[2] = (!b.att && drop && b.m.db[b.m.nl - 1]) ? b.m.db[b.m.nl - 1] : nullptr;
    }
    {
      float* wsk = chain_gate_ws(c, L, k);
      int nwg = 0;
      if ((rc = node_mix_bwd_impl(zs, as, bs, width, c->gate + grow, cur_dy, dact, act, c->dgate + grow, wsk, M, c->d, eps, st, false, &nwg,
                                  lnb.dz ? &lnb : nullptr)))
        return rc;
      if (nwg > 0) { reds.part[reds.n] = wsk; reds.out[reds.n] = c->dgate + grow; reds.nwg[reds.n] = nwg; reds.width[reds.n] = width; ++reds.n; }
      lnpre.nrows = nwg;
    }
    if ((rc = chain_run_bwd(b, st, nullptr, S.RG.hoisted[act_op], S.GS.hoisted[act_op], lnb.dz ? &lnpre : nullptr))) return rc;
    if ((rc = chain_guided_release(S, act_op, st))) return rc;
    cur_dy = dx;
    if ((rc = chain_first_done(S, i0, act_op, st))) return rc;
  }
  return chain_bwd_close(S, &reds);
}
}

extern "C" int mmnas_chain_fwd(const mmnas_chain* c, void* stream) {
  int rc = chain_check(c, "chain_fwd");
  if (rc) return rc;
  MMNAS_REQUIRE(c->x_in && c->y_in && c->x_out && c->y_out && c->arena, MMNAS_E_ARG, "chain_fwd: null pointer");
  hipStream_t st = (hipStream_t)stream;
  ChainLayout L;
  if ((rc = chain_layout(c, L))) return rc;
  if (c->mixed) return chain_fwd_mixed(c, st, L);
  RelGroups RG;
  chain_rel_groups(c, L, false, RG);
  const int G = first_guided(c);
  const bool ovl = chain_overlap_on() && !c->use_side_stream && L.last_x >= 0 && L.first_y >= 0 && G > L.first_y;
  SideCtx* rsc = nullptr;
  if ((rc = chain_rel_prologue(c, L, RG, st, !ovl, &rsc))) return rc;
  int rel_join_at = -1;
  for (int i = L.first_y; rsc && i < c->n_ops && rel_join_at < 0; ++i)
    if (RG.hoisted[i] && c->ops[i].on_y) rel_join_at = i;
  GuidedSet GS;
  chain_guided_set(c, false, !ovl, GS);
  auto run = [&](int i, hipStream_t s) -> int {
    BoundOp b;
    chain_bind(c, L, i, b);
    chain_bind_fwd(b, c, L, chain_out(c, L, i));
    bool done;
    return chain_run_fwd(b, s, false, &done, RG.hoisted[i], GS.hoisted[i]);
  };
  if (!ovl) {
    for (int i = 0; i < c->n_ops; ++i) {
      if (GS.n && i == G && (rc = chain_guided_kv_fwd(c, L, GS, st))) return rc;
      if (i == rel_join_at && (rc = chain_rel_join(rsc, st))) return rc;
      if ((rc = run(i, st))) return rc;
    }
  } else {
    SideCtx* sc = side_ctx(st, true);
    MMNAS_REQUIRE(sc, MMNAS_E_LAUNCH, "chain_fwd: cannot create the encoder stream");
    if ((rc = ev_fork(st, sc->enc, sc->ovl[0]))) return rc;
    int ie = L.first_x, id = L.first_y;
    while (ie <= L.last_x || id < G) {
      if (ie <= L.last_x && (rc = run(ie++, sc->enc))) return rc;
      if (id < G && (rc = run(id++, st))) return rc;
    }
    if ((rc = ev_fork(sc->enc, st, sc->ovl[1]))) return rc;
    for (int i = G; i < c->n_ops; ++i)
      if ((rc = run(i, st))) return rc;
  }
  return chain_fwd_passthrough(c, L, st);
}

extern "C" int mmnas_chain_bwd(const mmnas_chain* c, void* stream) {
  int rc = chain_check(c, "chain_bwd");
  if (rc) return rc;
  MMNAS_REQUIRE(c->x_in && c->y_in && c->x_out && c->y_out && c->arena && c->dy_out && c->dx_in && c->dy_in, MMNAS_E_ARG,
                "chain_bwd: null pointer");
  hipStream_t st = (hipStream_t)stream;
  ChainLayout L;
  if ((rc = chain_layout(c, L))) return rc;
  if (c->mixed) return chain_bwd_mixed(c, st, L);
  SideCtx* sc = c->use_side_stream ? side_ctx(st, true) : nullptr;
  MMNAS_REQUIRE(!c->use_side_stream || sc, MMNAS_E_LAUNCH, "chain_bwd: cannot create the side stream");
  hipStream_t side = sc ? sc->side : nullptr;
  if (sc) sc->used = true;
  SideQueue q;
  q.rel_only = c->use_side_stream == 2;
  SideQueue* sq = sc ? &q : nullptr;
  static const bool per_op = sw::side_flush.get() && !strcmp(getenv(sw::side_flush.name), "op");
  const int G = first_guided(c);
  const bool ovl = chain_overlap_on() && !c->use_side_stream && L.last_x >= 0 && L.first_y >= 0 && G > L.first_y;
  ChainBwd S;
  if ((rc = chain_bwd_begin(S, c, L, st, sq, !ovl))) return rc;
  auto run = [&](int i, hipStream_t s, const float* dyi, const float** dxo) -> int {
    BoundOp b;
    chain_bind(c, L, i, b);
    float* dx = chain_bind_bwd(b, c, L, dyi);
    int r;
    if ((r = chain_run_bwd(b, s, sq, S.RG.hoisted[i], S.GS.hoisted[i]))) return r;
    if ((r = chain_guided_release(S, i, s))) return r;
    *dxo = dx;
    return chain_first_done(S, i, ovl ? -1 : i, s);
  };
  const float* cur_dy = c->dy_out;
  if (!ovl) {
    for (int i = c->n_ops - 1; i >= 0; --i) {
      if (sq && i == L.last_x && (rc = q.flush(st, side, sc->ev[0]))) return rc;
      if (i == L.last_x && (rc = chain_enc_dy(S, st, &cur_dy))) return rc;
      if ((rc = run(i, st, cur_dy, &cur_dy))) return rc;
      if (sq && per_op && (rc = q.flush(st, side, sc->ev[i + 1]))) return rc;
    }
    if (sq && (rc = q.flush(st, side, sc->ev[1]))) return rc;
  } else {
    SideCtx* oc = side_ctx(st, true);
    MMNAS_REQUIRE(oc, MMNAS_E_LAUNCH, "chain_bwd: cannot create the encoder stream");
    for (int i = c->n_ops - 1; i >= G; --i)
      if ((rc = run(i, st, cur_dy, &cur_dy))) return rc;
    if ((rc = ev_fork(st, oc->enc, oc->ovl[2]))) return rc;
    const float* enc_dy = nullptr;
    if ((rc = chain_enc_dy(S, oc->enc, &enc_dy))) return rc;
    int ie = L.last_x, id = G - 1;
    while (ie >= L.first_x || id >= L.first_y) {
      if (ie >= L.first_x && (rc = run(ie--, oc->enc, enc_dy, &enc_dy))) return rc;
      if (id >= L.first_y && (rc = run(id--, st, cur_dy, &cur_dy))) return rc;
    }
    if ((rc = ev_fork(oc->enc, st, oc->ovl[3]))) return rc;
    if (c->marks)
      for (int i = 0; i < c->n_ops; ++i)
        if (c->marks[i] && hipEventRecord((hipEvent_t)c->marks[i], st) != hipSuccess) {
          set_error("chain_bwd: cannot record the mark event of operator %d", i);
          return MMNAS_E_LAUNCH;
        }
  }
  return chain_bwd_close(S, nullptr);
}

extern "C" int mmnas_chain_join(void* main_stream, void* waiting_stream) {
  SideCtx* sc = side_ctx((hipStream_t)main_stream, false);
  if (!sc || !sc->used) return MMNAS_OK;
  hipEvent_t e = sc->ev[MMNAS_CHAIN_MAX_OPS];
  if (hipEventRecord(e, sc->side) != hipSuccess || hipStreamWaitEvent((hipStream_t)waiting_stream, e, 0) != hipSuccess) {
    set_error("chain_join: event record / wait failed");
    return MMNAS_E_LAUNCH;
  }
  return MMNAS_OK;
}

namespace mmnas {

struct HeadSideLayout { float *h, *logit, *probs, *pooled, *dpooled, *dlog, *dh, *dxpool, *g1part; };
static inline int head_rows(const mmnas_head* hd, const mmnas_attflat_side& sd) { return sd.off ? sd.M : hd->B * sd.S; }
struct HeadLayout {
  HeadSideLayout s[2];
  float *xo, *sum, *xy, *dxy, *dsum, *lnws, *g1proj, *dlogT;
  size_t total;
};

static HeadLayout head_layout(const mmnas_head* hd) {
  HeadLayout L;
  Carver c(hd->arena);
  const size_t B = hd->B;
  for (int k = 0; k < 2; ++k) {
    const mmnas_attflat_side& sd = k ? hd->sy : hd->sx;
    const size_t M = sd.off ? (size_t)sd.M : B * sd.S;
    HeadSideLayout& s = L.s[k];
    s.h = c.take(M * hd->MID); s.logit = c.take(M * hd->G); s.probs = c.take(M * hd->G); s.pooled = c.take(B * hd->G * hd->d);
    s.dpooled = c.take(B * hd->G * hd->d); s.dlog = c.take(M * hd->G); s.dh = c.take(M * hd->MID); s.dxpool = c.take(M * hd->d);
    s.g1part = (hd->G == 1 && glimpse1_supported(hd->MID)) ? c.take((size_t)glimpse1_bwd_blocks((long)M, hd->MID) * 3 * hd->MID) : nullptr;
  }
  L.xo = c.take(B * hd->OUT); L.sum = c.take(B * hd->OUT); L.xy = c.take(B * hd->OUT);
  L.dxy = c.take(B * hd->OUT); L.dsum = c.take(B * hd->OUT);
  L.lnws = c.take(mmnas_layernorm_bwd_ws_floats(hd->B, hd->OUT));
  L.g1proj = (hd->ANS == 1 && glimpse1_supported(hd->OUT)) ? c.take((size_t)glimpse1_bwd_blocks((long)B, hd->OUT) * 3 * hd->OUT) : nullptr;
  L.dlogT = (hd->ANS % 4 != 0 && hd->B % 4 == 0 && hd->ANS > 1) ? c.take((size_t)hd->ANS * B) : nullptr;
  L.total = c.off;
  return L;
}

static int head_check(const mmnas_head* hd, const char* who) {
  MMNAS_REQUIRE(hd, MMNAS_E_ARG, "%s: null descriptor", who);
  MMNAS_REQUIRE(hd->B > 0 && hd->d > 0 && hd->MID > 0 && hd->G > 0 && hd->OUT > 0 && hd->ANS > 0 && hd->sx.S > 0 && hd->sy.S > 0,
                MMNAS_E_SHAPE, "%s: B=%d d=%d MID=%d G=%d OUT=%d ANS=%d Sx=%d Sy=%d", who, hd->B, hd->d, hd->MID, hd->G, hd->OUT,
                hd->ANS, hd->sx.S, hd->sy.S);
  MMNAS_REQUIRE(hd->d % 4 == 0 && hd->MID % 4 == 0 && hd->OUT % 4 == 0, MMNAS_E_SHAPE, "%s: d, MID, OUT must be multiples of 4", who);
  for (int k = 0; k < 2; ++k) {
    const mmnas_attflat_side& sd = k ? hd->sy : hd->sx;
    if (sd.off) MMNAS_REQUIRE(sd.M > 0 && sd.M <= hd->B * sd.S, MMNAS_E_ARG, "%s: packed side %d: M=%d of B*S=%d rows", who, k, sd.M, hd->B * sd.S);
  }
  return MMNAS_OK;
}

}

extern "C" int mmnas_head_plan(const mmnas_head* hd, size_t* arena_bytes) {
  int rc = head_check(hd, "head_plan");
  if (rc) return rc;
  MMNAS_REQUIRE(arena_bytes, MMNAS_E_ARG, "head_plan: null output");
  mmnas_head tmp = *hd;
  tmp.arena = nullptr;
  *arena_bytes = head_layout(&tmp).total;
  return MMNAS_OK;
}

extern "C" int mmnas_head_fwd(const mmnas_head* hd, void* stream) {
  int rc = head_check(hd, "head_fwd");
  if (rc) return rc;
  MMNAS_REQUIRE(hd->arena && hd->logits && hd->ln_a && hd->ln_b && hd->Wp, MMNAS_E_ARG, "head_fwd: null pointer");
  HeadLayout L = head_layout(hd);
  const bool drop = drops(hd);
  const int B = hd->B, d = hd->d, MID = hd->MID, G = hd->G, OUT = hd->OUT;
  mmnas_gemm_desc g;
  hipStream_t st = (hipStream_t)stream;
  SideCtx* oc = head_overlap_on() ? side_ctx(st, true) : nullptr;
  if (oc && (rc = ev_fork(st, oc->enc, oc->ovl[0]))) return rc;
  const mmnas_attflat_side* sides[2] = {&hd->sx, &hd->sy};
  for (int k = 0; k < 2; ++k)
    MMNAS_REQUIRE(sides[k]->x && sides[k]->W1 && sides[k]->W2 && sides[k]->Wm, MMNAS_E_ARG, "head_fwd: side %d null pointer", k);
  auto side_stream = [&](int k) -> void* { return (oc && k == 0) ? (void*)oc->enc : stream; };
  if (!oc) {
    gemm_init(g, MMNAS_GEMM_NT, MID, d, d, d, MID);
    g.ngroups = 2; g.relu = 1;
    if (drop) { g.drop_p = hd->drop_p; g.drop_seed = sides[0]->seed; g.drop_site = 0; }
    for (int k = 0; k < 2; ++k) {
      const mmnas_attflat_side& sd = *sides[k];
      g.g[k].M = head_rows(hd, sd); g.g[k].A[0] = sd.x; g.g[k].B[0] = sd.W1; g.g[k].bias = sd.b1; g.g[k].C = L.s[k].h;
      if (drop) g.g[k].drop_seed = sd.seed;
    }
    if ((rc = mmnas_gemm(&g, stream))) return rc;
  }
  for (int k = 0; k < 2 && oc; ++k) {
    const mmnas_attflat_side& sd = *sides[k];
    gemm_init(g, MMNAS_GEMM_NT, MID, d, d, d, MID);
    g.g[0].M = head_rows(hd, sd); g.g[0].A[0] = sd.x; g.g[0].B[0] = sd.W1; g.g[0].bias = sd.b1; g.g[0].C = L.s[k].h; g.relu = 1;
    if (drop) { g.drop_p = hd->drop_p; g.drop_seed = sd.seed; g.drop_site = 0; }
    if ((rc = mmnas_gemm(&g, side_stream(k)))) return rc;
  }
  const bool g1 = G == 1 && !oc && glimpse1_supported(MID) && head_glimpse1_on();
  if (g1) {
    if ((rc = glimpse1_fwd(L.s[0].h, hd->sx.W2, hd->sx.b2, L.s[0].logit, (long)head_rows(hd, hd->sx), L.s[1].h, hd->sy.W2, hd->sy.b2,
                           L.s[1].logit, (long)head_rows(hd, hd->sy), MID, st)))
      return rc;
  }
  gemm_init(g, MMNAS_GEMM_NT, G, MID, MID, MID, G);
  for (int k = 0; k < 2 && !g1; ++k) {
    const mmnas_attflat_side& sd = *sides[k];
    mmnas_gemm_group& gg = g.g[oc ? 0 : k];
    gg.M = head_rows(hd, sd); gg.A[0] = L.s[k].h; gg.B[0] = sd.W2; gg.bias = sd.b2; gg.C = L.s[k].logit;
    if (oc && (rc = mmnas_gemm(&g, side_stream(k)))) return rc;
  }
// ... 99 lines not shown
```

mmnas_amd/csrc/switches.h:

```cpp
#pragma once

namespace mmnas {

int env_int(const char* name, int dflt);

enum SwKind { sw_int, sw_bool, sw_exact1, sw_presence, sw_string };
enum SwPolicy { sw_once, sw_every_call, sw_reload };

struct Switch {
  const char* name;
  int dflt;
  SwKind kind;
  SwPolicy policy;
  const char* help;
  int value;
  int state;

  int get() { return state ? value : read(); }
  int read();
  int reload();
  int set(int v);
  int peek(int* source) const;
};

#define MMNAS_SWITCHES(X) \
   \
  X(chain_overlap, "MMNAS_CHAIN_OVERLAP", 0, bool, once, "language stream beside the leading image-stream operators (mmnas_set_chain_overlap); measured: no gain, DESIGN.md section 5") \
  X(head_overlap, "MMNAS_HEAD_OVERLAP", 0, bool, once, "the answer head's two AttFlat sides on two streams") \
  X(head_glimpse1, "MMNAS_HEAD_GLIMPSE1", 1, bool, every_call, "0: the head's one-glimpse logit layer as GEMM launches (A/B, tests); ops.py reads it too") \
  X(head_projt, "MMNAS_HEAD_PROJT", 1, bool, every_call, "0: the answer projection's gradients from the untransposed loss gradient") \
  X(rel_hoist, "MMNAS_REL_HOIST", 1, bool, once, "relation bias of all lazy-handle operators of a stream in one launch per direction (mmnas_set_rel_hoist); 0: one fused launch per operator (supernet step 4.54 -> 5.00 ms)") \
  X(rel_overlap, "MMNAS_REL_OVERLAP", 0, bool, once, "the image stream's relation launches on a second stream (mmnas_set_rel_overlap); measured slower, +2.5 % on the supernet step") \
  X(node_lnb, "MMNAS_NODE_LNB", 1, bool, once, "architecture step: the sampled candidate's LayerNorm backward inside the node's mix kernel (7.81 -> 7.72 ms, profiles/r06_node_lnb_ab.txt); 0: its own launch") \
  X(guided_hoist, "MMNAS_GUIDED_HOIST", 1, bool, once, "key / value projections of a chain's guided operators as grouped launches (mmnas_set_guided_hoist)") \
  X(rel_fwd_valu, "MMNAS_REL_FWD_VALU", 0, exact1, every_call, "1: a lone RelSelfAtt computes its bias with the per-operator fused kernel instead of the one-operator multi kernel (A/B)") \
  X(side_prio, "MMNAS_SIDE_PRIO", 1, bool, every_call, "0: the chains' extra streams without stream priorities (read when a stream pair is created)") \
  X(side_flush, "MMNAS_SIDE_FLUSH", 0, string, once, "op: side-stream parameter-gradient work released behind every operator instead of once per phase") \
   \
  X(small_ops, "MMNAS_SMALL_OPS", 1, bool, once, "SelfAtt of <= 16 rows as one launch forward (mmnas_set_small_ops); 0: the general path") \
  X(small_bwd, "MMNAS_SMALL_BWD", 1, bool, once, "the same operators' backward as two launches (mmnas_set_small_bwd)") \
  X(small_ffn, "MMNAS_SMALL_FFN", 0, int, once, "FeedForward forward as one launch (mmnas_set_small_ffn): 1 four slices of 256 hidden units, 2 eight of 128; measured neutral (profiles/r05_small_ffn_ab.txt)") \
   \
  X(gemm_ln, "MMNAS_GEMM_LN", 0, exact1, once, "1: the merge / last FFN product and its LayerNorm as one row-panel launch (mmnas_set_gemm_ln); measured neutral, profiles/r06_ab.txt") \
  X(gemm_ln_minm, "MMNAS_GEMM_LN_MINM", 2048, int, once, "fewest rows for the row-panel kernel (read together with MMNAS_GEMM_LN)") \
  X(gemm_ln_maxk, "MMNAS_GEMM_LN_MAXK", 256, int, once, "largest K for the row-panel kernel (read together with MMNAS_GEMM_LN)") \
   \
  X(mha_nw, "MMNAS_MHA_NW", 4, int, every_call, "2: attention cores never use 4-wave workgroups (4-wave groups measured 7-15 % faster)") \
  X(mha_pair, "MMNAS_MHA_PAIR", 1, bool, once, "0: two attention cores of one geometry as two launches (mixed chain)") \
  X(mha_bwd_fused, "MMNAS_MHA_BWD_FUSED", 1, bool, once, "0: the attention backward as separate dQ and dK / dV kernels (dense rows only)") \
  X(mha_fwd_b16, "MMNAS_MHA_FWD_B16", 1, bool, once, "0: attention forward (d_h = 64, 65..128 keys) on the fp32 MFMA kernels instead of split-bf16 operands (profiles/r06_attention_b16_ab.txt)") \
  X(mha_fwd_b16_two, "MMNAS_MHA_FWD_B16_TWO", 320, int, once, "more than this many (sample, head) pairs: the split-bf16 forward runs two per workgroup") \
  X(mha_bwd_b16, "MMNAS_MHA_BWD_B16", 1, bool, once, "0: attention backward (d_h = 64, 65..128 keys) on the fp32 MFMA kernels instead of split-bf16 operands (supernet step -1.6 % with both)") \
   \
  X(rel_multi_dbg, "MMNAS_REL_MULTI_DBG", 0, int, once, "timing experiments of a -DMMNAS_DBG_REL=1 build only (wrong results): 1 no stores, 2 no raw reloads, 4 no head-projection MFMAs") \
  X(rel_multi_wgs, "MMNAS_REL_MULTI_WGS", 3, int, once, "workgroups per CU of the multi-operator relation forward (tuning)") \
  X(rel_multi_yield, "MMNAS_REL_MULTI_YIELD", 0, int, once, "1 | 3: the multi-operator relation kernels' yield variants (tuning)") \
  X(rel_keylimit, "MMNAS_REL_KEYLIMIT", 1, int, once, "multi-operator relation kernels of a padded batch walk only the elements under keys up to each sample's last unmasked one (mmnas_set_rel_keylimit); 0: all B S^2 elements") \
  X(rel_bwd_valu, "MMNAS_REL_BWD_VALU", 1, bool, once, "0: the fused relation backward as the all-MFMA kernel (A/B)") \
   \
  X(gemm_tile, "MMNAS_GEMM_TILE", 0, int, reload, "64 | 128: force the tile shape") \
  X(gemm_generic, "MMNAS_GEMM_GENERIC", 0, presence, reload, "set (to anything): force the guarded-load path; ops.py reads it too") \
  X(gemm_sk, "MMNAS_GEMM_SK", 1, int, reload, "stream-K / split-K: 0 never, 1 automatic, 2 always") \
  X(gemm_wgs, "MMNAS_GEMM_WGS", 0, int, reload, "co-resident workgroup budget (0: 1024 for 64^2 tiles, 512 for 128^2)") \
  X(gemm_min_units, "MMNAS_GEMM_MIN_UNITS", 4, int, reload, "fewest K-tiles a workgroup is given (at least 1)") \
  X(gemm_gm, "MMNAS_GEMM_GM", 0, int, reload, "row-panels per tile-order block (0: 8)") \
  X(gemm_xcd, "MMNAS_GEMM_XCD", 1, int, reload, "0: identity workgroup mapping") \
  X(gemm_split, "MMNAS_GEMM_SPLIT", 6, int, reload, "products as 6 / 3 / 1 bf16 MFMA products of split operands (6: fp32-grade; 3, 1: reduced precision), 0: fp32 MFMA") \
  X(gemm_pair, "MMNAS_GEMM_PAIR", 1, int, reload, "0: mmnas_gemm_pair launches its two products separately") \
  X(gemm_split_slots, "MMNAS_GEMM_SPLIT_SLOTS", 0, int, reload, "split-K pieces wanted over all tiles (0: from SPLIT_P and SPLIT_MINWG)") \
  X(gemm_split_p, "MMNAS_GEMM_SPLIT_P", 24, int, reload, "K-tiles per split-K piece (at least 1)") \
  X(gemm_split_minwg, "MMNAS_GEMM_SPLIT_MINWG", 256, int, reload, "fewest split-K pieces in total when pieces of SPLIT_P would be fewer") \
  X(gemm_pf, "MMNAS_GEMM_PF", 2, int, reload, "1 | 2: K-tiles of operand loads in flight ahead of the MFMA block (64^2 fp32 path)") \
  X(gemm_hyb_t, "MMNAS_GEMM_HYB_T", 16, int, reload, "fewest K-tiles per output tile for the whole-tiles + streamed-tail hybrid") \
  X(gemm_wide_min, "MMNAS_GEMM_WIDE_MIN", 200, int, reload, "fewest 128x64 tiles for that shape to be chosen") \
  X(gemm_lean, "MMNAS_GEMM_LEAN", 3, int, reload, "lean kernels: bit 0 NT / NN products, bit 1 split-K TN products") \
  X(gemm_lean_maxb, "MMNAS_GEMM_LEAN_MAXB", 8 << 20, int, reload, "largest B matrix (bytes) the lean tile order is used for") \
  X(lstm_fwd_p, "MMNAS_LSTM_FWD_P", 0, int, every_call, "K-tiles per workgroup of the LSTM forward step's stream-K product (0: whole tiles; read per time step)") \
  X(lstm_bwd_p, "MMNAS_LSTM_BWD_P", 8, int, every_call, "K-tiles per workgroup of the LSTM backward step's stream-K product (0: whole tiles; read per time step)") \
   \
  X(prof_dump, "MMNAS_PROF_DUMP", 0, string, every_call, "file: mmnas_prof_collect appends one kind,tag,ms,flops,bytes row per bracketed launch (tools/prof_shapes.py)")

namespace sw {
#define MMNAS_SW_DECLARE(id, var, dflt, kind, policy, help) extern Switch id;
MMNAS_SWITCHES(MMNAS_SW_DECLARE)
#undef MMNAS_SW_DECLARE
}

}
```

Before: 230.9 steps/s.

## Skip dead padded rows in image-stream weight-gradient GEMMs via live K-tile table

Adds a kernel that scans the upstream gradient and the padding mask of the y-stream chain and builds a table of 32-row K-tiles that hold any nonzero gradient row. The TN weight-gradient GEMMs of that chain's attention and MLP ops take this table (a new lean level 4), so split-K slices walk only the live K-tiles and skip the padded rows' zero contributions. This spends one extra small launch per backward chain and adds per-tile lane lookups for the row offsets. It also relies on masked rows carrying exactly zero gradient.

After: 238.5 steps/s (median of 6 runs). +3.3%, better.

```diff
diff --git a/include/mmnas_hip.h b/include/mmnas_hip.h
--- a/include/mmnas_hip.h
+++ b/include/mmnas_hip.h
@@ -69,6 +69,7 @@
   uint32_t drop_site;
   uint64_t drop_seed;
   mmnas_gemm_group g[MMNAS_GEMM_MAX_GROUPS];
+  const int* ktab;
 } mmnas_gemm_desc;
 
 int mmnas_gemm(const mmnas_gemm_desc* d, void* stream);
@@ -320,6 +321,9 @@
 int mmnas_chain_bwd(const mmnas_chain* c, void* stream);
 int mmnas_chain_join(void* main_stream, void* waiting_stream);
 int mmnas_set_chain_overlap(int on);
+int mmnas_set_wgrad_live(int on);
+int mmnas_wgrad_live_table_ints(int M);
+int mmnas_wgrad_live_table(const float* dy, const unsigned char* mask, int M, int d, int* tab, void* stream);
 
 typedef struct mmnas_attflat_side {
   int S, reserved;
diff --git a/mmnas_amd/_lib.py b/mmnas_amd/_lib.py
--- a/mmnas_amd/_lib.py
+++ b/mmnas_amd/_lib.py
@@ -46,7 +46,7 @@
                 ('lda', C.c_int), ('ldb', C.c_int), ('ldc', C.c_int), ('ldres', C.c_int), ('ldgate', C.c_int),
                 ('relu', C.c_int), ('split_k', C.c_int), ('accumulate', C.c_int), ('b_planes', C.c_int), ('alpha', C.c_float), ('gate_scale', C.c_float),
                 ('drop_p', C.c_float), ('drop_site', C.c_uint32), ('drop_seed', C.c_uint64),
-                ('g', GemmGroup * GEMM_MAX_GROUPS)]
+                ('g', GemmGroup * GEMM_MAX_GROUPS), ('ktab', _fp)]
 
 
 class MhaDesc(C.Structure):
@@ -203,6 +203,9 @@
     'mmnas_rel_multi_bwd': (_i, [C.POINTER(RelMulti), _fp]),
     'mmnas_set_rel_hoist': (_i, [_i]),
     'mmnas_set_rel_keylimit': (_i, [_i]),
+    'mmnas_set_wgrad_live': (_i, [_i]),
+    'mmnas_wgrad_live_table_ints': (_i, [_i]),
+    'mmnas_wgrad_live_table': (_i, [_fp, _fp, _i, _i, _fp, _fp]),
     'mmnas_set_guided_hoist': (_i, [_i]),
     'mmnas_set_rel_overlap': (_i, [_i]),
     'mmnas_mha_core_fwd': (_i, [C.POINTER(MhaDesc), _fp]),
diff --git a/mmnas_amd/csrc/gemm.hip b/mmnas_amd/csrc/gemm.hip
--- a/mmnas_amd/csrc/gemm.hip
+++ b/mmnas_amd/csrc/gemm.hip
@@ -52,7 +52,10 @@
   float* lg_h2;
   float* lg_dc;
   const float* lg_act;
-  int lg_ldh2, lg_pad;
+  int lg_ldh2;
+  int ksl;
+  unsigned ksl_magic;
+  const int* ktab;
   GemmGroupK g[MAXG];
 };
 
@@ -143,8 +146,10 @@
   static_assert(PF == 1 || (PF == 2 && FAST && (NS == 0 || NS == 1 || NS == 3)), "the two-stage prefetch exists for the buffer-load path (fp32, bf16x1 and bf16x6)");
   static_assert(NS == 0 || (FAST && BK == 32), "the bf16-split path exists for the buffer-load path only");
   static_assert(!BDMA || (NS == 3 && AKC && BKC && FAST && PF == 1 && BM == 64 && BN == 64 && EPI == 0), "LDS-DMA weight planes: NT 64^2 bf16x6 only");
+  static_assert(LEAN >= 0 && LEAN <= 4 && (LEAN != 4 || !AKC), "lean levels 1-3; 4 = TN with the live-row table");
   static_assert(!LEAN || (NS > 0 && (AKC || !BKC) && FAST && PF == 2 && BM == 64 && BN == 64 && EPI == 0 && !BDMA), "lean form: 64^2 split-operand kernels");
   constexpr bool LEAN_TN = LEAN && !AKC;
+  constexpr bool KTAB = LEAN == 4;
   constexpr bool LEAN_EL = LEAN == 3;
   constexpr bool LEAN_SW = LEAN && AKC && !LEAN_EL;
   constexpr bool LEAN_WT = (LEAN_SW && LEAN == 1) || LEAN_EL;
@@ -193,6 +198,14 @@
   static_assert(MAXG == 9, "the list of group boundaries below names nine groups");
   asm volatile("" : "+s"(h.U), "+s"(h.gt[1]), "+s"(h.gt[2]), "+s"(h.gt[3]), "+s"(h.gt[4]), "+s"(h.gt[5]), "+s"(h.gt[6]), "+s"(h.gt[7]),
                "+s"(h.gt[8]));
+  const int* const ktab = KTAB ? p.ktab : nullptr;
+  unsigned ktab_cnt = 0, ktab_w[4] = {0, 0, 0, 0};
+  if (KTAB) {
+    const __amdgpu_buffer_rsrc_t t_rs = __builtin_amdgcn_make_buffer_rsrc((void*)ktab, 0, (unsigned)(h.T + 1) * 4u, 0x00020000);
+    ktab_cnt = __builtin_amdgcn_raw_buffer_load_b32(t_rs, 0u, 0, 0);
+#pragma unroll
+    for (int j = 0; j < 4; ++j) ktab_w[j] = __builtin_amdgcn_raw_buffer_load_b32(t_rs, (unsigned)(1 + lane + 64 * j) * 4u, 0, 0);
+  }
   int v;
   {
     const int q = nwg >> 3, r = nwg & 7, xcd = bid & 7, in = bid >> 3;
@@ -214,6 +227,8 @@
 
   while (u < uend) {
     int tile, q0, nq;
+    int ksl_i = 0;
+    static_assert(!KTAB || LEAN_TN, "the table walk deals K-tiles over split-K slices: KTAB kernels are LEAN_TN, whose mode is MODE_SPLIT by construction");
     if (mode == MODE_TILE || whole >= 0) {
       tile = whole >= 0 ? whole : v; q0 = 0; nq = h.T;
       u = uend;
@@ -222,8 +237,9 @@
       tile = v - sl * h.ntiles;
       q0 = sl * h.P;
       nq = min(h.P, h.T - q0);
+      ksl_i = sl;
       u = uend;
-      if (nq <= 0) break;
+      if (nq <= 0 && !KTAB) break;
     } else {
       const int tt = u / h.T;
       tile = h.n_full + tt;
@@ -322,6 +338,20 @@
       bytesb = (unsigned)(BKC ? h.N : h.K) * (unsigned)h.ldb * 4u;
     }
 
+    int krow = 0;
+    if (KTAB) {
+      const int count = min(__builtin_amdgcn_readfirstlane((int)ktab_cnt), h.T);
+      const int pp = (int)__umulhi((unsigned)(count + p.ksl - 1), p.ksl_magic);
+      q0 = ksl_i * pp;
+      nq = min(pp, count - q0);
+      if (nq <= 0) break;
+      const int e = q0 + lane;
+#pragma unroll
+      for (int j = 0; j < 4; ++j) {
+        const int vj = __shfl((int)ktab_w[j], e & 63, 64);
+        krow = (e >> 6) == j ? vj : krow;
+      }
+    }
     int seg_c = 0, kt_c = 0;
     if (LEAN_TN) kt_c = q0;
     else if (q0 != 0) { seg_c = q0 / h.ntk; kt_c = q0 - seg_c * h.ntk; }
@@ -335,7 +365,12 @@
       if (FAST) {
         const __amdgpu_buffer_rsrc_t ra_src = __builtin_amdgcn_make_buffer_rsrc((void*)Ap, 0, bytesa, 0x00020000);
         const __amdgpu_buffer_rsrc_t rb_src = __builtin_amdgcn_make_buffer_rsrc((void*)Bp, 0, bytesb, 0x00020000);
-        const unsigned ka = (unsigned)kt * stepa, kb = (unsigned)kt * stepb;
+        unsigned ka = (unsigned)kt * stepa, kb = (unsigned)kt * stepb;
+        if (KTAB) {
+          const unsigned row = (unsigned)__builtin_amdgcn_readlane(krow, (kt - q0) & 63);
+          ka = row * ((unsigned)h.lda * 4u);
+          kb = row * ((unsigned)h.ldb * 4u);
+        }
         if (LEAN_SW || LEAN_EL) {
           const __amdgpu_buffer_rsrc_t la_src = __builtin_amdgcn_make_buffer_rsrc((void*)Ap, 0, live ? bytesa : 0u, 0x00020000);
           const __amdgpu_buffer_rsrc_t lb_src = __builtin_amdgcn_make_buffer_rsrc((void*)Bp, 0, live ? bytesb : 0u, 0x00020000);
@@ -1229,6 +1264,15 @@
     }
     out.lean = ok ? 1 : 0;
     if (ok) k.nt_magic = (unsigned)(((1ull << 32) + (unsigned)k.ntiles - 1) / (unsigned)k.ntiles);
+    const int S = nwg / k.ntiles;
+    if (ok && d->ktab && k.P <= 64 && k.T <= 256 && S >= 2 && S < 65536 &&
+        maxbytes + 4.0 * BK * (d->lda > d->ldb ? d->lda : d->ldb) < 4.0e9) {
+      out.lean = 4;
+      k.ktab = d->ktab;
+      k.ksl = S;
+      k.ksl_magic = (unsigned)(((1ull << 32) + (unsigned)S - 1) / (unsigned)S);
+      if (out.tag[0]) strncat(out.tag, " live", sizeof(out.tag) - strlen(out.tag) - 1);
+    }
   }
   if (out.lean) {
     int sh = 0;
@@ -1256,7 +1300,8 @@
       if (pl.lean == 3) MMNAS_LAUNCH((gemm_kernel<64, 64, true, false, true, 3, 0, 2, false, 3>), grid, block, 0, st, k);
       else if (pl.lean == 1) MMNAS_LAUNCH((gemm_kernel<64, 64, true, false, true, 3, 0, 2, false, 1>), grid, block, 0, st, k);
       else MMNAS_LAUNCH((gemm_kernel<64, 64, true, false, true, 3, 0, 2, false, 2>), grid, block, 0, st, k);
-    } else MMNAS_LAUNCH((gemm_kernel<64, 64, false, false, true, 3, 0, 2, false, 1>), grid, block, 0, st, k);
+    } else if (pl.lean == 4) MMNAS_LAUNCH((gemm_kernel<64, 64, false, false, true, 3, 0, 2, false, 4>), grid, block, 0, st, k);
+    else MMNAS_LAUNCH((gemm_kernel<64, 64, false, false, true, 3, 0, 2, false, 1>), grid, block, 0, st, k);
     return check_launch("gemm");
   }
   if (pl.big) {
@@ -1305,7 +1350,7 @@
   } else if (aux && (rc = launch_aux_reduce(*aux, st))) return rc;
   const int naux8 = (ak.njobs + 7) / 8 * 8;
   char tag[96] = "";
-  if (prof_enabled()) snprintf(tag, sizeof(tag), "PAIR %.44s | %.40s", p0.tag, p1.tag);
+  if (prof_enabled()) snprintf(tag, sizeof(tag), p1.k.ktab ? "PAIR %.44s | %.35s live" : "PAIR %.44s | %.40s", p0.tag, p1.tag);
   ProfScope ps(MMNAS_K_GEMM, p0.flops + p1.flops, p0.bytes + p1.bytes, st, tag);
   const int nwg0p = (p0.nwg + 7) / 8 * 8;
   dim3 grid(naux8 + nwg0p + p1.nwg), block(256);
@@ -1313,7 +1358,12 @@
     case 1: MMNAS_LAUNCH((gemm_pair_kernel<64, 64, 1, 2>), grid, block, 0, st, p0.k, p1.k, p0.nwg, nwg0p, ak, naux8); break;
     case 2: MMNAS_LAUNCH((gemm_pair_kernel<64, 64, 2>), grid, block, 0, st, p0.k, p1.k, p0.nwg, nwg0p, ak, naux8); break;
     case 3:
-      if (p0.lean == 3 && p1.lean) MMNAS_LAUNCH((gemm_pair_kernel<64, 64, 3, 2, 3, 1>), grid, block, 0, st, p0.k, p1.k, p0.nwg, nwg0p, ak, naux8);
+      if (p1.lean == 4) {
+        if (p0.lean == 3) MMNAS_LAUNCH((gemm_pair_kernel<64, 64, 3, 2, 3, 4>), grid, block, 0, st, p0.k, p1.k, p0.nwg, nwg0p, ak, naux8);
+        else if (p0.lean == 1) MMNAS_LAUNCH((gemm_pair_kernel<64, 64, 3, 2, 1, 4>), grid, block, 0, st, p0.k, p1.k, p0.nwg, nwg0p, ak, naux8);
+        else if (p0.lean == 2) MMNAS_LAUNCH((gemm_pair_kernel<64, 64, 3, 2, 2, 4>), grid, block, 0, st, p0.k, p1.k, p0.nwg, nwg0p, ak, naux8);
+        else MMNAS_LAUNCH((gemm_pair_kernel<64, 64, 3, 2, 0, 4>), grid, block, 0, st, p0.k, p1.k, p0.nwg, nwg0p, ak, naux8);
+      } else if (p0.lean == 3 && p1.lean) MMNAS_LAUNCH((gemm_pair_kernel<64, 64, 3, 2, 3, 1>), grid, block, 0, st, p0.k, p1.k, p0.nwg, nwg0p, ak, naux8);
       else if (p0.lean == 3) MMNAS_LAUNCH((gemm_pair_kernel<64, 64, 3, 2, 3, 0>), grid, block, 0, st, p0.k, p1.k, p0.nwg, nwg0p, ak, naux8);
       else if (p0.lean == 1 && p1.lean) MMNAS_LAUNCH((gemm_pair_kernel<64, 64, 3, 2, 1, 1>), grid, block, 0, st, p0.k, p1.k, p0.nwg, nwg0p, ak, naux8);
       else if (p0.lean == 2 && p1.lean) MMNAS_LAUNCH((gemm_pair_kernel<64, 64, 3, 2, 2, 1>), grid, block, 0, st, p0.k, p1.k, p0.nwg, nwg0p, ak, naux8);
@@ -1350,10 +1400,11 @@
   ak.njobs = 3 * ak.ncb;
   const int naux8 = (ak.njobs + 7) / 8 * 8;
   char tag[96] = "";
-  if (prof_enabled()) snprintf(tag, sizeof(tag), "WGRAD+AUX %.60s", p1.tag);
+  if (prof_enabled()) snprintf(tag, sizeof(tag), "WGRAD+AUX %.60s%s", p1.tag, p1.k.ktab ? " live" : "");
   ProfScope ps(MMNAS_K_GEMM, p1.flops, p1.bytes, st, tag);
   dim3 grid(naux8 + p1.nwg), block(256);
-  if (p1.lean) MMNAS_LAUNCH((gemm_pair_kernel<64, 64, 3, 2, 0, 1>), grid, block, 0, st, p1.k, p1.k, 0, 0, ak, naux8);
+  if (p1.lean == 4) MMNAS_LAUNCH((gemm_pair_kernel<64, 64, 3, 2, 0, 4>), grid, block, 0, st, p1.k, p1.k, 0, 0, ak, naux8);
+  else if (p1.lean) MMNAS_LAUNCH((gemm_pair_kernel<64, 64, 3, 2, 0, 1>), grid, block, 0, st, p1.k, p1.k, 0, 0, ak, naux8);
   else MMNAS_LAUNCH((gemm_pair_kernel<64, 64, 3, 2>), grid, block, 0, st, p1.k, p1.k, 0, 0, ak, naux8);
   return check_launch("gemm_wgrad_aux");
 }
diff --git a/mmnas_amd/csrc/ops.hip b/mmnas_amd/csrc/ops.hip
--- a/mmnas_amd/csrc/ops.hip
+++ b/mmnas_amd/csrc/ops.hip
@@ -240,7 +240,7 @@
 };
 
 static int att_bwd_impl(const mmnas_att_op* op, hipStream_t stream, SideQueue* sq, bool acc_kv = false, bool rel_defer = false, bool kv_defer = false,
-                        const AuxReduce* ln_pre = nullptr) {
+                        const AuxReduce* ln_pre = nullptr, const int* ktab = nullptr) {
   const bool side = sq != nullptr && !sq->rel_only;
   const bool side_rel = sq != nullptr;
   int rc = att_check(op, "att_op_bwd");
@@ -296,7 +296,7 @@
   g.g[0].M = Mq; g.g[0].A[0] = dt; g.g[0].B[0] = op->Wm; g.g[0].C = L.datt;
   gemm_init(wm, MMNAS_GEMM_TN, di, Mq, d, di, di);
   wm.g[0].M = d; wm.g[0].A[0] = dt; wm.g[0].B[0] = L.att; wm.g[0].C = op->dWm;
-  wm.accumulate = 1;
+  wm.accumulate = 1; wm.ktab = ktab;
   if (side) { if ((rc = mmnas_gemm(&g, stream))) return rc; }
   else if ((rc = gemm_pair_aux(&g, &wm, &lnred, (hipStream_t)stream))) return rc;
 
@@ -311,7 +311,7 @@
     w.g[0].M = di; w.g[0].A[0] = L.dQ; w.g[0].B[0] = op->xq;  w.g[0].C = op->dWq;
     w.g[1].M = di; w.g[1].A[0] = L.dK; w.g[1].B[0] = op->xkv; w.g[1].C = op->dWk;
     w.g[2].M = di; w.g[2].A[0] = L.dV; w.g[2].B[0] = op->xkv; w.g[2].C = op->dWv;
-    w.accumulate = 1;
+    w.accumulate = 1; w.ktab = ktab;
     gemm_init(g, MMNAS_GEMM_NN, d, di, di, d, d);
     g.nseg = 3;
     g.g[0].M = Mq; g.g[0].C = op->dxq;
@@ -325,7 +325,7 @@
   } else {
     gemm_init(w, MMNAS_GEMM_TN, d, Mq, di, d, d);
     w.g[0].M = di; w.g[0].A[0] = L.dQ; w.g[0].B[0] = op->xq; w.g[0].C = op->dWq;
-    w.accumulate = 1;
+    w.accumulate = 1; w.ktab = ktab;
     gemm_init(g, MMNAS_GEMM_NN, d, di, di, d, d);
     g.g[0].M = Mq; g.g[0].C = op->dxq; g.g[0].A[0] = L.dQ; g.g[0].B[0] = op->Wq;
     if (fl & MMNAS_F_RESIDUAL) { g.g[0].residual = dz; g.ldres = d; }
@@ -484,7 +484,7 @@
 }
 
 namespace mmnas {
-static int mlp_bwd_impl(const mmnas_mlp_op* op, hipStream_t stream, SideQueue* sq, const AuxReduce* ln_pre = nullptr) {
+static int mlp_bwd_impl(const mmnas_mlp_op* op, hipStream_t stream, SideQueue* sq, const AuxReduce* ln_pre = nullptr, const int* ktab = nullptr) {
   const bool side = sq != nullptr && !sq->rel_only;
   int rc = mlp_check(op, "mlp_op_bwd");
   if (rc) return rc;
@@ -529,7 +529,7 @@
     mmnas_gemm_desc& w = wd[i];
     gemm_init(w, MMNAS_GEMM_TN, nin, M, nout, nin, nin);
     w.g[0].M = nout; w.g[0].A[0] = dpre; w.g[0].B[0] = hin; w.g[0].C = op->dW[i];
-    w.accumulate = 1;
+    w.accumulate = 1; w.ktab = ktab;
     gemm_init(g, MMNAS_GEMM_NN, nin, nout, nout, nin, nin);
     g.g[0].M = M; g.g[0].A[0] = dpre; g.g[0].B[0] = op->W[i];
     if (i == 0) {
@@ -574,7 +574,7 @@
 struct ChainLayout {
   size_t y[MMNAS_CHAIN_MAX_OPS], save[MMNAS_CHAIN_MAX_OPS], ws[MMNAS_CHAIN_MAX_OPS], dx[MMNAS_CHAIN_MAX_OPS],
       tmp[MMNAS_CHAIN_MAX_OPS];
-  size_t dpre, encdy, relws, total;
+  size_t dpre, encdy, relws, ktab, total;
   int last_x, last_y, first_x, first_y, n_guided;
   int src[MMNAS_CHAIN_MAX_OPS], head[MMNAS_CHAIN_MAX_OPS];
   size_t nout[MMNAS_CHAIN_MAX_OPS], ndact[MMNAS_CHAIN_MAX_OPS], mixws;
@@ -687,6 +687,7 @@
     }
     L.mixws = take((size_t)(nodes > 0 ? nodes : 1) * mmnas_mixed_sum_ws_floats() * sizeof(float));
   }
+  L.ktab = L.first_y >= 0 ? L.dx[L.first_y] : 0;
   L.total = off;
   return MMNAS_OK;
 }
@@ -697,12 +698,13 @@
   mmnas_att_op a; mmnas_mlp_op m;
   AttLayout al; MlpLayout ml;
   float* y;
+  const int* ktab;
   int flags() const { return att ? a.flags : m.flags; }
   float eps() const { return att ? a.eps : m.eps; }
 };
 static inline float* chain_buf(const mmnas_chain* c, size_t off) { return (float*)((char*)c->arena + off); }
 static void chain_bind(const mmnas_chain* c, const ChainLayout& L, int i, BoundOp& b, bool layouts = false) {
-  b.i = i; b.att = c->ops[i].kind == MMNAS_CHAIN_ATT;
+  b.i = i; b.att = c->ops[i].kind == MMNAS_CHAIN_ATT; b.ktab = nullptr;
   chain_op_shapes(c, i, b.a, b.m);
   b.y = chain_buf(c, L.y[i]);
   if (b.att) { b.a.save = chain_buf(c, L.save[i]); b.a.ws = chain_buf(c, L.ws[i]); if (layouts) b.al = att_layout(&b.a); }
@@ -742,7 +744,7 @@
   return b.att ? att_fwd_impl(&b.a, s, defer_ln, ln_done, rel_ready, kv_ready) : mlp_fwd_impl(&b.m, s, defer_ln, ln_done);
 }
 static int chain_run_bwd(const BoundOp& b, hipStream_t s, SideQueue* sq, bool rel_defer, bool kv_defer, const AuxReduce* ln_pre = nullptr) {
-  return b.att ? att_bwd_impl(&b.a, s, sq, !(b.a.flags & MMNAS_F_SELF), rel_defer, kv_defer, ln_pre) : mlp_bwd_impl(&b.m, s, sq, ln_pre);
+  return b.att ? att_bwd_impl(&b.a, s, sq, !(b.a.flags & MMNAS_F_SELF), rel_defer, kv_defer, ln_pre, b.ktab) : mlp_bwd_impl(&b.m, s, sq, ln_pre, b.ktab);
 }
 static LnPlace chain_cand_view(const BoundOp& b, const float** z, const float** la, const float** lb) {
   LnPlace p = {false, false};
@@ -752,6 +754,80 @@
   else { *z = b.ml.z; *la = b.m.ln_a; *lb = b.m.ln_b; }
   return p;
 }
+
+constexpr int LIVE_MAX_ROWS = 8192;
+int sk_workspace(hipStream_t st, float** ws, size_t* ws_floats, int** cnt, int* ncnt);
+typedef unsigned u32x4_t __attribute__((ext_vector_type(4)));
+
+__global__ void __launch_bounds__(256) wgrad_live_kernel(const float* __restrict__ dy, const uint8_t* __restrict__ mask, const int M, const int d,
+                                                         int* __restrict__ tab, unsigned* __restrict__ bits, const int nwords, int* __restrict__ cnt) {
+  __shared__ int s_last;
+  const int tid = threadIdx.x, lane = tid & 63, wave = tid >> 6;
+  const int w = blockIdx.x * 4 + wave;
+  if (w < nwords) {
+    const int r0 = w * 32;
+    const int r = r0 + (lane & 31);
+    const bool in = lane < 32 && r < M;
+    const bool masked = in && mask[r] != 0;
+    const unsigned need = (unsigned)__ballot(masked);
+    unsigned live = (unsigned)__ballot(in && !masked);
+    const __amdgpu_buffer_rsrc_t rs = __builtin_amdgcn_make_buffer_rsrc((void*)dy, 0, (unsigned)M * (unsigned)d * 4u, 0x00020000);
+    for (int c0 = 0; c0 < d; c0 += 256) {
+      const int col = c0 + lane * 4;
+#pragma unroll
+      for (int hb = 0; hb < 2; ++hb) {
+        u32x4_t v[16];
+#pragma unroll
+        for (int i = 0; i < 16; ++i) {
+          const int rr = hb * 16 + i;
+          const bool ld = ((need >> rr) & 1u) != 0 && col < d;
+          v[i] = __builtin_amdgcn_raw_buffer_load_b128(rs, ld ? (unsigned)((r0 + rr) * d + col) * 4u : ~0u, 0, 0);
+        }
+#pragma unroll
+        for (int i = 0; i < 16; ++i) {
+          const bool nz = ((v[i].x | v[i].y | v[i].z | v[i].w) & 0x7fffffffu) != 0;
+          if (__ballot(nz) != 0) live |= 1u << (hb * 16 + i);
+        }
+      }
+    }
+    if (lane == 0) __hip_atomic_store(bits + w, live, __ATOMIC_RELAXED, __HIP_MEMORY_SCOPE_AGENT);
+  }
+  asm volatile("s_waitcnt vmcnt(0)" ::: "memory");
+  __syncthreads();
+  if (tid == 0) s_last = __hip_atomic_fetch_add(cnt, 1, __ATOMIC_RELAXED, __HIP_MEMORY_SCOPE_AGENT) == (int)gridDim.x - 1;
+  __syncthreads();
+  if (!s_last || wave != 0) return;
+  if (lane == 0) __hip_atomic_store(cnt, 0, __ATOMIC_RELAXED, __HIP_MEMORY_SCOPE_AGENT);
+  unsigned wd[4];
+#pragma unroll
+  for (int j = 0; j < 4; ++j) {
+    const int i = 2 * lane + (j & 1) + 128 * (j >> 1);
+    wd[j] = i < nwords ? __hip_atomic_load(bits + i, __ATOMIC_RELAXED, __HIP_MEMORY_SCOPE_AGENT) : 0u;
+  }
+  int count = 0, pos = 0;
+  while (pos < M) {
+    const int wi = pos >> 6, sl = wi & 63;
+    const unsigned lo = wi < 64 ? __builtin_amdgcn_readlane(wd[0], sl) : __builtin_amdgcn_readlane(wd[2], sl);
+    const unsigned hi = wi < 64 ? __builtin_amdgcn_readlane(wd[1], sl) : __builtin_amdgcn_readlane(wd[3], sl);
+    const unsigned long long m = (((unsigned long long)hi << 32) | lo) >> (pos & 63);
+    if (m == 0) { pos = (wi + 1) << 6; continue; }
+    const int r = pos + __builtin_ctzll(m);
+    if (lane == 0) tab[1 + count] = r;
+    ++count;
+    pos = r + 32;
+  }
+  if (lane == 0) tab[0] = count;
+}
+
+static int live_table_launch(const float* dy, const uint8_t* mask, int M, int d, int* tab, hipStream_t st) {
+  const int nwords = cdiv(M, 32);
+  float* ws; size_t wsf; int* cnt; int ncnt;
+  const int rc = sk_workspace(st, &ws, &wsf, &cnt, &ncnt);
+  if (rc) return rc;
+  MMNAS_LAUNCH(wgrad_live_kernel, dim3(cdiv(nwords, 4)), dim3(256), 0, st, dy, mask, M, d, tab, (unsigned*)(tab + 1 + nwords), nwords, cnt + ncnt - 1);
+  return check_launch("wgrad_live_table");
+}
+static bool live_table_fits(long M, int d) { return M > 0 && M <= LIVE_MAX_ROWS && d > 0 && d % 4 == 0 && (double)M * d * 4.0 < 4.0e9; }
 
 struct SideCtx { hipStream_t side; hipStream_t enc; hipEvent_t ev[MMNAS_CHAIN_MAX_OPS + 2]; hipEvent_t ovl[4]; bool used; };
 static std::mutex g_side_mu;
@@ -945,6 +1021,14 @@
 extern "C" int mmnas_set_rel_hoist(int on) { return mmnas::sw::rel_hoist.set(on != 0); }
 extern "C" int mmnas_set_chain_overlap(int on) { return mmnas::sw::chain_overlap.set(on != 0); }
 
+extern "C" int mmnas_set_wgrad_live(int on) { return sw::wgrad_live.set(on != 0); }
+extern "C" int mmnas_wgrad_live_table_ints(int M) { return M > 0 ? 2 * cdiv(M, 32) + 1 : 1; }
+extern "C" int mmnas_wgrad_live_table(const float* dy, const unsigned char* mask, int M, int d, int* tab, void* stream) {
+  MMNAS_REQUIRE(dy && mask && tab, MMNAS_E_ARG, "wgrad_live_table: null pointer");
+  MMNAS_REQUIRE(live_table_fits(M, d), MMNAS_E_SHAPE, "wgrad_live_table: M=%d (1..%d) d=%d (a multiple of 4)", M, LIVE_MAX_ROWS, d);
+  return live_table_launch(dy, mask, M, d, tab, (hipStream_t)stream);
+}
+
 extern "C" int mmnas_chain_plan(const mmnas_chain* c, size_t* arena_bytes) {
   int rc = chain_check(c, "chain_plan");
   if (rc) return rc;
@@ -984,11 +1068,21 @@
   size_t ex;
   const float* enc_grad = nullptr;
   SideCtx* rel_bwd_side = nullptr;
+  const int* ktab = nullptr;
 };
+static int chain_live_table(const mmnas_chain* c, const ChainLayout& L, hipStream_t st, const int** out) {
+  *out = nullptr;
+  if (!c->y_mask || c->y_off || L.first_y < 0 || !sw::wgrad_live.get() || !live_table_fits((long)c->B * c->Sy, c->d)) return MMNAS_OK;
+  int* tab = (int*)chain_buf(c, L.ktab);
+  const int rc = live_table_launch(c->dy_out, c->y_mask, c->B * c->Sy, c->d, tab, st);
+  if (!rc) *out = tab;
+  return rc;
+}
 static int chain_bwd_begin(ChainBwd& S, const mmnas_chain* c, const ChainLayout& L, hipStream_t st, SideQueue* sq, bool hoist) {
   S.c = c; S.L = &L; S.st = st; S.sq = sq;
   S.dpre = chain_buf(c, L.dpre); S.encdy = chain_buf(c, L.encdy);
   S.ex = (size_t)c->B * c->Sx * c->d;
+  if (int r = chain_live_table(c, L, st, &S.ktab)) return r;
   if (hoist) chain_rel_groups(c, L, true, S.RG);
   chain_guided_set(c, true, hoist, S.GS);
   S.G = -1;
@@ -1173,6 +1267,7 @@
     const int M = c->ops[i0].on_y ? (int)chain_rows_y(c) : c->B * c->Sx;
     const size_t grow = (size_t)c->ops[i0].node * c->gate_width;
     BoundOp& b = cand[act_op - i0];
+    if (c->ops[act_op].on_y) b.ktab = S.ktab;
     float* dx = chain_bind_bwd(b, c, L, dact);
     NodeLnBwd lnb;
     lnb.dz = nullptr;
@@ -1276,6 +1371,7 @@
   auto run = [&](int i, hipStream_t s, const float* dyi, const float** dxo) -> int {
     BoundOp b;
     chain_bind(c, L, i, b);
+    if (c->ops[i].on_y) b.ktab = S.ktab;
     float* dx = chain_bind_bwd(b, c, L, dyi);
     int r;
     if ((r = chain_run_bwd(b, s, sq, S.RG.hoisted[i], S.GS.hoisted[i]))) return r;
diff --git a/mmnas_amd/csrc/switches.h b/mmnas_amd/csrc/switches.h
--- a/mmnas_amd/csrc/switches.h
+++ b/mmnas_amd/csrc/switches.h
@@ -36,6 +36,7 @@
   X(rel_fwd_valu, "MMNAS_REL_FWD_VALU", 0, exact1, every_call, "1: a lone RelSelfAtt computes its bias with the per-operator fused kernel instead of the one-operator multi kernel (A/B)") \
   X(side_prio, "MMNAS_SIDE_PRIO", 1, bool, every_call, "0: the chains' extra streams without stream priorities (read when a stream pair is created)") \
   X(side_flush, "MMNAS_SIDE_FLUSH", 0, string, once, "op: side-stream parameter-gradient work released behind every operator instead of once per phase") \
+  X(wgrad_live, "MMNAS_WGRAD_LIVE", 1, int, once, "image-stream weight gradients of a padded batch's chain reduce over the 32-row K-tiles that cover the live gradient rows only (mmnas_set_wgrad_live); 0: all B Sy rows") \
    \
   X(small_ops, "MMNAS_SMALL_OPS", 1, bool, once, "SelfAtt of <= 16 rows as one launch forward (mmnas_set_small_ops); 0: the general path") \
   X(small_bwd, "MMNAS_SMALL_BWD", 1, bool, once, "the same operators' backward as two launches (mmnas_set_small_bwd)") \
```
